# modelscope/KAN-TTS

Hardware: AMD Instinct MI355X
Metric: mel-frames/sec (SAM-BERT train) (higher is better)
Workload: dtype bf16; 1 GPU; SAM-BERT full (sambert_16k.yaml zhcn) fwd+bwd+clip+Adam, batch 32/GPU, T_in 64, 14797 valid mel frames on rank 0, dropout on; global_batch=32, parallelism=dp1, launch=graph, collective_world_size=1

## Files before the change

include/kantts_hip.h:

```cpp
#ifndef KANTTS_HIP_H
#define KANTTS_HIP_H

#include <stddef.h>
#include <stdint.h>

#ifdef __cplusplus
extern "C" {
#endif

#define KANTTS_OK 0
#define KANTTS_E_BADARG (-1)
#define KANTTS_E_UNSUPPORTED (-2)
#define KANTTS_E_WORKSPACE (-3)

int kantts_abi_version(void);
const char* kantts_target_arch(void);

#define KANTTS_GEMM_MAX_SEG 4
typedef struct kantts_gemm_seg {
  const float* a;
  const float* a_gate;
  const float* b;
  int64_t a_is, a_ks;
  int64_t b_js, b_ks;
  int64_t b_tap;
  int32_t klen;
  int32_t ntaps;
  int32_t a_tok_axis;
  int32_t a_shift0, a_shift_step;
  int32_t b_tok_axis;
  int32_t b_shift0, b_shift_step;
  float a_drop_p;
  uint64_t a_drop_seed;
  int32_t a_inner, a_Tq, a_Tsrc, a_mul, a_div, a_up;
  int32_t b_inner, b_Tq, b_Tsrc, b_mul, b_div, b_up;
  float a_slope;
  int32_t a_act;
  float b_slope;
  int32_t b_act;
  float a_gate_slope;
  int32_t a_mode, b_mode;
} kantts_gemm_seg;

typedef struct kantts_gemm_args {
  kantts_gemm_seg seg[KANTTS_GEMM_MAX_SEG];
  int32_t nseg;
  int32_t M, N;
  int32_t T;
  float* c;
  int64_t c_is, c_js;
  const float* bias;
  const float* bias2;
  const float* res;
  int64_t r_is, r_js;
  const uint8_t* rowmask;
  const uint8_t* kmask;
  float* a_rowsum;
  float alpha;
  int32_t relu;
  int32_t accumulate;
  int32_t splitk;
  int32_t precision;
  float drop_p;
  uint64_t drop_seed;
  const uint64_t* seed_dev;
  int32_t groups;
  int64_t a_gs, b_gs, c_gs, bias_gs, r_gs;
  float out_slope;
  int32_t out_act;
  const float* gate;
  float gate_slope;
  int32_t z_taps;
  int64_t c_tap;
} kantts_gemm_args;

int kantts_gemm_seg_launch(const kantts_gemm_args* args_host, void* stream);

int kantts_layernorm_fwd(const float* x, const float* gamma, const float* beta, float* y, float* mean,
                         float* rstd, int M, int C, float eps, void* stream);
int kantts_layernorm_bwd(const float* dy, const float* x, const float* gamma, const float* mean,
                         const float* rstd, float* dx, float* dgamma_accum, float* dbeta_accum, int M, int C,
                         void* stream);

int kantts_attn_fwd(const float* q, const float* k, const float* v, int ldq, int ldk, int ldv, float* o, int ldo,
                    float* lse, float* probs, const int32_t* lens, const int32_t* bw_dev, int bw, int B, int H,
                    int L, int d_head, int mode, float drop_p, uint64_t seed, const uint64_t* seed_dev,
                    void* stream);
int kantts_attn_bwd(const float* q, const float* k, const float* v, int ldq, int ldk, int ldv, const float* o,
                    int ldo, const float* d_o, int lddo, const float* lse, float* dvec, float* dq, float* dk,
                    float* dv, int lddq, int lddk, int lddv, int accumulate_dq, const int32_t* lens,
                    const int32_t* bw_dev, int bw, int B, int H, int L, int d_head, int mode, float drop_p,
                    uint64_t seed, const uint64_t* seed_dev, void* stream);

int kantts_pnca_attn_fwd(const float* qkv, const float* hkv, int ldh, float* ox, float* oh, float* lse_x, float* lse_h,
                         const int32_t* lens, const int32_t* bw_dev, int bw_x, int bw_h, int B, int H, int L, int d_head,
                         float drop_p, uint64_t seed_x, uint64_t seed_h, const uint64_t* seed_dev, void* stream);
int kantts_pnca_attn_bwd(const float* qkv, const float* hkv, int ldh, const float* ox, const float* oh, const float* d_ox,
                         const float* d_oh, const float* lse_x, const float* lse_h, float* dqkv, float* dqh, float* dhkv,
                         const int32_t* lens, const int32_t* bw_dev, int bw_x, int bw_h, int B, int H, int L, int d_head,
                         float drop_p, uint64_t seed_x, uint64_t seed_h, const uint64_t* seed_dev, void* stream);

int kantts_lstm_fwd(const float* gx, const float* whh, const float* bhh, const int32_t* lens, float* out,
                    float* gates_save, float* c_save, int B, int T, int H, int ndir, int reverse_first,
                    int precision, void* stream);
int kantts_lstm_bwd(const float* dout, const float* whh, const int32_t* lens, const float* gates_save,
                    const float* c_save, float* dgates, int B, int T, int H, int ndir, int reverse_first,
                    int precision, void* stream);
int kantts_lstm_fwd_range(const float* gx, const float* whh, const float* bhh, const int32_t* lens, float* out,
                          float* gates_save, float* c_save, int B, int T, int H, int ndir, int reverse_first, int t0,
                          int t1, int precision, void* stream);

int kantts_embed_sum_fwd(const float* const* tables_host, int ntab, const int64_t* ids, const float* pos,
                         float* out, float* scaled_out, int rows, int T, int D, float scale, void* stream);
int kantts_embed_sum_bwd(float* const* dtables_host, int ntab, const int64_t* ids, const float* dout, int rows,
                         int D, float scale, void* stream);
typedef struct kantts_plan_args {
  const int64_t* in_lens;
  const int64_t* out_lens;
  const int64_t* dur;
  const float* mel;
  const float* pos;
  const float* inv_ts;
  int32_t B, N, T_mel, Tp, max_len, r, d_mel, depth;
  int64_t* in_l64;
  int32_t* in_l32;
  uint8_t* in_mask;
  int64_t* out_l64;
  int32_t* out_l32;
  uint8_t* out_mask;
  int64_t* lfr_l64;
  int32_t* lfr_l32;
  uint8_t* lfr_mask;
  int64_t* valid;
  float* pos_enc;
  float* prev;
  float* bw_val;
  int32_t* bw_dev;
  float* dec_input;
} kantts_plan_args;
int kantts_teacher_plan(const kantts_plan_args* args, void* stream);

int kantts_lr_index(const int64_t* dur_int, const float* dur_float, int32_t* idx, float* pos, int32_t* cs,
                    int64_t* lens, int B, int N, int Tp, void* stream);
int kantts_lr_gather_fwd(const float* x, const int32_t* idx, const int64_t* valid_lens, float* out, int B, int N,
                         int Tp, int C, int ldo, int out_col_offset, void* stream);
int kantts_lr_gather_bwd(const float* dout, const int32_t* cs, const int64_t* valid_lens, float* dx, int B, int N,
                         int Tp, int C, int ldo, int out_col_offset, int accumulate, void* stream);

int kantts_fsmn_dwconv_fwd(const float* x, const float* w, const float* res, const int64_t* lens, float* y, int B,
                           int T, int C, int K, int left_pad, void* stream);
int kantts_fsmn_dwconv_fwd_rows(const float* x, const float* w, const float* res, const int64_t* lens, float* y, int B,
                                int T, int C, int K, int left_pad, int t0, int t1, void* stream);
int kantts_fsmn_dwconv_bwd(const float* dy, const float* x, const float* w, const int64_t* lens, float* dx,
                           float* dw_accum, float* workspace, long long ws_floats, int B, int T, int C, int K,
                           int left_pad, void* stream);
long long kantts_fsmn_dwconv_bwd_ws(int B, int T, int C, int K);

int kantts_masked_l1(const float* pred, const float* target, const int64_t* lens, float* loss_accum, float* grad,
                     int B, int T, int C, void* stream);

int kantts_elem_loss(const float* a, const float* b, float target, int mode, float scale, float* loss_accum,
                     float* grad, long long n, void* stream);

int kantts_sumsq(const float* x, float* out_accum, long long n, void* stream);

int kantts_adam_step(float* p, const float* g, float* m, float* v, long long n, float lr, float beta1,
                     float beta2, float eps, float weight_decay, float bias_corr1, float bias_corr2,
                     const float* gnorm_sq, float max_norm, const float* dyn_lr_step, void* stream);

int kantts_melspec_fwd(const float* wav, int B, int T, int n_fft, int hop, int frames, int pad_mode,
                       const float* window, const float* twiddle, float eps_power, const int32_t* mel_start,
                       const int32_t* mel_len, const int32_t* mel_off, const float* mel_w, int n_mels,
                       float eps_mel, float* out_mel, float* out_mag, void* stream);

int kantts_melspec_norm_fwd(const float* wav, int B, int T, int n_fft, int hop, int frames, int pad_mode,
                            const float* window, const float* twiddle, float eps_power, const int32_t* mel_start,
                            const int32_t* mel_len, const int32_t* mel_off, const float* mel_w, int n_mels,
                            float eps_mel, float ref_level_db, float min_level_db, float max_norm, int symmetric,
                            float* out_mel, float* out_mag, void* stream);

int kantts_melspec_norm_fwd_fm(const float* wav, int B, int T, int n_fft, int hop, int frames, int pad_mode,
                               const float* window, const float* twiddle, float eps_power, const int32_t* mel_start,
                               const int32_t* mel_len, const int32_t* mel_off, const float* mel_w, int n_mels, float eps_mel,
                               float ref_level_db, float min_level_db, float max_norm, int symmetric, int mel_frame_major,
                               float* out_mel, float* out_mag, void* stream);
int kantts_melspec_bwd_fm(const float* wav, const float* dmel, int B, int T, int n_fft, int hop, int frames, int pad_mode,
                          const float* window, const float* twiddle, float eps_power, const int32_t* mel_start,
                          const int32_t* mel_len, const int32_t* mel_off, const float* mel_w, int n_mels, float eps_mel,
                          int mel_frame_major, float* dwav_accum, void* stream);

int kantts_copy_roof(const void* src, long long read_bytes, void* dst, long long write_bytes, void* stream);

int kantts_melspec_tuning(int grid_cap, int generic_only);

int kantts_melspec_bwd(const float* wav, const float* dmel, int B, int T, int n_fft, int hop, int frames,
                       int pad_mode, const float* window, const float* twiddle, float eps_power,
                       const int32_t* mel_start, const int32_t* mel_len, const int32_t* mel_off, const float* mel_w,
                       int n_mels, float eps_mel, float* dwav_accum, void* stream);

#define KANTTS_LOSS_MAX_TERMS 5
typedef struct kantts_loss_term {
  const float* pred;
  const void* target;
  const int64_t* lens;
  float* grad;
  int32_t B, T, C, target_log1p;
} kantts_loss_term;
int kantts_masked_l1_many(const kantts_loss_term* terms, int nterms, float* losses, void* stream);
int kantts_scale_many(float* const* x, const long long* n, int count, const float* scale_dev, void* stream);

#define KANTTS_ELOSS_MAX_TERMS 64
typedef struct kantts_eloss_term {
  const float* a;
  const float* b;
  float* grad;
  long long n;
  float target, scale;
  int32_t mode, out;
} kantts_eloss_term;
int kantts_elem_loss_many(const kantts_eloss_term* terms, int nterms, float* losses, void* stream);

int kantts_weight_norm_fwd(const float* v, const float* g, float* w, int rows, int cols, void* stream);
int kantts_weight_norm_bwd(const float* dw, const float* v, const float* g, float* dv, float* dg, int rows,
                           int cols, void* stream);

int kantts_weight_norm_strided_fwd(const float* v, const float* g, float* w, int rows, int cin, int K, long long rs,
                                   long long cs, long long ks, void* stream);
int kantts_weight_norm_strided_bwd(const float* dw, const float* v, const float* g, float* dv, float* dg, int rows,
                                   int cin, int K, long long rs, long long cs, long long ks, void* stream);

int kantts_weight_norm_tap_images(const float* v, const float* g, float* w, void* wf_bf16, void* wd_bf16, int rows, int cin,
                                  int K, int groups, void* stream);

typedef struct kantts_wn_desc {
  int64_t v_off, g_off, w_off, wf_off, wd_off;
  int32_t rows, cin, K, groups, row0, pad_;
} kantts_wn_desc;
int kantts_weight_norm_table(const float* flat, float* w, void* wf_bf16, void* wd_bf16, const kantts_wn_desc* table_dev,
                             int ndesc, int total_tiles, void* stream);

#define KANTTS_WN_BWD_MAX 64
typedef struct kantts_wn_bwd_args {
  const float* dw[KANTTS_WN_BWD_MAX];
  int32_t desc[KANTTS_WN_BWD_MAX];
  int32_t tile0[KANTTS_WN_BWD_MAX + 1];
  int32_t nl;
} kantts_wn_bwd_args;
int kantts_weight_norm_table_bwd(const float* flat, float* grad_flat, const kantts_wn_desc* table_dev,
                                 const kantts_wn_bwd_args* args, void* stream);

int kantts_sinadd_fwd(const float* x, float* y, long long n, void* stream);
int kantts_sinadd_bwd(const float* dy, const float* x, float* dx, long long n, void* stream);

typedef struct {
  const float* in;
  const float* in_gate;
  const float* w;
  float* out;
  const float* bias;
  const float* res;
  const float* out_gate;
  int B, Tsrc, Tdst, Cin_tot, Ntot, CR, NG, groups, K;
  int in_mul, in_add, in_kstep, in_div, phases;
  int inner;
  int up;
  float in_slope;
  int in_act;
  float in_gate_slope;
  float out_slope;
  int out_act;
  float out_gate_slope;
  int precision;
} kantts_conv_args;
int kantts_conv_win_launch(const kantts_conv_args* args, void* stream);

typedef struct {
  const float* x;
  const float* dy;
  const float* dy_gate;
  float* dw;
  float* db;
  int B, Tsrc, Tdst, Cin_tot, Ntot, CR, NG, groups, K;
  int stride, dil, pad, inner;
  int up;
  float x_slope;
  int x_act;
  float dy_gate_slope;
  int precision;
} kantts_convw_args;
int kantts_conv_wgrad_launch(const kantts_convw_args* args, void* stream);

typedef struct {
  const float* x;
  float* dx;
  float* y;
  const float* gate;
  const float* w;
  const float* bias;
  float* dw;
  float* db;
// ... 135 lines not shown
  int32_t relu;
  float alpha1;
  float drop1_p;
  float drop2_p;
  float xdrop_p;
  uint64_t drop1_seed;
  uint64_t drop2_seed;
  uint64_t xdrop_seed;
  const uint64_t* seed_dev;
  const void* gate;
  const uint8_t* rowmask1;
  const uint8_t* rowmask2;
  const uint8_t* xrowmask;
  void* t_out;
  const float* res;
  int64_t ldr;
  void* y;
  int64_t ldy;
  int32_t y_bf16;
  int32_t KT2, s2_first, s2_step;
  const float* ln_gamma;
  const float* ln_beta;
  void* ln_out;
  int32_t ln_out_bf16;
  float ln_eps;
  float* ln_mean;
  float* ln_rstd;
} kantts_ffn_args;
int kantts_ffn_pair(const kantts_ffn_args* args, void* stream);

typedef struct kantts_pnca_block_args {
  const float* x;
  const void* xn;
  const float* hkv;
  int64_t ldh;
  int32_t B, L, H, C, F;
  const int32_t* lens;
  const int32_t* bw_dev;
  int32_t bw_x, bw_h;
  const uint8_t* rowmask;
  const void* wqkv;
  const float* bqkv;
  const void* wfcx;
  const void* wfch;
  const float* bfcx;
  const float* bfch;
  const float* ln1_gamma;
  const float* ln1_beta;
  float ln1_eps;
  const void* w1;
  const void* w2;
  const float* bias1;
  const float* bias2;
  float att_p, fc_p, drop1_p, drop2_p;
  uint64_t seed_x, seed_h, fc_seed, drop1_seed, drop2_seed;
  const uint64_t* seed_dev;
  float* qkv;
  float* ox;
  float* oh;
  float* lse_x;
  float* lse_h;
  float* y1;
  void* xn1;
  float* mean1;
  float* rstd1;
  void* hid;
  float* out;
  const float* ln2_gamma;
  const float* ln2_beta;
  void* ln2_out;
  int32_t ln2_out_bf16;
  float ln2_eps;
  float* ln2_mean;
  float* ln2_rstd;
} kantts_pnca_block_args;
int kantts_pnca_block_fwd(const kantts_pnca_block_args* args, void* stream);

typedef struct kantts_pnca_block_bwd_args {
  const float* dy;
  const void* hid;
  const float* y1;
  const float* mean1;
  const float* rstd1;
  const float* ln1_gamma;
  const uint8_t* rowmask;
  int32_t M, C, F;
  const void* wt2;
  const void* wt1;
  const void* wfcxT;
  const void* wfchT;
  float alpha1, drop2_p, fc_p;
  uint64_t drop2_seed, fc_seed;
  const uint64_t* seed_dev;
  void* dz;
  float* g1;
  float* d_ox;
  float* d_oh;
  float* ws;
  long long ws_floats;
} kantts_pnca_block_bwd_args;
int kantts_pnca_block_bwd(const kantts_pnca_block_bwd_args* args, void* stream);
long long kantts_pnca_block_bwd_ws_floats(int M);
typedef struct kantts_pnca_attn_bwd_args {
  const float* qkv;
  const float* hkv;
  int64_t ldh;
  const float* ox;
  const float* oh;
  const float* d_ox;
  const float* d_oh;
  const float* lse_x;
  const float* lse_h;
  int32_t B, L, H, C;
  const int32_t* lens;
  const int32_t* bw_dev;
  int32_t bw_x, bw_h;
  float att_p;
  uint64_t seed_x, seed_h;
  const uint64_t* seed_dev;
  const void* wqkvT;
  const float* x;
  const float* mean0;
  const float* rstd0;
  const float* ln0_gamma;
  const float* dres;
  const uint8_t* zero_rows;
  float* dqkv;
  float* dhkv;
  int64_t lddh;
  float* dx;
  float* ws;
  long long ws_floats;
} kantts_pnca_attn_bwd_args;
int kantts_pnca_attn_qkv_bwd(const kantts_pnca_attn_bwd_args* args, void* stream);

#define KANTTS_ROWSUM_MAX 32
typedef struct kantts_rowsum_args {
  int32_t n, cols, split;
  int32_t rows[KANTTS_ROWSUM_MAX];
  const float* src[KANTTS_ROWSUM_MAX];
  float* dst0[KANTTS_ROWSUM_MAX];
  float* dst1[KANTTS_ROWSUM_MAX];
} kantts_rowsum_args;
int kantts_rows_sum_many(const kantts_rowsum_args* args, void* stream);

typedef struct kantts_fragmajor_desc {
  int64_t src_off, dst_off;
  int64_t sr, sk;
  int32_t R, K;
} kantts_fragmajor_desc;
int kantts_fragmajor_bf16(const float* src, void* dst_bf16, const kantts_fragmajor_desc* table_dev, int ndesc,
                          int blocks_per_desc, void* stream);

int kantts_ln128_fwd(const float* x, const float* gamma, const float* beta, void* y, int y_bf16, float* mean, float* rstd,
                     int M, float eps, void* stream);
int kantts_ln128_bwd(const void* dy, int dy_bf16, const float* x, const float* gamma, const float* mean, const float* rstd,
                     const float* dres, float* dx, float* dgamma_accum, float* dbeta_accum, int M, void* stream);
int kantts_ln128_bwd_rows(const void* dy, int dy_bf16, const float* x, const float* gamma, const float* mean,
                          const float* rstd, const float* dres, float* dx, float* dgamma_accum, float* dbeta_accum,
                          const unsigned char* zero_rows, int M, void* stream);

int kantts_stft_mag_bwd(const float* wav, const float* dmag, int B, int T, int n_fft, int hop, int frames, int pad_mode,
                        const float* window, const float* twiddle, float eps_power, float* dwav_accum, void* stream);

int kantts_sumsq_det(const float* x, float* out, float* workspace, long long ws_floats, long long n, void* stream);

int kantts_pnca_decode_step(const float* qkv, int ldq, float* xkv_cache, const float* hkv, float* ox, float* oh,
                            const int32_t* lens, const int32_t* bw_seq, int B, int H, int L, int d_head, int step,
                            const int32_t* step_dev, int bw, void* stream);
int kantts_step_rows(const float* src, float* dst, int B, int n, long long src_batch_stride, long long dst_batch_stride,
                     long long src_step_stride, long long dst_step_stride, int step, const int32_t* step_dev, void* stream);
int kantts_step_rowmask(const int32_t* lens, uint8_t* mask, int B, int step, const int32_t* step_dev, void* stream);

int kantts_mean_many(const float* const* xs_host, int n, float scale, float* out, void* act_bf16, float slope,
                     long long numel, void* stream);
int kantts_scale_to_many(const float* g, float scale, float* const* outs_host, int n, long long numel, void* stream);

int kantts_upsample_stream(const void* x_bf16, const void* wp_bf16, const float* bias, const void* res, void* out, int B,
                           int T, int Cin, int Cout, int S, float in_slope, int out_bf16, void* stream);
int kantts_sinadd_lrelu_fwd(const float* x, float* y, void* act_bf16, float slope, long long n, void* stream);

int kantts_dropout2_add(const float* x, const float* res, float* y, long long n, float p1, uint64_t seed1, float p2,
                        uint64_t seed2, const uint64_t* seed_dev, void* stream);

typedef struct {
  const void* in;
  const void* w;
  const float* bias;
  const float* res;
  const void* out_gate;
  float* out;
  void* out_bf;
  int B, Tsrc, Tdst, Cin_tot, Ntot, CR, NG, groups, K;
  int in_mul, in_add, in_kstep, in_div, phases;
  int inner;
  int up;
  float out_slope;
  int out_act;
  float out_gate_slope;
  int out_gate_bf16;
  float bf_slope;
  int bf_act;
  int tile;
  int res_after_gate;
} kantts_cconv_args;
int kantts_cconv_launch(const kantts_cconv_args* args, void* stream);

typedef struct {
  const void* x;
  const void* dy;
  float* dw;
  float* db;
  int B, Tsrc, Tdst, Cin_tot, Ntot, CR, NG, groups, K;
  int stride, dil, pad, inner, up;
  int slices;
  float* workspace;
  long long ws_floats;
} kantts_cconvw_args;
int kantts_cconv_wgrad_launch(const kantts_cconvw_args* args, void* stream);
long long kantts_cconv_wgrad_ws_floats(const kantts_cconvw_args* args);

int kantts_act_cast_bf16(const float* src, const void* gate, int gate_bf16, void* dst, int act, float slope, long long n,
                         void* stream);

int kantts_ragged_rows_f32(const float* src, const int64_t* row_off, const int32_t* start, const int32_t* len,
                           const float* pad, float* out, int B, int Tmax, int C, int transpose, void* stream);
int kantts_ragged_rows_i64(const int64_t* src, const int64_t* row_off, const int32_t* start, const int32_t* len,
                           const int64_t* pad, int64_t* out, int B, int Tmax, int C, int transpose, void* stream);

int kantts_launch_tuning(int tn_tile, int tn_slices, int c1_wgrad_wgs);

typedef struct kantts_decode_args {
  const void* w;
  const float* f;
  const float* memory;
  const float* hkv;
  float* xkv;
  float* out;
  const int32_t* lens;
  const int32_t* bw_seq;
  int B, L, d_mem, d_mel, d_out, n_layer, bw;
  float in_scale;
  float eps;
} kantts_decode_args;
int kantts_pnca_decode_run(const kantts_decode_args* args, void* stream);
int kantts_pnca_decode_range(const kantts_decode_args* args, int t0, int t1, void* stream);
int kantts_pnca_decode_blob_sizes(int d_mel, int d_mem, int d_out, int n_layer, long long* w_elems, long long* f_elems);

typedef struct kantts_durar_args {
  const void* w;
  const float* f;
  const float* gc;
  float* out;
  const int32_t* lens;
  int B, T;
} kantts_durar_args;
int kantts_dur_ar_run(const kantts_durar_args* args, void* stream);
int kantts_dur_ar_run_f32(const kantts_durar_args* args, void* stream);

typedef struct kantts_ctc_args {
  const float* logits;
  const int32_t* in_lens;
  const int32_t* out_lens;
  float* ws;
  float* loss;
  float* grad;
  int B, T1, T2;
  float blank;
  float grad_scale;
} kantts_ctc_args;
long long kantts_ctc_attn_workspace(int B, int T1, int T2);
int kantts_ctc_attn(const kantts_ctc_args* args, void* stream);

typedef struct kantts_enc_attn_args {
  const float* x;
  const void* xn;
  const int32_t* lens;
  const uint8_t* rowmask;
  const void* wqkv;
  const float* bqkv;
  const void* wfc;
  const float* bfc;
  const float* ln1_gamma;
  const float* ln1_beta;
  float ln1_eps;
  float att_p, fc_p;
  uint64_t att_seed, fc_seed;
  const uint64_t* seed_dev;
  float* qkv;
  float* o;
  float* lse;
  float* y1;
  void* xn1;
  int xn1_bf16;
  float* mean1;
  float* rstd1;
  int B, L;
} kantts_enc_attn_args;
int kantts_enc_attn_fwd(const kantts_enc_attn_args* args, void* stream);

typedef struct {
  const float* in;
  const float* hist_in;
  float* hist_out;
  const void* w;
  const float* bias;
// ... 17 lines not shown
```

kan-tts_amd/csrc/ffn_pair.hip:

```cpp
#include "common.h"

typedef float f32x4 __attribute__((ext_vector_type(4)));
typedef __bf16 bf16x8 __attribute__((ext_vector_type(8)));
typedef __bf16 bf16x4 __attribute__((ext_vector_type(4)));
typedef unsigned int u32x4 __attribute__((ext_vector_type(4)));
typedef unsigned int u32x2 __attribute__((ext_vector_type(2)));

#define FP_THREADS 512
#define FP_BM 32
#define FP_K1 128
#define FP_N 128
#define FP_F 1024
#define FP_XP (FP_K1 + 16)
#define FP_XROWS 40
#define FP_TP (FP_F + 16)

__device__ __forceinline__ unsigned fp_pack2(float a, float b) {
  bf16x4 t = {(__bf16)a, (__bf16)b, (__bf16)0.f, (__bf16)0.f};
  return ((u32x2&)t).x;
}
__device__ __forceinline__ float fp_lo(unsigned u) { return __uint_as_float(u << 16); }
__device__ __forceinline__ float fp_hi(unsigned u) { return __uint_as_float(u & 0xffff0000u); }

template <bool BWD, int KT2>
__global__ __launch_bounds__(FP_THREADS) void ffn_pair_kernel(const kantts_ffn_args g) {
#include "ffn_pair_body.inc"
}
static bool fp_aligned16(const void* p) { return ((uintptr_t)p & 15) == 0; }

extern "C" int kantts_ffn_pair(const kantts_ffn_args* gp, void* stream) {
  if (!gp) return KANTTS_E_BADARG;
  const kantts_ffn_args& g = *gp;
  if (!g.x || !g.w1 || !g.w2 || !g.y || g.M < 0 || g.KT < 1) return KANTTS_E_BADARG;
  if (g.K1 != FP_K1 || g.N != FP_N || g.F != FP_F) return KANTTS_E_UNSUPPORTED;
  if (g.KT > 9 || g.pad < 0 || g.pad >= g.KT || (g.KT > 1 && g.T <= 0)) return KANTTS_E_UNSUPPORTED;
  if ((g.ldx & 7) || (g.ldy & 3) || (g.res && (g.ldr & 3))) return KANTTS_E_UNSUPPORTED;
  if (!fp_aligned16(g.x) || !fp_aligned16(g.w1) || !fp_aligned16(g.w2) || !fp_aligned16(g.y) ||
      (g.t_out && !fp_aligned16(g.t_out)) || (g.gate && !fp_aligned16(g.gate)) || (g.res && !fp_aligned16(g.res)) ||
      (g.bias1 && !fp_aligned16(g.bias1)) || (g.bias2 && !fp_aligned16(g.bias2)))
    return KANTTS_E_UNSUPPORTED;
  if (g.xdrop_p > 0.f && !g.x_f32) return KANTTS_E_UNSUPPORTED;
  if (g.gate && g.KT != 1) return KANTTS_E_UNSUPPORTED;
  const int kt2 = g.KT2 < 1 ? 1 : g.KT2;
  if (kt2 != 1 && kt2 != 3) return KANTTS_E_UNSUPPORTED;
  if (kt2 == 3 && (!g.gate || g.T <= 0 || (g.s2_step != 1 && g.s2_step != -1) || g.M % g.T)) return KANTTS_E_UNSUPPORTED;
  if (g.ln_out) {
    if (!g.ln_gamma || !g.ln_beta || !g.ln_mean || !g.ln_rstd) return KANTTS_E_BADARG;
    if (g.gate || kt2 != 1 || !fp_aligned16(g.ln_out) || !fp_aligned16(g.ln_gamma) || !fp_aligned16(g.ln_beta))
      return KANTTS_E_UNSUPPORTED;
  }
  if (g.M == 0) return KANTTS_OK;
  hipStream_t st = (hipStream_t)stream;
  if (kt2 == 3)
    hipLaunchKernelGGL((ffn_pair_kernel<true, 3>), dim3(kantts_cdiv(g.M, FP_BM - 2)), dim3(FP_THREADS), 0, st, g);
  else if (g.gate)
    hipLaunchKernelGGL((ffn_pair_kernel<true, 1>), dim3(kantts_cdiv(g.M, FP_BM)), dim3(FP_THREADS), 0, st, g);
  else
    hipLaunchKernelGGL((ffn_pair_kernel<false, 1>), dim3(kantts_cdiv(g.M, FP_BM)), dim3(FP_THREADS), 0, st, g);
  KANTTS_CHECK_LAUNCH();
}

__global__ __launch_bounds__(256) void fragmajor_bf16_kernel(const float* __restrict__ src, __bf16* __restrict__ dst,
                                                            const kantts_fragmajor_desc* __restrict__ tab) {
  const kantts_fragmajor_desc d = tab[blockIdx.y];
  const long long total = (long long)d.R * d.K;
  const unsigned KB = (unsigned)d.K >> 5;
  const bool fast = total < (1ll << 31) && (d.dst_off & 7) == 0;
  if (fast) {
    const unsigned total8 = (unsigned)(total >> 3);
    const bool contig = d.sk == 1 && ((d.src_off | d.sr) & 3) == 0;
    for (unsigned o8 = blockIdx.x * blockDim.x + threadIdx.x; o8 < total8; o8 += gridDim.x * blockDim.x) {
      const unsigned lane = o8 & 63u, blk = o8 >> 6;
      const unsigned rb = blk / KB, kb = blk - rb * KB;
      const long long r = (long long)rb * 16 + (lane & 15u), k0 = (long long)kb * 32 + (lane >> 4) * 8;
      const float* sp = src + d.src_off + r * d.sr + k0 * d.sk;
      float v[8];
      if (contig) {
        const float4 a = reinterpret_cast<const float4*>(sp)[0], b = reinterpret_cast<const float4*>(sp)[1];
        v[0] = a.x, v[1] = a.y, v[2] = a.z, v[3] = a.w, v[4] = b.x, v[5] = b.y, v[6] = b.z, v[7] = b.w;
      } else {
#pragma unroll
        for (int e = 0; e < 8; ++e) v[e] = sp[(long long)e * d.sk];
      }
      bf16x8 o;
#pragma unroll
      for (int e = 0; e < 8; ++e) o[e] = (__bf16)v[e];
      *reinterpret_cast<bf16x8*>(dst + d.dst_off + (long long)o8 * 8) = o;
    }
    return;
  }
  for (long long o = (long long)blockIdx.x * blockDim.x + threadIdx.x; o < total; o += (long long)gridDim.x * blockDim.x) {
    const int e = (int)(o & 7), lane = (int)((o >> 3) & 63);
    const long long blk = o >> 9;
    const int kb = (int)(blk % KB), rb = (int)(blk / KB);
    const long long r = (long long)rb * 16 + (lane & 15), k = (long long)kb * 32 + (lane >> 4) * 8 + e;
    dst[d.dst_off + o] = (__bf16)src[d.src_off + r * d.sr + k * d.sk];
  }
}

extern "C" int kantts_fragmajor_bf16(const float* src, void* dst, const kantts_fragmajor_desc* table_dev, int ndesc,
                                     int blocks_per_desc, void* stream) {
  if (!src || !dst || !table_dev || ndesc < 0 || blocks_per_desc < 1) return KANTTS_E_BADARG;
  if (ndesc == 0) return KANTTS_OK;
  hipLaunchKernelGGL(fragmajor_bf16_kernel, dim3(blocks_per_desc, ndesc), dim3(256), 0, (hipStream_t)stream, src,
                     reinterpret_cast<__bf16*>(dst), table_dev);
  KANTTS_CHECK_LAUNCH();
}
```

kan-tts_amd/csrc/gemm_bf16.hip:

```cpp
#include <stdlib.h>

#include "common.h"

typedef float f32x4 __attribute__((ext_vector_type(4)));
typedef __bf16 bf16x8 __attribute__((ext_vector_type(8)));
typedef __bf16 bf16x4 __attribute__((ext_vector_type(4)));
typedef unsigned int u32x4 __attribute__((ext_vector_type(4)));
typedef unsigned int u32x2 __attribute__((ext_vector_type(2)));

#define BG_THREADS 256
#define BG_BN 128
#define BG_BK 64
#define BG_LDKN (BG_BN + 16)

typedef __attribute__((address_space(3))) bf16x4 bg_lds_bf16x4;
__device__ __forceinline__ bf16x4 bg_tr4(const __bf16* p) {
  return __builtin_amdgcn_ds_read_tr16_b64_v4bf16((bg_lds_bf16x4*)(p));
}

__device__ __forceinline__ unsigned bg_pack2(float a, float b) {
  bf16x4 t = {(__bf16)a, (__bf16)b, (__bf16)0.f, (__bf16)0.f};
  return ((u32x2&)t).x;
}
__device__ __forceinline__ float bg_lo(unsigned u) { return __uint_as_float(u << 16); }
// ... 320 lines not shown
#pragma unroll
      for (int m = 0; m < MR; ++m)
#pragma unroll
        for (int n = 0; n < NR; ++n)
          acc[m][n] = __builtin_amdgcn_mfma_f32_16x16x32_bf16(af[m], bf[n], acc[m][n], 0, 0, 0);
    }
  };

  const int st = g.slices;
  int t = slice;
  const int tlast = ntile - 1;
  fetch(min(t, tlast), ra0, rb0);
  fetch(min(t + st, tlast), ra1, rb1);
  for (; t < ntile; t += 2 * st) {
    commit(0, t, ra0, rb0);
    __syncthreads();
    fetch(min(t + 2 * st, tlast), ra0, rb0);
    compute(0);
    if (t + st < ntile) {
      commit(1, t + st, ra1, rb1);
      __syncthreads();
      fetch(min(t + 3 * st, tlast), ra1, rb1);
      compute(1);
    }
  }

  if (do_bias && tid < BN && (n0 + tid) < g.N && colsum != 0.f) atomicAdd(&g.db[n0 + tid], colsum * g.alpha);
  float* cbase = g.c + (long long)tap * g.c_ts;
#pragma unroll
  for (int m = 0; m < MR; ++m)
#pragma unroll
    for (int n = 0; n < NR; ++n)
#pragma unroll
      for (int r = 0; r < 4; ++r) {
        const int i = n0 + wr * (BN / 2) + m * 16 + kg * 4 + r;
        const int j = c0 + wc * (BK / 2) + n * 16 + li;
        if (i < g.N && j < g.K) {
          const float v = acc[m][n][r] * g.alpha;
#ifdef TN_NO_ATOMICS
          if (v != 0.f) cbase[(long long)i * g.c_ns + (long long)j * g.c_ks] = v;
#else
          if (v != 0.f) atomicAdd(cbase + (long long)i * g.c_ns + (long long)j * g.c_ks, v);
#endif
        }
      }
}

template <bool A_F32, bool B_F32, int BN, int BK>
static int bg_tn_go(TnGroupArgs& ga, dim3 grid, hipStream_t st) {
  constexpr size_t LDS = 2 * (size_t)TN_BT * ((BN + 16) + (BK + 16)) * 2;
  static bool attr_set = false;
  if (!attr_set && LDS > 64 * 1024) {
    hipError_t e = hipFuncSetAttribute(reinterpret_cast<const void*>(&bgemm_tn_kernel<A_F32, B_F32, BN, BK>),
                                       hipFuncAttributeMaxDynamicSharedMemorySize, (int)LDS);
    if (e != hipSuccess) return (int)e;
    attr_set = true;
  }
  hipLaunchKernelGGL((bgemm_tn_kernel<A_F32, B_F32, BN, BK>), grid, dim3(BG_THREADS), LDS, st, ga);
  KANTTS_CHECK_LAUNCH();
}

template <int BN, int BK>
static int bg_tn_dispatch(TnGroupArgs& ga, dim3 grid, hipStream_t st) {
  const kantts_bgemm_tn_args& g = ga.g;
  if (g.a_f32) {
    if (g.b_f32) return bg_tn_go<true, true, BN, BK>(ga, grid, st);
    return bg_tn_go<true, false, BN, BK>(ga, grid, st);
  }
  if (g.b_f32) return bg_tn_go<false, true, BN, BK>(ga, grid, st);
  return bg_tn_go<false, false, BN, BK>(ga, grid, st);
}

static int bg_tn_tile_rule(const kantts_bgemm_tn_args& g, int nprob) {
  (void)g;
  (void)nprob;
  return 64128;
}

static int bg_tn_launch(TnGroupArgs& ga, hipStream_t st) {
  kantts_bgemm_tn_args& g = ga.g;
  if (g.M < 0 || g.N < 1 || g.K < 1 || g.ntaps < 1 || ga.nprob < 1 || ga.nprob > KANTTS_TN_MAX_GROUP) return KANTTS_E_BADARG;
  if (g.M == 0) return KANTTS_OK;
  if ((g.N & 7) || (g.K & 7) || (g.lda & 7) || (g.ldb & 7)) return KANTTS_E_UNSUPPORTED;
  for (int p = 0; p < ga.nprob; ++p) {
    if (!ga.a[p] || !ga.b[p] || !ga.c[p]) return KANTTS_E_BADARG;
    if (!bg_aligned16(ga.a[p]) || !bg_aligned16(ga.b[p])) return KANTTS_E_UNSUPPORTED;
  }
  if ((g.shift0 != 0 || g.shift_step != 0) && g.T <= 0) return KANTTS_E_BADARG;
  int code = kantts_tune_tn_tile.load(std::memory_order_relaxed);
  const int forced_slices = kantts_tune_tn_slices.load(std::memory_order_relaxed);
  bool xcd_map = true;
  if (code == 64129 || code == 128129 || code == 64257 || code == 128257) code -= 1, xcd_map = false;
  if (code != 64128 && code != 128128 && code != 64256 && code != 128256) code = bg_tn_tile_rule(g, ga.nprob);
  const int BN = code / 1000, BK = code % 1000;
  const int tiles = kantts_cdiv(g.N, BN) * kantts_cdiv(g.K, BK) * g.ntaps * ga.nprob;
  const int ntile = kantts_cdiv(g.M, TN_BT);
  int slices = g.slices;
  if (forced_slices > 0) slices = forced_slices;
  if (slices <= 0) {
    static const bool r2_rule = getenv("KANTTS_TN_SLICE_RULE_R2") != nullptr;
    slices = r2_rule ? kantts_cdiv(320, tiles) : 512 / tiles;
    if (xcd_map && !r2_rule) {
      const int P = kantts_cdiv(g.N, BN) * kantts_cdiv(g.K, BK);
      const int per_xcd = P <= 64 ? 64 / P : 1;
      slices = 8 * per_xcd / (g.ntaps * ga.nprob);
    }
    if (slices < 1) slices = 1;
    if (slices > 16 && !r2_rule) slices = 16;
    const long long cap = ((r2_rule ? 3ll << 19 : 1ll << 22)) / ((long long)g.N * g.K * g.ntaps * ga.nprob) + 1;
    if (slices > cap) slices = (int)cap;
  }
  if (slices > ntile) slices = ntile;
  if (slices < 1) slices = 1;
  g.slices = slices;
  dim3 grid(kantts_cdiv(g.K, BK), kantts_cdiv(g.N, BN), ga.nprob * g.ntaps * slices);
  ga.ktiles = ga.ntiles = ga.ngroups = 0;
  if (xcd_map && (int)grid.z * 4 < 3 * 8 * kantts_cdiv((int)grid.z, 8)) xcd_map = false;
  if (xcd_map) {
    ga.ktiles = (int)grid.x, ga.ntiles = (int)grid.y, ga.ngroups = (int)grid.z;
    grid = dim3(8u * grid.x * grid.y * (unsigned)kantts_cdiv(ga.ngroups, 8), 1, 1);
  }
  switch (code) {
    case 128256: return bg_tn_dispatch<128, 256>(ga, grid, st);
    case 128128: return bg_tn_dispatch<128, 128>(ga, grid, st);
    case 64256: return bg_tn_dispatch<64, 256>(ga, grid, st);
    default: return bg_tn_dispatch<64, 128>(ga, grid, st);
  }
}

extern "C" int kantts_bgemm_tn(const kantts_bgemm_tn_args* gp, void* stream) {
  if (!gp) return KANTTS_E_BADARG;
  TnGroupArgs ga = {};
  ga.g = *gp;
  ga.nprob = 1;
  ga.a[0] = gp->a; ga.b[0] = gp->b; ga.c[0] = gp->c; ga.db[0] = gp->db; ga.a_drop_seed[0] = gp->a_drop_seed;
  return bg_tn_launch(ga, (hipStream_t)stream);
}

extern "C" int kantts_bgemm_tn_grouped(const kantts_bgemm_tn_args* shape, int nprob, const void* const* a,
                                       const void* const* b, float* const* c, float* const* db,
                                       const uint64_t* a_drop_seed, void* stream) {
  if (!shape || !a || !b || !c || nprob < 1 || nprob > KANTTS_TN_MAX_GROUP) return KANTTS_E_BADARG;
  TnGroupArgs ga = {};
  ga.g = *shape;
  ga.nprob = nprob;
  for (int p = 0; p < nprob; ++p) {
    ga.a[p] = a[p]; ga.b[p] = b[p]; ga.c[p] = c[p];
    ga.db[p] = db ? db[p] : nullptr;
    ga.a_drop_seed[p] = a_drop_seed ? a_drop_seed[p] : shape->a_drop_seed;
  }
  return bg_tn_launch(ga, (hipStream_t)stream);
}

__global__ __launch_bounds__(256) void cast_bf16_kernel(const float* __restrict__ src, __bf16* __restrict__ dst, long long n8) {
  const long long i = (long long)blockIdx.x * blockDim.x + threadIdx.x;
  if (i >= n8) return;
  const float4 a = reinterpret_cast<const float4*>(src)[2 * i], b = reinterpret_cast<const float4*>(src)[2 * i + 1];
  u32x4 w = {bg_pack2(a.x, a.y), bg_pack2(a.z, a.w), bg_pack2(b.x, b.y), bg_pack2(b.z, b.w)};
  reinterpret_cast<u32x4*>(dst)[i] = w;
}

extern "C" int kantts_cast_f32_bf16(const float* src, void* dst, long long n, void* stream) {
  if (!src || !dst || n < 0 || (n & 7) || !bg_aligned16(src) || !bg_aligned16(dst)) return KANTTS_E_BADARG;
  if (n == 0) return KANTTS_OK;
  const long long n8 = n / 8;
  hipLaunchKernelGGL(cast_bf16_kernel, dim3(kantts_cdiv(n8, 256)), dim3(256), 0, (hipStream_t)stream, src,
                     reinterpret_cast<__bf16*>(dst), n8);
  KANTTS_CHECK_LAUNCH();
}

__global__ __launch_bounds__(256) void tapmajor_bf16_kernel(const float* __restrict__ src, __bf16* __restrict__ dst,
                                                           const kantts_tapmajor_desc* __restrict__ tab) {
  const kantts_tapmajor_desc d = tab[blockIdx.y];
  const long long total = (long long)d.N * d.Cin * d.KT;
  for (long long o = (long long)blockIdx.x * blockDim.x + threadIdx.x; o < total; o += (long long)gridDim.x * blockDim.x) {
    const int c = (int)(o % d.Cin);
    const long long q = o / d.Cin;
    const int n = (int)(q % d.N), tap = (int)(q / d.N);
    dst[d.dst_off + o] = (__bf16)src[d.src_off + ((long long)n * d.Cin + c) * d.KT + tap];
  }
}

extern "C" int kantts_tapmajor_bf16(const float* src, void* dst, const kantts_tapmajor_desc* table_dev, int ndesc,
                                    int blocks_per_desc, void* stream) {
  if (!src || !dst || !table_dev || ndesc < 0 || blocks_per_desc < 1) return KANTTS_E_BADARG;
  if (ndesc == 0) return KANTTS_OK;
  hipLaunchKernelGGL(tapmajor_bf16_kernel, dim3(blocks_per_desc, ndesc), dim3(256), 0, (hipStream_t)stream, src,
                     reinterpret_cast<__bf16*>(dst), table_dev);
  KANTTS_CHECK_LAUNCH();
}

template <bool DY_BF16, bool Y_BF16>
__global__ __launch_bounds__(256) void relu_gate_kernel(const void* __restrict__ dy, const void* __restrict__ y,
                                                       __bf16* __restrict__ dz, float scale, long long n8) {
  const long long i = (long long)blockIdx.x * blockDim.x + threadIdx.x;
  if (i >= n8) return;
  float d[8], a[8];
  if (DY_BF16) {
    const u32x4 q = reinterpret_cast<const u32x4*>(dy)[i];
    d[0] = bg_lo(q.x); d[1] = bg_hi(q.x); d[2] = bg_lo(q.y); d[3] = bg_hi(q.y);
    d[4] = bg_lo(q.z); d[5] = bg_hi(q.z); d[6] = bg_lo(q.w); d[7] = bg_hi(q.w);
  } else {
    const float4 p = reinterpret_cast<const float4*>(dy)[2 * i], q = reinterpret_cast<const float4*>(dy)[2 * i + 1];
    d[0] = p.x; d[1] = p.y; d[2] = p.z; d[3] = p.w; d[4] = q.x; d[5] = q.y; d[6] = q.z; d[7] = q.w;
  }
  if (Y_BF16) {
    const u32x4 q = reinterpret_cast<const u32x4*>(y)[i];
    a[0] = bg_lo(q.x); a[1] = bg_hi(q.x); a[2] = bg_lo(q.y); a[3] = bg_hi(q.y);
    a[4] = bg_lo(q.z); a[5] = bg_hi(q.z); a[6] = bg_lo(q.w); a[7] = bg_hi(q.w);
  } else {
    const float4 p = reinterpret_cast<const float4*>(y)[2 * i], q = reinterpret_cast<const float4*>(y)[2 * i + 1];
    a[0] = p.x; a[1] = p.y; a[2] = p.z; a[3] = p.w; a[4] = q.x; a[5] = q.y; a[6] = q.z; a[7] = q.w;
  }
  float o[8];
#pragma unroll
  for (int e = 0; e < 8; ++e) o[e] = a[e] > 0.f ? d[e] * scale : 0.f;
  u32x4 w = {bg_pack2(o[0], o[1]), bg_pack2(o[2], o[3]), bg_pack2(o[4], o[5]), bg_pack2(o[6], o[7])};
  reinterpret_cast<u32x4*>(dz)[i] = w;
}

extern "C" int kantts_relu_gate_bf16(const void* dy, int dy_bf16, const void* y, int y_bf16, void* dz_bf16, float scale,
                                     long long n, void* stream) {
  if (!dy || !y || !dz_bf16 || n < 0 || (n & 7) || !bg_aligned16(dy) || !bg_aligned16(y) || !bg_aligned16(dz_bf16))
    return KANTTS_E_BADARG;
  if (n == 0) return KANTTS_OK;
  const long long n8 = n / 8;
  dim3 grid(kantts_cdiv(n8, 256)), block(256);
  hipStream_t st = (hipStream_t)stream;
  __bf16* o = reinterpret_cast<__bf16*>(dz_bf16);
  if (dy_bf16) {
    if (y_bf16)
      hipLaunchKernelGGL((relu_gate_kernel<true, true>), grid, block, 0, st, dy, y, o, scale, n8);
    else
      hipLaunchKernelGGL((relu_gate_kernel<true, false>), grid, block, 0, st, dy, y, o, scale, n8);
  } else {
    if (y_bf16)
      hipLaunchKernelGGL((relu_gate_kernel<false, true>), grid, block, 0, st, dy, y, o, scale, n8);
    else
      hipLaunchKernelGGL((relu_gate_kernel<false, false>), grid, block, 0, st, dy, y, o, scale, n8);
  }
  KANTTS_CHECK_LAUNCH();
}
```

kan-tts_amd/csrc/seq.hip:

```cpp
#include "common.h"

struct EmbedArgs {
  const float* tab[4];
  int ntab;
  const int64_t* ids;
  const float* pos;
  float* out;
  float* scaled;
  int rows, T, D;
  float scale;
};

__global__ void embed_sum_kernel(const EmbedArgs a) {
  long long idx = (long long)blockIdx.x * blockDim.x + threadIdx.x;
  long long total = (long long)a.rows * a.D;
  if (idx >= total) return;
  int row = (int)(idx / a.D), d = (int)(idx % a.D);
  float s = 0.f;
  for (int k = 0; k < a.ntab; ++k) s += a.tab[k][(long long)a.ids[(long long)row * a.ntab + k] * a.D + d];
  s *= a.scale;
  if (a.scaled) a.scaled[idx] = s;
  if (a.pos) s += a.pos[(long long)(row % a.T) * a.D + d];
  a.out[idx] = s;
}
// ... 53 lines not shown
      for (int w = 0; w < EB_WAYS; ++w) {
        if (w == next) {
          if (tag[w] >= 0) atomicAdd(&tab[tag[w] * a.D + d], acc[w]);
          tag[w] = id;
          acc[w] = g;
        }
      }
      next = (next + 1) & (EB_WAYS - 1);
    }
   }
  }
#pragma unroll
  for (int w = 0; w < EB_WAYS; ++w)
    if (tag[w] >= 0) atomicAdd(&tab[tag[w] * a.D + d], acc[w]);
}

extern "C" int kantts_embed_sum_fwd(const float* const* tables_host, int ntab, const int64_t* ids, const float* pos,
                                    float* out, float* scaled_out, int rows, int T, int D, float scale, void* stream) {
  if (!tables_host || ntab < 1 || ntab > 4 || !ids || !out || rows < 0 || D < 1 || T < 1) return KANTTS_E_BADARG;
  if (rows == 0) return KANTTS_OK;
  EmbedArgs a = {};
  for (int k = 0; k < ntab; ++k) a.tab[k] = tables_host[k];
  a.ntab = ntab; a.ids = ids; a.pos = pos; a.out = out; a.scaled = scaled_out; a.rows = rows; a.T = T; a.D = D;
  a.scale = scale;
  hipLaunchKernelGGL(embed_sum_kernel, dim3(kantts_cdiv((long long)rows * D, 256)), dim3(256), 0, (hipStream_t)stream, a);
  KANTTS_CHECK_LAUNCH();
}

extern "C" int kantts_embed_sum_bwd(float* const* dtables_host, int ntab, const int64_t* ids, const float* dout,
                                    int rows, int D, float scale, void* stream) {
  if (!dtables_host || ntab < 1 || ntab > 4 || !ids || !dout || rows < 0 || D < 1) return KANTTS_E_BADARG;
  if (rows == 0) return KANTTS_OK;
  EmbedBwdArgs a = {};
  for (int k = 0; k < ntab; ++k) a.dtab[k] = dtables_host[k];
  a.ntab = ntab; a.ids = ids; a.dout = dout; a.rows = rows; a.D = D; a.scale = scale;
  const long long threads = (long long)kantts_cdiv(rows, EB_CHUNK) * ntab * D;
  hipLaunchKernelGGL(embed_sum_bwd_kernel, dim3(kantts_cdiv(threads, 256)), dim3(256), 0, (hipStream_t)stream, a);
  KANTTS_CHECK_LAUNCH();
}

__global__ __launch_bounds__(64) void lr_index_kernel(const int64_t* __restrict__ dur_i, const float* __restrict__ dur_f,
                                                      int32_t* __restrict__ idx, float* __restrict__ pos,
                                                      int32_t* __restrict__ cs, int64_t* __restrict__ lens, int N,
                                                      int Tp) {
  const int b = blockIdx.x, lane = threadIdx.x;
  int32_t* csb = cs + (long long)b * (N + 1);
  int carry = 0;
  for (int n0 = 0; n0 < N; n0 += 64) {
    int n = n0 + lane;
    int rep = 0;
    if (n < N) {
      if (dur_i)
        rep = (int)dur_i[(long long)b * N + n];
      else
        rep = (int)(long long)(dur_f[(long long)b * N + n] + 0.5f);
    }
    int v = rep;
#pragma unroll
    for (int off = 1; off < 64; off <<= 1) {
      int u = __shfl_up(v, off, 64);
      if (lane >= off) v += u;
    }
    if (n < N) csb[n + 1] = carry + v;
    carry += __shfl(v, 63, 64);
  }
  if (lane == 0) {
    csb[0] = 0;
    lens[b] = carry;
  }
  __syncthreads();
  __threadfence_block();
  const int total = carry;
  for (int t = lane; t < Tp; t += 64) {
    int id = -1;
    float p = (float)(t + 1);
    if (t < total) {
      int lo = 0, hi = N;
      while (hi - lo > 1) {
        int mid = (lo + hi) >> 1;
        if (csb[mid] <= t)
          lo = mid;
        else
          hi = mid;
      }
      id = lo;
      p = (float)(t - csb[lo] + 1);
    }
    idx[(long long)b * Tp + t] = id;
    pos[(long long)b * Tp + t] = p;
  }
}

extern "C" int kantts_lr_index(const int64_t* dur_int, const float* dur_float, int32_t* idx, float* pos, int32_t* cs,
                               int64_t* lens, int B, int N, int Tp, void* stream) {
  if ((!dur_int && !dur_float) || !idx || !pos || !cs || !lens || B < 0 || N < 1 || Tp < 0) return KANTTS_E_BADARG;
  if (B == 0) return KANTTS_OK;
  hipLaunchKernelGGL(lr_index_kernel, dim3(B), dim3(64), 0, (hipStream_t)stream, dur_int, dur_float, idx, pos, cs,
                     lens, N, Tp);
  KANTTS_CHECK_LAUNCH();
}

__global__ void lr_gather_kernel(const float* __restrict__ x, const int32_t* __restrict__ idx,
                                 const int64_t* __restrict__ valid, float* __restrict__ out, int B, int N, int Tp, int C,
                                 int ldo, int ooff) {
  long long g = (long long)blockIdx.x * blockDim.x + threadIdx.x;
  long long total = (long long)B * Tp * C;
  if (g >= total) return;
  int c = (int)(g % C);
  long long bt = g / C;
  int t = (int)(bt % Tp), b = (int)(bt / Tp);
  int id = idx[bt];
  float v = 0.f;
  if (id >= 0 && (!valid || t < (int)valid[b])) v = x[((long long)b * N + id) * C + c];
  out[bt * ldo + ooff + c] = v;
}

__global__ void lr_gather_bwd_kernel(const float* __restrict__ dout, const int32_t* __restrict__ cs,
                                     const int64_t* __restrict__ valid, float* __restrict__ dx, int B, int N, int Tp,
                                     int C, int ldo, int ooff, int accumulate) {
  long long g = (long long)blockIdx.x * blockDim.x + threadIdx.x;
  long long total = (long long)B * N * C;
  if (g >= total) return;
  int c = (int)(g % C);
  long long bn = g / C;
  int n = (int)(bn % N), b = (int)(bn / N);
  int s = cs[(long long)b * (N + 1) + n], e = cs[(long long)b * (N + 1) + n + 1];
  if (e > Tp) e = Tp;
  if (valid && e > (int)valid[b]) e = (int)valid[b];
  float acc = 0.f;
  for (int t = s; t < e; ++t) acc += dout[((long long)b * Tp + t) * ldo + ooff + c];
  if (accumulate)
    dx[g] += acc;
  else
    dx[g] = acc;
}

extern "C" int kantts_lr_gather_fwd(const float* x, const int32_t* idx, const int64_t* valid_lens, float* out, int B,
                                    int N, int Tp, int C, int ldo, int out_col_offset, void* stream) {
  if (!x || !idx || !out || B < 0 || N < 1 || Tp < 0 || C < 1 || ldo < C) return KANTTS_E_BADARG;
  long long total = (long long)B * Tp * C;
  if (total == 0) return KANTTS_OK;
  hipLaunchKernelGGL(lr_gather_kernel, dim3(kantts_cdiv(total, 256)), dim3(256), 0, (hipStream_t)stream, x, idx,
                     valid_lens, out, B, N, Tp, C, ldo, out_col_offset);
  KANTTS_CHECK_LAUNCH();
}

extern "C" int kantts_lr_gather_bwd(const float* dout, const int32_t* cs, const int64_t* valid_lens, float* dx, int B,
                                    int N, int Tp, int C, int ldo, int out_col_offset, int accumulate, void* stream) {
  if (!dout || !cs || !dx || B < 0 || N < 1 || Tp < 0 || C < 1 || ldo < C) return KANTTS_E_BADARG;
  long long total = (long long)B * N * C;
  if (total == 0) return KANTTS_OK;
  hipLaunchKernelGGL(lr_gather_bwd_kernel, dim3(kantts_cdiv(total, 256)), dim3(256), 0, (hipStream_t)stream, dout, cs,
                     valid_lens, dx, B, N, Tp, C, ldo, out_col_offset, accumulate);
  KANTTS_CHECK_LAUNCH();
}

#define DW_TT 32
template <bool ROWS>
__global__ void fsmn_dwconv_fwd_kernel(const float* __restrict__ x, const float* __restrict__ w,
                                       const float* __restrict__ res, const int64_t* __restrict__ lens,
                                       float* __restrict__ y, int B, int T, int C, int K, int lp, int r0, int r1) {
  const int b = blockIdx.y, t0 = (ROWS ? r0 : 0) + blockIdx.x * DW_TT;
  const int len = lens ? (int)min((long long)lens[b], (long long)T) : T;
  const float* xb = x + (long long)b * T * C;
  for (int c = threadIdx.x; c < C; c += blockDim.x) {
    const float* wc = w + (long long)c * K;
    for (int tt = 0; tt < DW_TT; ++tt) {
      const int t = t0 + tt;
      if (t >= (ROWS ? r1 : T)) break;
      float acc = 0.f;
      if (t < len) {
        for (int k = 0; k < K; ++k) {
          int ts = t + k - lp;
          if (ts >= 0 && ts < len) acc = fmaf(wc[k], xb[(long long)ts * C + c], acc);
        }
        acc += xb[(long long)t * C + c];
      }
      long long o = ((long long)b * T + t) * C + c;
      if (res) acc += res[o];
      y[o] = acc;
    }
  }
}

__global__ void fsmn_dwconv_bwd_dx_kernel(const float* __restrict__ dy, const float* __restrict__ w,
                                          const int64_t* __restrict__ lens, float* __restrict__ dx, int B, int T, int C,
                                          int K, int lp) {
  const int b = blockIdx.y, t0 = blockIdx.x * DW_TT;
  const int len = lens ? (int)min((long long)lens[b], (long long)T) : T;
  const float* db = dy + (long long)b * T * C;
  for (int c = threadIdx.x; c < C; c += blockDim.x) {
    const float* wc = w + (long long)c * K;
    for (int tt = 0; tt < DW_TT; ++tt) {
      const int t = t0 + tt;
      if (t >= T) break;
      float acc = 0.f;
      if (t < len) {
        for (int k = 0; k < K; ++k) {
          int ts = t - k + lp;
          if (ts >= 0 && ts < len) acc = fmaf(wc[k], db[(long long)ts * C + c], acc);
        }
        acc += db[(long long)t * C + c];
      }
      dx[((long long)b * T + t) * C + c] = acc;
    }
  }
}

#define DW_WT 128
__global__ void fsmn_dwconv_bwd_dw_kernel(const float* __restrict__ dy, const float* __restrict__ x,
                                          const int64_t* __restrict__ lens, float* __restrict__ dw, int B, int T, int C,
                                          int K, int lp) {
  const int b = blockIdx.y, t0 = blockIdx.x * DW_WT;
  const int len = lens ? (int)min((long long)lens[b], (long long)T) : T;
  if (t0 >= len) return;
  const int t1 = min(t0 + DW_WT, len);
  const float* db = dy + (long long)b * T * C;
  const float* xb = x + (long long)b * T * C;
  for (int c = threadIdx.x; c < C; c += blockDim.x) {
    for (int k = 0; k < K; ++k) {
      float acc = 0.f;
      for (int t = t0; t < t1; ++t) {
        int ts = t + k - lp;
        if (ts >= 0 && ts < len) acc = fmaf(db[(long long)t * C + c], xb[(long long)ts * C + c], acc);
      }
      atomicAdd(&dw[(long long)c * K + k], acc);
    }
  }
}

#define FS_K 41
#define FS_TT 16
template <bool FLIP, bool ROWS>
__global__ __launch_bounds__(256, 2) void fsmn_fir41_kernel(const float* __restrict__ x, const float* __restrict__ w,
                                                        const float* __restrict__ res,
                                                        const int64_t* __restrict__ lens, float* __restrict__ y, int B,
                                                        int T, int C, int lp, int xcd_order, int r0, int r1) {
  int bx = blockIdx.x, by = blockIdx.y;
  if (xcd_order) {
    const int gx = gridDim.x, total = gx * gridDim.y;
    if (total >= 64) {
      const int L = by * gx + bx, k = L & 7, j = L >> 3;
      const int q = total >> 3, r = total & 7;
      const int vid = k * q + (k < r ? k : r) + j;
      by = vid / gx;
      bx = vid - by * gx;
    }
  }
  const int b = by, t0 = (ROWS ? r0 : 0) + bx * FS_TT;
  const int len = lens ? (int)min((long long)lens[b], (long long)T) : T;
  const int lpe = FLIP ? (FS_K - 1 - lp) : lp;
  const int xlim = ROWS ? min(len, r1 + (FS_K - 1 - lpe)) : len;
  const int tlim = ROWS ? r1 : T;
  const float* xb = x + (long long)b * T * C;
  for (int c = threadIdx.x; c < C; c += blockDim.x) {
    float wk[FS_K];
#pragma unroll
    for (int k = 0; k < FS_K; ++k) wk[k] = w[(long long)c * FS_K + (FLIP ? (FS_K - 1 - k) : k)];
    float xin[FS_TT + FS_K - 1];
#pragma unroll
    for (int n = 0; n < FS_TT + FS_K - 1; ++n) {
      const int ts = t0 + n - lpe;
      const bool ok = (ts >= 0) && (ts < xlim);
      const float v = xb[(long long)(ok ? ts : 0) * C + c];
      xin[n] = ok ? v : 0.f;
    }
    float ctr[FS_TT];
#pragma unroll
    for (int o = 0; o < FS_TT; ++o) {
      const int t = t0 + o;
      const bool ok = t < (ROWS ? min(len, r1) : len);
      const float v = xb[(long long)(ok ? t : 0) * C + c];
      ctr[o] = ok ? v : 0.f;
    }
#pragma unroll
    for (int o = 0; o < FS_TT; ++o) {
      const int t = t0 + o;
      float acc = ctr[o];
#pragma unroll
      for (int k = 0; k < FS_K; ++k) acc = fmaf(wk[k], xin[o + k], acc);
      if (t < tlim) {
        const long long oidx = ((long long)b * T + t) * C + c;
        float outv = (t < len) ? acc : 0.f;
        if (!FLIP && res) outv += res[oidx];
        y[oidx] = outv;
      }
    }
  }
}

#define FS_CH 128
#define FS_SUB (FS_CH / 4)
__global__ __launch_bounds__(256) void fsmn_dw41_partial_kernel(const float* __restrict__ dy, const float* __restrict__ x,
                                                            const int64_t* __restrict__ lens,
                                                            float* __restrict__ part, int B, int T, int C, int lp) {
  __shared__ float sm[4][FS_K][65];
  const int b = blockIdx.y, chunk = blockIdx.x, nchunk = gridDim.x;
  const int wave = threadIdx.x >> 6, lane = threadIdx.x & 63;
  const int c0 = blockIdx.z * 64, c = c0 + lane;
  const bool cok = c < C;
  const int cc = cok ? c : 0;
  const int len = lens ? (int)min((long long)lens[b], (long long)T) : T;
  const float* xb = x + (long long)b * T * C;
  const float* db = dy + (long long)b * T * C;
  const int tbeg = chunk * FS_CH + wave * FS_SUB, tend = min(tbeg + FS_SUB, T);
  float acc[FS_K];
// ... 223 lines not shown
```

kan-tts_amd/kantts/_hip/__init__.py:

```python
import ctypes
import os
from ctypes import (POINTER, Structure, c_char_p, c_float, c_int, c_int32, c_int64, c_longlong,
                    c_uint64, c_void_p)

import torch

_HERE = os.path.dirname(os.path.abspath(__file__))
LIB_PATH = os.environ.get("KANTTS_LIB") or os.path.normpath(os.path.join(_HERE, "..", "..", "libkantts_hip.so"))
_lib = None

GEMM_MAX_SEG = 4
PREC_FP32, PREC_BF16, PREC_REF = 0, 1, 2


class GemmSeg(Structure):
    _fields_ = [
        ("a", c_void_p), ("a_gate", c_void_p), ("b", c_void_p),
        ("a_is", c_int64), ("a_ks", c_int64), ("b_js", c_int64), ("b_ks", c_int64), ("b_tap", c_int64),
        ("klen", c_int32), ("ntaps", c_int32),
        ("a_tok_axis", c_int32), ("a_shift0", c_int32), ("a_shift_step", c_int32),
        ("b_tok_axis", c_int32), ("b_shift0", c_int32), ("b_shift_step", c_int32),
        ("a_drop_p", c_float), ("a_drop_seed", c_uint64),
        ("a_inner", c_int32), ("a_Tq", c_int32), ("a_Tsrc", c_int32), ("a_mul", c_int32), ("a_div", c_int32),
        ("a_up", c_int32),
# ... 125 lines not shown
        ("x", c_void_p), ("gamma", c_void_p), ("mean", c_void_p), ("rstd", c_void_p), ("dres", c_void_p),
        ("zero_rows", c_void_p), ("dx", c_void_p), ("dgamma_accum", c_void_p), ("dbeta_accum", c_void_p),
        ("part_rows", c_void_p),
    ]


LOSS_MAX_TERMS = 5


class LossTerm(Structure):
    _fields_ = [("pred", c_void_p), ("target", c_void_p), ("lens", c_void_p), ("grad", c_void_p),
                ("B", c_int32), ("T", c_int32), ("C", c_int32), ("target_log1p", c_int32)]


ELOSS_MAX_TERMS = 64


class ElossTerm(Structure):
    _fields_ = [("a", c_void_p), ("b", c_void_p), ("grad", c_void_p), ("n", ctypes.c_longlong), ("target", ctypes.c_float),
                ("scale", ctypes.c_float), ("mode", c_int32), ("out", c_int32)]


WN_BWD_MAX = 64


class WnBwdArgs(Structure):
    _fields_ = [("dw", c_void_p * WN_BWD_MAX), ("desc", c_int32 * WN_BWD_MAX), ("tile0", c_int32 * (WN_BWD_MAX + 1)),
                ("nl", c_int32)]


class BGemmTnArgs(Structure):
    _fields_ = [
        ("a", c_void_p), ("b", c_void_p), ("lda", c_int64), ("ldb", c_int64),
        ("M", c_int32), ("N", c_int32), ("K", c_int32), ("T", c_int32),
        ("a_f32", c_int32), ("b_f32", c_int32),
        ("ntaps", c_int32), ("shift0", c_int32), ("shift_step", c_int32), ("slices", c_int32),
        ("c", c_void_p), ("c_ns", c_int64), ("c_ks", c_int64), ("c_ts", c_int64),
        ("db", c_void_p), ("alpha", c_float), ("a_drop_p", c_float),
        ("a_drop_seed", c_uint64), ("seed_dev", c_void_p),
    ]


class FfnArgs(Structure):
    _fields_ = [
        ("x", c_void_p), ("ldx", c_int64), ("x_f32", c_int32),
        ("M", c_int32), ("T", c_int32), ("K1", c_int32), ("F", c_int32), ("N", c_int32), ("KT", c_int32), ("pad", c_int32),
        ("w1", c_void_p), ("w2", c_void_p), ("bias1", c_void_p), ("bias2", c_void_p),
        ("relu", c_int32), ("alpha1", c_float), ("drop1_p", c_float), ("drop2_p", c_float), ("xdrop_p", c_float),
        ("drop1_seed", c_uint64), ("drop2_seed", c_uint64), ("xdrop_seed", c_uint64), ("seed_dev", c_void_p),
        ("gate", c_void_p), ("rowmask1", c_void_p), ("rowmask2", c_void_p), ("xrowmask", c_void_p),
        ("t_out", c_void_p), ("res", c_void_p), ("ldr", c_int64), ("y", c_void_p), ("ldy", c_int64), ("y_bf16", c_int32),
        ("KT2", c_int32), ("s2_first", c_int32), ("s2_step", c_int32),
        ("ln_gamma", c_void_p), ("ln_beta", c_void_p), ("ln_out", c_void_p), ("ln_out_bf16", c_int32), ("ln_eps", c_float),
        ("ln_mean", c_void_p), ("ln_rstd", c_void_p),
    ]


class PncaBlockArgs(Structure):
    _fields_ = [
        ("x", c_void_p), ("xn", c_void_p), ("hkv", c_void_p), ("ldh", c_int64),
        ("B", c_int32), ("L", c_int32), ("H", c_int32), ("C", c_int32), ("F", c_int32),
        ("lens", c_void_p), ("bw_dev", c_void_p), ("bw_x", c_int32), ("bw_h", c_int32), ("rowmask", c_void_p),
        ("wqkv", c_void_p), ("bqkv", c_void_p), ("wfcx", c_void_p), ("wfch", c_void_p), ("bfcx", c_void_p), ("bfch", c_void_p),
        ("ln1_gamma", c_void_p), ("ln1_beta", c_void_p), ("ln1_eps", c_float),
        ("w1", c_void_p), ("w2", c_void_p), ("bias1", c_void_p), ("bias2", c_void_p),
        ("att_p", c_float), ("fc_p", c_float), ("drop1_p", c_float), ("drop2_p", c_float),
        ("seed_x", c_uint64), ("seed_h", c_uint64), ("fc_seed", c_uint64), ("drop1_seed", c_uint64), ("drop2_seed", c_uint64),
        ("seed_dev", c_void_p),
        ("qkv", c_void_p), ("ox", c_void_p), ("oh", c_void_p), ("lse_x", c_void_p), ("lse_h", c_void_p), ("y1", c_void_p),
        ("xn1", c_void_p), ("mean1", c_void_p), ("rstd1", c_void_p), ("hid", c_void_p), ("out", c_void_p),
        ("ln2_gamma", c_void_p), ("ln2_beta", c_void_p), ("ln2_out", c_void_p), ("ln2_out_bf16", c_int32), ("ln2_eps", c_float),
        ("ln2_mean", c_void_p), ("ln2_rstd", c_void_p),
    ]


class PncaBlockBwdArgs(Structure):
    _fields_ = [
        ("dy", c_void_p), ("hid", c_void_p), ("y1", c_void_p), ("mean1", c_void_p), ("rstd1", c_void_p), ("ln1_gamma", c_void_p),
        ("rowmask", c_void_p), ("M", c_int32), ("C", c_int32), ("F", c_int32),
        ("wt2", c_void_p), ("wt1", c_void_p), ("wfcxT", c_void_p), ("wfchT", c_void_p),
        ("alpha1", c_float), ("drop2_p", c_float), ("fc_p", c_float), ("drop2_seed", c_uint64), ("fc_seed", c_uint64),
        ("seed_dev", c_void_p),
        ("dz", c_void_p), ("g1", c_void_p), ("d_ox", c_void_p), ("d_oh", c_void_p), ("ws", c_void_p), ("ws_floats", c_int64),
    ]


class PncaAttnBwdArgs(Structure):
    _fields_ = [
        ("qkv", c_void_p), ("hkv", c_void_p), ("ldh", c_int64), ("ox", c_void_p), ("oh", c_void_p), ("d_ox", c_void_p),
        ("d_oh", c_void_p), ("lse_x", c_void_p), ("lse_h", c_void_p),
        ("B", c_int32), ("L", c_int32), ("H", c_int32), ("C", c_int32),
        ("lens", c_void_p), ("bw_dev", c_void_p), ("bw_x", c_int32), ("bw_h", c_int32), ("att_p", c_float),
        ("seed_x", c_uint64), ("seed_h", c_uint64), ("seed_dev", c_void_p),
        ("wqkvT", c_void_p), ("x", c_void_p), ("mean0", c_void_p), ("rstd0", c_void_p), ("ln0_gamma", c_void_p),
        ("dres", c_void_p), ("zero_rows", c_void_p),
        ("dqkv", c_void_p), ("dhkv", c_void_p), ("lddh", c_int64), ("dx", c_void_p), ("ws", c_void_p), ("ws_floats", c_int64),
    ]


class PlanArgs(Structure):
    _fields_ = [("in_lens", c_void_p), ("out_lens", c_void_p), ("dur", c_void_p), ("mel", c_void_p), ("pos", c_void_p),
                ("inv_ts", c_void_p),
                ("B", c_int32), ("N", c_int32), ("T_mel", c_int32), ("Tp", c_int32), ("max_len", c_int32), ("r", c_int32),
                ("d_mel", c_int32), ("depth", c_int32),
                ("in_l64", c_void_p), ("in_l32", c_void_p), ("in_mask", c_void_p), ("out_l64", c_void_p), ("out_l32", c_void_p),
                ("out_mask", c_void_p), ("lfr_l64", c_void_p), ("lfr_l32", c_void_p), ("lfr_mask", c_void_p),
                ("valid", c_void_p), ("pos_enc", c_void_p), ("prev", c_void_p), ("bw_val", c_void_p), ("bw_dev", c_void_p),
                ("dec_input", c_void_p)]


class DecodeArgs(Structure):
    _fields_ = [("w", c_void_p), ("f", c_void_p), ("memory", c_void_p), ("hkv", c_void_p), ("xkv", c_void_p),
                ("out", c_void_p), ("lens", c_void_p), ("bw_seq", c_void_p),
                ("B", c_int32), ("L", c_int32), ("d_mem", c_int32), ("d_mel", c_int32), ("d_out", c_int32),
                ("n_layer", c_int32), ("bw", c_int32), ("in_scale", c_float), ("eps", c_float)]


class DurArArgs(Structure):
    _fields_ = [("w", c_void_p), ("f", c_void_p), ("gc", c_void_p), ("out", c_void_p), ("lens", c_void_p),
                ("B", c_int32), ("T", c_int32)]


class EncAttnArgs(Structure):
    _fields_ = [("x", c_void_p), ("xn", c_void_p), ("lens", c_void_p), ("rowmask", c_void_p), ("wqkv", c_void_p),
                ("bqkv", c_void_p), ("wfc", c_void_p), ("bfc", c_void_p), ("ln1_gamma", c_void_p), ("ln1_beta", c_void_p),
                ("ln1_eps", c_float), ("att_p", c_float), ("fc_p", c_float), ("att_seed", c_uint64), ("fc_seed", c_uint64),
                ("seed_dev", c_void_p), ("qkv", c_void_p), ("o", c_void_p), ("lse", c_void_p), ("y1", c_void_p),
                ("xn1", c_void_p), ("xn1_bf16", c_int32), ("mean1", c_void_p), ("rstd1", c_void_p), ("B", c_int32),
                ("L", c_int32)]


class CtcArgs(Structure):
    _fields_ = [("logits", c_void_p), ("in_lens", c_void_p), ("out_lens", c_void_p), ("ws", c_void_p), ("loss", c_void_p),
                ("grad", c_void_p), ("B", c_int32), ("T1", c_int32), ("T2", c_int32), ("blank", c_float),
                ("grad_scale", c_float)]


ROWSUM_MAX = 32


class RowSumArgs(Structure):
    _fields_ = [("n", c_int32), ("cols", c_int32), ("split", c_int32), ("rows", c_int32 * ROWSUM_MAX),
                ("src", c_void_p * ROWSUM_MAX), ("dst0", c_void_p * ROWSUM_MAX), ("dst1", c_void_p * ROWSUM_MAX)]


class FragMajorDesc(Structure):
    _fields_ = [("src_off", c_int64), ("dst_off", c_int64), ("sr", c_int64), ("sk", c_int64), ("R", c_int32),
                ("K", c_int32)]


class TapMajorDesc(Structure):
    _fields_ = [("src_off", c_int64), ("dst_off", c_int64), ("N", c_int32), ("Cin", c_int32), ("KT", c_int32),
                ("pad_", c_int32)]


def available() -> bool:
    return os.path.exists(LIB_PATH)


def lib():
    global _lib
    if _lib is None:
        if not os.path.exists(LIB_PATH):
            raise RuntimeError(
                "libkantts_hip.so is not built (%s). Run `python -c 'import __graft_entry__ as g; g.build()'` "
                "or `make -C kan-tts_amd/csrc`. There is no CPU fallback." % LIB_PATH)
        L = ctypes.CDLL(LIB_PATH)
        L.kantts_abi_version.restype = c_int
        L.kantts_target_arch.restype = c_char_p
        L.kantts_gemm_seg_launch.argtypes = [POINTER(GemmArgs), c_void_p]
        i, f, p, ll, u64 = c_int, c_float, c_void_p, c_longlong, c_uint64
        L.kantts_layernorm_fwd.argtypes = [p, p, p, p, p, p, i, i, f, p]
        L.kantts_layernorm_bwd.argtypes = [p, p, p, p, p, p, p, p, i, i, p]
        L.kantts_attn_fwd.argtypes = [p, p, p, i, i, i, p, i, p, p, p, p, i, i, i, i, i, i, f, u64, p, p]
        L.kantts_attn_bwd.argtypes = [p, p, p, i, i, i, p, i, p, i, p, p, p, p, p, i, i, i, i, p, p, i, i, i, i, i,
                                      i, f, u64, p, p]
        L.kantts_pnca_attn_fwd.argtypes = [p, p, i, p, p, p, p, p, p, i, i, i, i, i, i, f, u64, u64, p, p]
        L.kantts_pnca_attn_bwd.argtypes = [p, p, i, p, p, p, p, p, p, p, p, p, p, p, i, i, i, i, i, i, f, u64, u64, p, p]
        L.kantts_lstm_fwd.argtypes = [p, p, p, p, p, p, p, i, i, i, i, i, i, p]
        L.kantts_attn_decode.argtypes = [p, p, p, i, i, i, p, i, p, p, i, i, i, i, i, i, i, p]
        L.kantts_lstm_cell.argtypes = [p, p, p, p, i, i, p]
        L.kantts_mas_width1.argtypes = [p, p, p, p, p, i, i, i, p]
        L.kantts_align_attn_fwd.argtypes = [p, p, p, p, p, p, i, i, i, i, p]
        L.kantts_align_attn_bwd.argtypes = [p, p, p, p, p, p, p, p, p, p, i, i, i, i, p]
        L.kantts_lstm_bwd.argtypes = [p, p, p, p, p, p, i, i, i, i, i, i, p]
        L.kantts_embed_sum_fwd.argtypes = [POINTER(c_void_p), i, p, p, p, p, i, i, i, f, p]
        L.kantts_embed_sum_bwd.argtypes = [POINTER(c_void_p), i, p, p, i, i, f, p]
        L.kantts_lr_index.argtypes = [p, p, p, p, p, p, i, i, i, p]
        L.kantts_lr_gather_fwd.argtypes = [p, p, p, p, i, i, i, i, i, i, p]
        L.kantts_lr_gather_bwd.argtypes = [p, p, p, p, i, i, i, i, i, i, i, p]
        L.kantts_fsmn_dwconv_fwd.argtypes = [p, p, p, p, p, i, i, i, i, i, p]
        L.kantts_fsmn_dwconv_bwd.argtypes = [p, p, p, p, p, p, p, ll, i, i, i, i, i, p]
        L.kantts_fsmn_dwconv_bwd_ws.argtypes = [i, i, i, i]
        L.kantts_fsmn_dwconv_bwd_ws.restype = ll
        L.kantts_masked_l1.argtypes = [p, p, p, p, p, i, i, i, p]
        L.kantts_sumsq.argtypes = [p, p, ll, p]
        L.kantts_elem_loss.argtypes = [p, p, f, i, f, p, p, ll, p]
        L.kantts_adam_step.argtypes = [p, p, p, p, ll, f, f, f, f, f, f, f, p, f, p, p]
        L.kantts_melspec_fwd.argtypes = [p, i, i, i, i, i, i, p, p, f, p, p, p, p, i, f, p, p, p]
        L.kantts_melspec_norm_fwd.argtypes = [p, i, i, i, i, i, i, p, p, f, p, p, p, p, i, f, f, f, f, i, p, p, p]
        L.kantts_melspec_bwd.argtypes = [p, p, i, i, i, i, i, i, p, p, f, p, p, p, p, i, f, p, p]
        L.kantts_melspec_norm_fwd_fm.argtypes = [p, i, i, i, i, i, i, p, p, f, p, p, p, p, i, f, f, f, f, i, i, p, p, p]
        L.kantts_melspec_bwd_fm.argtypes = [p, p, i, i, i, i, i, i, p, p, f, p, p, p, p, i, f, i, p, p]
        L.kantts_weight_norm_fwd.argtypes = [p, p, p, i, i, p]
        L.kantts_weight_norm_bwd.argtypes = [p, p, p, p, p, i, i, p]
        L.kantts_weight_norm_strided_fwd.argtypes = [p, p, p, i, i, i, ll, ll, ll, p]
        L.kantts_weight_norm_strided_bwd.argtypes = [p, p, p, p, p, i, i, i, ll, ll, ll, p]
        L.kantts_sinadd_fwd.argtypes = [p, p, ll, p]
        L.kantts_sinadd_bwd.argtypes = [p, p, p, ll, p]
        L.kantts_conv_win_launch.argtypes = [POINTER(ConvArgs), c_void_p]
        L.kantts_conv_wgrad_launch.argtypes = [POINTER(ConvWArgs), c_void_p]
        L.kantts_conv_c1_launch.argtypes = [POINTER(ConvC1Args), c_int, c_void_p]
        L.kantts_pnca_decode_step.argtypes = [p, i, p, p, p, p, p, p, i, i, i, i, i, p, i, p]
        L.kantts_step_rows.argtypes = [p, p, i, i, ll, ll, ll, ll, i, p, p]
        L.kantts_step_rowmask.argtypes = [p, p, i, i, p, p]
        L.kantts_upsample_stream.argtypes = [p, p, p, p, p, i, i, i, i, i, f, i, p]
        L.kantts_sinadd_lrelu_fwd.argtypes = [p, p, p, f, ll, p]
        L.kantts_dropout2_add.argtypes = [p, p, p, ll, f, c_uint64, f, c_uint64, p, p]
        L.kantts_sumsq_det.argtypes = [p, p, p, ll, ll, p]
        L.kantts_stft_mag_bwd.argtypes = [p, p, i, i, i, i, i, i, p, p, f, p, p]
        L.kantts_bgemm_nt.argtypes = [POINTER(BGemmArgs), c_void_p]
        L.kantts_ffn_pair.argtypes = [POINTER(FfnArgs), c_void_p]
        L.kantts_pnca_block_fwd.argtypes = [POINTER(PncaBlockArgs), c_void_p]
        L.kantts_pnca_block_bwd.argtypes = [POINTER(PncaBlockBwdArgs), c_void_p]
        L.kantts_rows_sum_many.argtypes = [POINTER(RowSumArgs), c_void_p]
        L.kantts_teacher_plan.argtypes = [POINTER(PlanArgs), c_void_p]
        L.kantts_pnca_attn_qkv_bwd.argtypes = [POINTER(PncaAttnBwdArgs), c_void_p]
        L.kantts_copy_roof.argtypes = [c_void_p, ctypes.c_longlong, c_void_p, ctypes.c_longlong, c_void_p]
        L.kantts_launch_tuning.argtypes = [c_int, c_int, c_int]
        L.kantts_pnca_decode_run.argtypes = [POINTER(DecodeArgs), c_void_p]
        L.kantts_dur_ar_run.argtypes = [POINTER(DurArArgs), c_void_p]
        L.kantts_dur_ar_run_f32.argtypes = [POINTER(DurArArgs), c_void_p]
        L.kantts_enc_attn_fwd.argtypes = [POINTER(EncAttnArgs), c_void_p]
        L.kantts_ctc_attn.argtypes = [POINTER(CtcArgs), c_void_p]
        L.kantts_ctc_attn_workspace.argtypes = [c_int, c_int, c_int]
        L.kantts_ctc_attn_workspace.restype = c_longlong
        L.kantts_pnca_decode_blob_sizes.argtypes = [c_int, c_int, c_int, c_int, POINTER(ctypes.c_longlong),
                                                    POINTER(ctypes.c_longlong)]
        L.kantts_pnca_block_bwd_ws_floats.argtypes = [c_int]
        L.kantts_pnca_block_bwd_ws_floats.restype = ctypes.c_longlong
        L.kantts_fragmajor_bf16.argtypes = [c_void_p, c_void_p, c_void_p, c_int, c_int, c_void_p]
        L.kantts_bgemm_tn.argtypes = [POINTER(BGemmTnArgs), c_void_p]
        L.kantts_bgemm_tn_grouped.argtypes = [POINTER(BGemmTnArgs), c_int, p, p, p, p, p, c_void_p]
        L.kantts_cast_f32_bf16.argtypes = [p, p, ll, p]
        L.kantts_tapmajor_bf16.argtypes = [p, p, p, i, i, p]
        L.kantts_relu_gate_bf16.argtypes = [p, i, p, i, p, f, ll, p]
        L.kantts_ln128_fwd.argtypes = [p, p, p, p, i, p, p, i, f, p]
        L.kantts_ln128_bwd.argtypes = [p, i, p, p, p, p, p, p, p, p, i, p]
        L.kantts_bgemm_nt_lnbwd.argtypes = [POINTER(BGemmArgs), POINTER(LnBwdArgs), c_void_p]
        L.kantts_ln128_bwd_rows.argtypes = [p, i, p, p, p, p, p, p, p, p, p, i, p]
        L.kantts_cconv_launch.argtypes = [POINTER(CConvArgs), c_void_p]
        L.kantts_cconv_wgrad_launch.argtypes = [POINTER(CConvWArgs), c_void_p]
        L.kantts_cconv_wgrad_ws_floats.argtypes = [POINTER(CConvWArgs)]
        L.kantts_cconv_wgrad_ws_floats.restype = ll
        L.kantts_act_cast_bf16.argtypes = [p, p, i, p, i, f, ll, p]
        L.kantts_ragged_rows_f32.argtypes = [p, p, p, p, p, p, i, i, i, i, p]
        L.kantts_weight_norm_tap_images.argtypes = [p, p, p, p, p, i, i, i, i, p]
        L.kantts_weight_norm_table.argtypes = [p, p, p, p, p, i, i, p]
        L.kantts_weight_norm_table_bwd.argtypes = [p, p, p, POINTER(WnBwdArgs), p]
        L.kantts_masked_l1_many.argtypes = [POINTER(LossTerm), i, p, p]
        L.kantts_scale_many.argtypes = [POINTER(c_void_p), POINTER(ll), i, p, p]
        L.kantts_conv_n1_launch.argtypes = [POINTER(ConvN1Args), i, p]
        L.kantts_elem_loss_many.argtypes = [POINTER(ElossTerm), i, p, p]
        L.kantts_mean_many.argtypes = [POINTER(c_void_p), i, f, p, p, f, ll, p]
        L.kantts_scale_to_many.argtypes = [p, f, POINTER(c_void_p), i, ll, p]
        L.kantts_ragged_rows_i64.argtypes = [p, p, p, p, p, p, i, i, i, i, p]
        L.kantts_sconv_launch.argtypes = [POINTER(SConvArgs), c_void_p]
        L.kantts_pnca_decode_range.argtypes = [POINTER(DecodeArgs), c_int, c_int, c_void_p]
        L.kantts_lstm_fwd_range.argtypes = [p, p, p, p, p, p, p, i, i, i, i, i, i, i, i, p]
        L.kantts_fsmn_dwconv_fwd_rows.argtypes = [p, p, p, p, p, i, i, i, i, i, i, i, p]
        _lib = L
    return _lib


EXPORTED_SYMBOLS = [
    "kantts_abi_version", "kantts_target_arch", "kantts_gemm_seg_launch", "kantts_layernorm_fwd",
    "kantts_layernorm_bwd", "kantts_attn_fwd", "kantts_attn_bwd", "kantts_pnca_attn_fwd", "kantts_pnca_attn_bwd", "kantts_lstm_fwd", "kantts_lstm_bwd",
    "kantts_embed_sum_fwd", "kantts_embed_sum_bwd", "kantts_lr_index", "kantts_lr_gather_fwd",
    "kantts_lr_gather_bwd", "kantts_fsmn_dwconv_fwd", "kantts_fsmn_dwconv_bwd", "kantts_fsmn_dwconv_bwd_ws", "kantts_masked_l1",
    "kantts_sumsq", "kantts_elem_loss", "kantts_adam_step", "kantts_melspec_fwd", "kantts_melspec_norm_fwd", "kantts_melspec_bwd", "kantts_melspec_norm_fwd_fm", "kantts_melspec_bwd_fm", "kantts_weight_norm_fwd", "kantts_weight_norm_bwd", "kantts_weight_norm_strided_fwd", "kantts_weight_norm_strided_bwd",
    "kantts_sinadd_fwd", "kantts_sinadd_bwd", "kantts_conv_win_launch", "kantts_conv_wgrad_launch", "kantts_conv_c1_launch", "kantts_attn_decode",
    "kantts_lstm_cell", "kantts_mas_width1", "kantts_align_attn_fwd", "kantts_align_attn_bwd",
    "kantts_bgemm_nt", "kantts_ffn_pair", "kantts_fragmajor_bf16", "kantts_bgemm_tn", "kantts_cast_f32_bf16", "kantts_tapmajor_bf16", "kantts_relu_gate_bf16",
    "kantts_ln128_fwd", "kantts_ln128_bwd", "kantts_ln128_bwd_rows", "kantts_bgemm_nt_lnbwd", "kantts_stft_mag_bwd", "kantts_bgemm_tn_grouped", "kantts_sumsq_det",
    "kantts_pnca_decode_step", "kantts_step_rows", "kantts_step_rowmask", "kantts_upsample_stream",
    "kantts_sinadd_lrelu_fwd", "kantts_dropout2_add",
    "kantts_cconv_launch", "kantts_cconv_wgrad_launch", "kantts_cconv_wgrad_ws_floats", "kantts_act_cast_bf16",
    "kantts_ragged_rows_f32", "kantts_ragged_rows_i64", "kantts_weight_norm_tap_images",
    "kantts_weight_norm_table", "kantts_weight_norm_table_bwd", "kantts_masked_l1_many", "kantts_scale_many",
    "kantts_mean_many", "kantts_scale_to_many", "kantts_elem_loss_many", "kantts_conv_n1_launch",
    "kantts_pnca_block_fwd", "kantts_pnca_block_bwd", "kantts_pnca_block_bwd_ws_floats", "kantts_rows_sum_many",
    "kantts_melspec_tuning", "kantts_teacher_plan", "kantts_copy_roof", "kantts_pnca_attn_qkv_bwd",
    "kantts_pnca_decode_run", "kantts_pnca_decode_blob_sizes", "kantts_dur_ar_run", "kantts_dur_ar_run_f32", "kantts_ctc_attn", "kantts_ctc_attn_workspace", "kantts_enc_attn_fwd",
    "kantts_launch_tuning", "kantts_sconv_launch",
    "kantts_pnca_decode_range", "kantts_lstm_fwd_range", "kantts_fsmn_dwconv_fwd_rows",
]


_launch_tuning = [None]


def apply_launch_tuning():
    L = lib()
    env = os.environ
    want = (id(L), int(env.get("KANTTS_TN_TILE", "0") or 0), int(env.get("KANTTS_TN_SLICES", "0") or 0),
            int(env.get("KANTTS_C1_WGRAD_WGS", "0") or 0))
    if want != _launch_tuning[0]:
        rc = L.kantts_launch_tuning(want[1], max(want[2], 0), max(want[3], 0))
        if rc != 0:
            raise RuntimeError("libkantts_hip: launch_tuning failed with code %d" % rc)
        _launch_tuning[0] = want


def check(rc, what):
    if rc != 0:
        raise RuntimeError("libkantts_hip: %s failed with code %d" % (what, rc))


def stream():
    return c_void_p(torch.cuda.current_stream().cuda_stream)


def ptr(t, dtype=None):
    if t is None:
        return None
    if not t.is_cuda:
        raise RuntimeError("kantts HIP op called with a CPU tensor; the product path has no CPU fallback")
    if dtype is not None and t.dtype != dtype:
        raise TypeError("expected %s, got %s" % (dtype, t.dtype))
    return t.data_ptr()


_precision = {"gemm": PREC_BF16 if os.environ.get("KANTTS_PRECISION", "fp32") == "bf16" else PREC_FP32}
if os.environ.get("KANTTS_GEMM_IMPL", "") == "ref":
    _precision["gemm"] = PREC_REF


def set_precision(mode: str):
    _precision["gemm"] = {"fp32": PREC_FP32, "bf16": PREC_BF16, "ref": PREC_REF}[mode]


def get_precision() -> str:
    return {PREC_FP32: "fp32", PREC_BF16: "bf16", PREC_REF: "ref"}[_precision["gemm"]]


class precision_scope:

    def __init__(self, mode):
        self.mode = mode

    def __enter__(self):
        self.before = _precision["gemm"]
        if self.mode is not None:
            set_precision(self.mode)
        return self

    def __exit__(self, *exc):
        _precision["gemm"] = self.before
        return False


def make_seg(a, a_is, a_ks, b, b_js, b_ks, klen, ntaps=1, b_tap=0, a_tok_axis=0, a_shift0=0, a_shift_step=0,
             b_tok_axis=0, b_shift0=0, b_shift_step=0, a_gate=None, a_drop_p=0.0, a_drop_seed=0, a_map=None,
             b_map=None, a_leaky=None, b_leaky=None, a_gate_slope=0.0):

    def addr(x):
        if x is None:
            return None
        if isinstance(x, tuple):
            return ptr(x[0], torch.float32) + 4 * int(x[1])
        return ptr(x, torch.float32)

    s = GemmSeg()
    s.a, s.a_gate, s.b = addr(a), addr(a_gate), addr(b)
    s.a_is, s.a_ks, s.b_js, s.b_ks, s.b_tap = int(a_is), int(a_ks), int(b_js), int(b_ks), int(b_tap)
    s.klen, s.ntaps = int(klen), int(ntaps)
    s.a_tok_axis, s.a_shift0, s.a_shift_step = int(a_tok_axis), int(a_shift0), int(a_shift_step)
    s.b_tok_axis, s.b_shift0, s.b_shift_step = int(b_tok_axis), int(b_shift0), int(b_shift_step)
    s.a_drop_p, s.a_drop_seed = float(a_drop_p), int(a_drop_seed)
    if a_map:
        s.a_inner, s.a_Tq, s.a_Tsrc = int(a_map.get("inner", 0)), int(a_map.get("Tq", 0)), int(a_map.get("Tsrc", 0))
        s.a_mul, s.a_div, s.a_up = int(a_map.get("mul", 0)), int(a_map.get("div", 0)), int(a_map.get("up", 0))
    if b_map:
        s.b_inner, s.b_Tq, s.b_Tsrc = int(b_map.get("inner", 0)), int(b_map.get("Tq", 0)), int(b_map.get("Tsrc", 0))
        s.b_mul, s.b_div, s.b_up = int(b_map.get("mul", 0)), int(b_map.get("div", 0)), int(b_map.get("up", 0))
    if a_leaky is not None:
        s.a_act, s.a_slope = 1, float(a_leaky)
    if b_leaky is not None:
        s.b_act, s.b_slope = 1, float(b_leaky)
    s.a_gate_slope = float(a_gate_slope)
    return s


def _staging_mode(base, row_stride, k_stride, klen, rows, tok_axis, group_stride, gate=None):
    aligned = (base % 16 == 0) and (gate is None or gate % 16 == 0) and (group_stride % 4 == 0)
    if k_stride == 1 and aligned and klen % 4 == 0 and row_stride % 4 == 0 and tok_axis != 2:
        return 2
    if row_stride == 1 and aligned and rows % 4 == 0 and k_stride % 4 == 0 and tok_axis != 1:
        return 3
    if row_stride == 1 and k_stride != 1:
        return 1
    return 0


_gemm_log = {} if os.environ.get("KANTTS_GEMM_LOG") else None


def gemm(segs, M, N, c, c_is, c_js, bias=None, bias2=None, res=None, r_is=0, r_js=0, rowmask=None, kmask=None,
         a_rowsum=None, alpha=1.0, relu=False, accumulate=False, splitk=1, T=0, drop_p=0.0, drop_seed=0,
         precision=None, c_off=0, groups=1, a_gs=0, b_gs=0, c_gs=0, bias_gs=0, r_gs=0, out_leaky=None, gate=None,
         gate_slope=0.0, res_off=0, z_taps=0, c_tap=0):
    g = GemmArgs()
    assert 1 <= len(segs) <= GEMM_MAX_SEG
    for k, s in enumerate(segs):
        s.a_mode = _staging_mode(s.a or 0, s.a_is, s.a_ks, s.klen, M, s.a_tok_axis, a_gs, s.a_gate)
        s.b_mode = _staging_mode((s.b or 0) + 0, s.b_js, s.b_ks, s.klen, N, 1 if False else (2 if s.b_tok_axis == 2 else 0),
                                 b_gs)
        if s.b_mode == 2 and (s.b_tap % 4 != 0 and s.ntaps > 1):
            s.b_mode = 0
        g.seg[k] = s
    g.nseg, g.M, g.N, g.T = len(segs), int(M), int(N), int(T)
    if _gemm_log is not None:
        s0 = segs[0]
        slow = any(s.a_mode < 2 or s.b_mode < 2 or s.a_inner > 1 or s.a_mul > 1 or s.a_div > 1 or s.a_up > 1 or
                   s.b_inner > 1 or s.b_mul > 1 or s.b_up > 1 for s in segs)
        key = ("generic" if slow else "fast", int(M), int(N), s0.klen, s0.ntaps, int(groups), int(splitk), int(z_taps),
               s0.a_mode, s0.b_mode)
        _gemm_log[key] = _gemm_log.get(key, 0) + 1
    g.c = ptr(c, torch.float32) + 4 * int(c_off)
    g.c_is, g.c_js = int(c_is), int(c_js)
    g.bias, g.bias2 = ptr(bias, torch.float32), ptr(bias2, torch.float32)
    g.res, g.r_is, g.r_js = ptr(res, torch.float32), int(r_is), int(r_js)
    if res is not None and res_off:
        g.res = g.res + 4 * int(res_off)
    g.groups, g.a_gs, g.b_gs, g.c_gs, g.bias_gs, g.r_gs = int(groups), int(a_gs), int(b_gs), int(c_gs), int(bias_gs), int(r_gs)
    if out_leaky is not None:
        g.out_act, g.out_slope = 1, float(out_leaky)
    if gate is not None:
        g.gate = ptr(gate, torch.float32) + 4 * int(c_off)
        g.gate_slope = float(gate_slope)
    g.z_taps, g.c_tap = int(z_taps), int(c_tap)
    g.rowmask = ptr(rowmask)
    g.kmask = ptr(kmask)
    g.a_rowsum = ptr(a_rowsum, torch.float32)
    g.alpha, g.relu, g.accumulate, g.splitk = float(alpha), int(bool(relu)), int(bool(accumulate)), int(splitk)
    g.precision = _precision["gemm"] if precision is None else precision
    g.drop_p, g.drop_seed = float(drop_p), int(drop_seed)
    g.seed_dev = rng_ptr(c.device) if (drop_p > 0 or any(s.a_drop_p > 0 for s in segs)) else None
# ... 781 lines not shown
```

kan-tts_amd/kantts/_hip/ops.py:

```python
import itertools
import os
import weakref
import math

import torch

from . import (E_UNSUPPORTED, act_cast_bf16, bgemm_nt, bgemm_tn, cconv, cconv_wgrad, check, get_precision, conv_c1, conv_n1, conv_wgrad,
               conv_win, gemm, lib, make_seg, ptr, rng_state, stream)
from . import ops_bf16

_seed_counter = itertools.count(1)


def next_seed():
    return (torch.initial_seed() * 0x9E3779B97F4A7C15 + next(_seed_counter) * 0xD1B54A32D192ED03) & ((1 << 63) - 1)


def _c(t):
    return t if t.is_contiguous() else t.contiguous()


def _new_side_stream():
    pr = os.environ.get("KANTTS_SIDE_PRIORITY")
    return torch.cuda.Stream(priority=int(pr)) if pr else torch.cuda.Stream()


class _ZeroPool:

    def __init__(self):
        self.buf = None
        self.off = self.hw = 0
        self.calls = 0
        self.plan = None
        self.log = None

    def enable(self, numel, device):
        have = 0 if (self.buf is None or self.buf.device != torch.device(device)) else self.buf.numel()
        self.buf = torch.zeros(int(have + numel), device=device, dtype=torch.float32)
        self.off = 0
        self.hw = 0

    def reset(self):
        self.calls = 0
        if self.buf is not None:
            self.buf[:min(self.buf.numel(), max(64, (self.hw + 63) // 64 * 64))].zero_()
            self.off = 0

    def take(self, shape, device):
        n = 1
        for d in shape:
            n *= int(d)
        idx = self.calls
        self.calls += 1
        if self.plan is not None:
            v = self.plan.get(idx)
            if v is not None and v.numel() == n and v.device == device:
                return v.view(shape)
        t = self._take(shape, device, n)
        if self.log is not None:
            self.log.append((idx, t.data_ptr(), n))
        return t

    def _take(self, shape, device, n):
        if self.buf is None or self.buf.device != device or self.off + n > self.buf.numel():
            return torch.zeros(shape, device=device, dtype=torch.float32)
        a = (self.off + 63) // 64 * 64
        if a + n > self.buf.numel():
            return torch.zeros(shape, device=device, dtype=torch.float32)
        self.off = a + n
        self.hw = max(self.hw, self.off)
        return self.buf[a:a + n].view(shape)


zero_pool = _ZeroPool()


def gzeros(shape, device):
    return zero_pool.take(tuple(shape), torch.device(device))


def gzeros_like(t):
    return zero_pool.take(tuple(t.shape), t.device)


def _splitk_for(n_out_rows, n_out_cols, k_total):
    tiles = ((n_out_rows + 63) // 64) * ((n_out_cols + 63) // 64)
    ktiles = max(1, (k_total + 31) // 32)
    want = max(1, 512 // max(1, tiles))
    return int(max(1, min(want, ktiles, 64)))


class _WgradOverlap:

    def __init__(self):
        self.enabled = False
        self._stream = None
        self._keep = []
        self._used = False

    def enable(self, on=True, group_wgrads=None):
        from . import deferred_tn

        self.enabled = bool(on)
        side_branch.enabled = bool(on) and os.environ.get("KANTTS_NO_SIDE_BRANCH", "") == ""
        deferred_tn.enabled = bool(on if group_wgrads is None else group_wgrads)
        if not deferred_tn.enabled:
            deferred_tn.flush()

    class _Ctx:
        def __init__(self, owner, keep):
            self.owner, self.keep, self.cm = owner, keep, None

        def __enter__(self):
            o = self.owner
            if not o.enabled:
                return self
            if o._stream is None:
                o._stream = _new_side_stream()
            ev = torch.cuda.Event()
            ev.record(torch.cuda.current_stream())
            o._stream.wait_event(ev)
            self.cm = torch.cuda.stream(o._stream)
            self.cm.__enter__()
            o._keep.extend(t for t in self.keep if t is not None)
            o._used = True
            return self

        def __exit__(self, *exc):
            if self.cm is not None:
                self.cm.__exit__(*exc)
            return False

    def side(self, *keep):
        return _WgradOverlap._Ctx(self, keep)

    def flush_early(self):
        from . import deferred_tn

        if not self.enabled or not (deferred_tn.groups or deferred_tn.copies or deferred_tn.rowsums):
            return
        keep = [k for probs in deferred_tn.groups.values() for q in probs for k in q[6] if k is not None]
        keep += [r[0] for r in deferred_tn.rowsums]
        with self.side(*keep):
            deferred_tn.flush()

    def join(self):
        from . import deferred_tn

        deferred_tn.flush()
        flush_weight_norm_backward()
        side_branch.join()
        side_branch.release()
# ... 718 lines not shown
        sv = ctx.saved_tensors
        lens, whh, out, gates, cst = sv[:5]
        xs, params = list(sv[5:5 + nx]), list(sv[5 + nx:5 + nx + 4 * ndir])
        wbs = list(sv[5 + nx + 4 * ndir:])
        dout = _c(dout)
        dg = torch.empty((ndir, B, T, G), device=dout.device, dtype=torch.float32)
        check(lib().kantts_lstm_bwd(ptr(dout, torch.float32), ptr(whh), ptr(lens), ptr(gates), ptr(cst), ptr(dg), B, T,
                                    H, ndir, 0, prec, stream()), "lstm_bwd")
        needs = ctx.needs_input_grad
        dxs = [None] * nx
        dparams = [None] * (4 * ndir)
        for d in range(ndir):
            dgd = dg[d].view(M, G)
            w_ih = _c(params[4 * d])
            ld = w_ih.shape[1]
            off = 0
            dw_ih = gzeros_like(w_ih)
            db = gzeros((G,), dout.device)
            first = True
            for k, x in enumerate(xs):
                kk = x.shape[-1]
                if ctx.use_b:
                    if needs[3 + k]:
                        first_dir = dxs[k] is None
                        if first_dir:
                            dxs[k] = torch.empty_like(x)
                        if not bgemm_nt([(dgd, G, (wbs[d], off), ld, G, 0)], M, kk, dxs[k], kk, b_kn=True,
                                        res=None if first_dir else dxs[k], ldr=kk):
                            raise RuntimeError("bgemm_nt declined the LSTM input gradient")
                    with wgrad_overlap.side(dgd, x):
                        if not bgemm_tn(dgd, G, x, kk, M, G, kk, (dw_ih, off), ld, 1, db=db if first else None):
                            raise RuntimeError("bgemm_tn declined the LSTM input-weight gradient")
                else:
                    if needs[3 + k]:
                        if dxs[k] is None:
                            dxs[k] = torch.zeros_like(x) if ndir > 1 else torch.empty_like(x)
                        gemm([make_seg(dgd, G, 1, (w_ih, off), 1, ld, G)], M, kk, dxs[k], kk, 1, accumulate=(ndir > 1))
                    gemm([make_seg(dgd, 1, G, x, 1, kk, M)], G, kk, dw_ih, ld, 1, c_off=off, accumulate=True,
                         splitk=_splitk_for(G, kk, M), a_rowsum=db if first else None)
                first = False
                off += kk
            dw_hh = gzeros((G, H), dout.device)
            shift = 1 if d == 1 else -1
            if ctx.use_b:
                with wgrad_overlap.side(dgd, out):
                    if not bgemm_tn(dgd, G, (out, d * H), ndir * H, M, G, H, dw_hh, H, 1, T=T, shift0=shift):
                        raise RuntimeError("bgemm_tn declined the LSTM recurrent-weight gradient")
            else:
                seg = make_seg(dgd, 1, G, (out, d * H), 1, ndir * H, M, b_tok_axis=2, b_shift0=shift)
                gemm([seg], G, H, dw_hh, H, 1, accumulate=True, splitk=_splitk_for(G, H, M), T=T)
            from . import deferred_tn

            dparams[4 * d], dparams[4 * d + 1] = dw_ih, dw_hh
            dparams[4 * d + 2], dparams[4 * d + 3] = db, (deferred_tn.shared_gradient(db) if ctx.use_b else db)
        return (None, None, None, *dxs, *dparams, *([None] * len(wbs)))


def lstm(xs, params, lens_i32=None):
    xs = [xs] if torch.is_tensor(xs) else list(xs)
    ndir = len(params) // 4
    return _LSTM.apply(len(xs), ndir, lens_i32, *xs, *params)


def _ptr_array(tensors):
    import ctypes

    arr = (ctypes.c_void_p * len(tensors))()
    for i, t in enumerate(tensors):
        arr[i] = ptr(t, torch.float32) if t is not None else None
    return arr


class _EmbedSum(torch.autograd.Function):
    @staticmethod
    def forward(ctx, ids, pos, scale, want_scaled, *tables):
        ids = _c(ids)
        if ids.dim() == 2:
            ids = ids.unsqueeze(-1)
        B, T, n = ids.shape
        assert n == len(tables) and ids.dtype == torch.int64
        D = tables[0].shape[1]
        out = torch.empty((B, T, D), device=ids.device, dtype=torch.float32)
        scaled = torch.empty_like(out) if want_scaled else None
        tabs = [_c(t) for t in tables]
        check(lib().kantts_embed_sum_fwd(_ptr_array(tabs), n, ptr(ids), ptr(pos), ptr(out), ptr(scaled), B * T, T, D,
                                         float(scale), stream()), "embed_sum_fwd")
        ctx.save_for_backward(ids)
        ctx.cfg = (scale, [tuple(t.shape) for t in tables])
        if want_scaled and want_scaled != "grad":
            ctx.mark_non_differentiable(scaled)
        return out, scaled

    @staticmethod
    def backward(ctx, dout, d_scaled):
        (ids,) = ctx.saved_tensors
        scale, shapes = ctx.cfg
        if d_scaled is not None:
            dout = d_scaled if dout is None else dout + d_scaled
        dout = _c(dout)
        B, T, n = ids.shape
        D = shapes[0][1]
        dt = [gzeros(s, dout.device) for s in shapes]
        check(lib().kantts_embed_sum_bwd(_ptr_array(dt), n, ptr(ids), ptr(dout, torch.float32), B * T, D, float(scale),
                                         stream()), "embed_sum_bwd")
        return (None, None, None, None, *dt)


def embed_sum(ids, tables, pos=None, scale=1.0, want_scaled=False):
    return _EmbedSum.apply(ids, pos, float(scale), want_scaled if want_scaled == "grad" else bool(want_scaled), *tables)


def lr_index(durations, Tp):
    d = _c(durations)
    B, N = d.shape
    dev = d.device
    idx = torch.empty((B, Tp), device=dev, dtype=torch.int32)
    pos = torch.empty((B, Tp), device=dev, dtype=torch.float32)
    cs = torch.empty((B, N + 1), device=dev, dtype=torch.int32)
    lens = torch.empty((B,), device=dev, dtype=torch.int64)
    if d.dtype == torch.int64:
        di, df = ptr(d), None
    else:
        di, df = None, ptr(d, torch.float32)
    check(lib().kantts_lr_index(di, df, ptr(idx), ptr(pos), ptr(cs), ptr(lens), B, N, Tp, stream()), "lr_index")
    return idx, pos, cs, lens


class _LRGather(torch.autograd.Function):
    @staticmethod
    def forward(ctx, x, idx, cs, valid):
        x = _c(x)
        B, N, C = x.shape
        Tp = idx.shape[1]
        out = torch.empty((B, Tp, C), device=x.device, dtype=torch.float32)
        check(lib().kantts_lr_gather_fwd(ptr(x, torch.float32), ptr(idx), ptr(valid), ptr(out), B, N, Tp, C, C, 0,
                                         stream()), "lr_gather_fwd")
        ctx.save_for_backward(cs, valid)
        ctx.cfg = (B, N, Tp, C)
        return out

    @staticmethod
    def backward(ctx, dout):
        cs, valid = ctx.saved_tensors
        B, N, Tp, C = ctx.cfg
        dout = _c(dout)
        dx = torch.empty((B, N, C), device=dout.device, dtype=torch.float32)
        check(lib().kantts_lr_gather_bwd(ptr(dout, torch.float32), ptr(cs), ptr(valid), ptr(dx), B, N, Tp, C, C, 0, 0,
                                         stream()), "lr_gather_bwd")
        return dx, None, None, None


def lr_gather(x, idx, cs, valid_lens):
    return _LRGather.apply(x, idx, cs, valid_lens)


class _FsmnMemory(torch.autograd.Function):
    @staticmethod
    def forward(ctx, x, w, res, lens, lp):
        x, w = _c(x), _c(w)
        B, T, C = x.shape
        K = w.shape[-1]
        y = torch.empty_like(x)
        r = _c(res) if res is not None else None
        check(lib().kantts_fsmn_dwconv_fwd(ptr(x, torch.float32), ptr(w, torch.float32), ptr(r), ptr(lens), ptr(y), B,
                                           T, C, K, int(lp), stream()), "fsmn_dwconv_fwd")
        ctx.save_for_backward(x, w, lens)
        ctx.cfg = (B, T, C, K, int(lp), res is not None)
        return y

    @staticmethod
    def backward(ctx, dy):
        x, w, lens = ctx.saved_tensors
        B, T, C, K, lp, has_res = ctx.cfg
        dy = _c(dy)
        dx = torch.empty_like(x)
        dw = gzeros_like(w)
        ws_n = int(lib().kantts_fsmn_dwconv_bwd_ws(B, T, C, K))
        ws = torch.empty(max(ws_n, 1), device=dy.device, dtype=torch.float32)
        check(lib().kantts_fsmn_dwconv_bwd(ptr(dy, torch.float32), ptr(x), ptr(w), ptr(lens), ptr(dx), None, None, 0,
                                           B, T, C, K, lp, stream()), "fsmn_dwconv_bwd (dx)")
        with wgrad_overlap.side(dy, x, ws):
            check(lib().kantts_fsmn_dwconv_bwd(ptr(dy, torch.float32), ptr(x), ptr(w), ptr(lens), None, ptr(dw), ptr(ws),
                                               ws_n, B, T, C, K, lp, stream()), "fsmn_dwconv_bwd (dw)")
        return dx, dw, (dy if has_res else None), None, None


def fsmn_memory(x, w, lens_i64, left_pad, res=None):
    return _FsmnMemory.apply(x, w, res, lens_i64, left_pad)


class _MaskedL1(torch.autograd.Function):
    @staticmethod
    def forward(ctx, pred, target, lens):
        pred, target = _c(pred), _c(target)
        if pred.dim() == 2:
            B, T = pred.shape
            C = 1
        else:
            B, T, C = pred.shape
        loss = torch.zeros((), device=pred.device, dtype=torch.float32)
        need_grad = ctx.needs_input_grad[0]
        grad = torch.empty_like(pred) if need_grad else None
        check(lib().kantts_masked_l1(ptr(pred, torch.float32), ptr(target, torch.float32), ptr(lens, torch.int64),
                                     ptr(loss), ptr(grad), B, T, C, stream()), "masked_l1")
        ctx.save_for_backward(grad)
        return loss

    @staticmethod
    def backward(ctx, g):
        (grad,) = ctx.saved_tensors
        return grad * g, None, None


def masked_l1(pred, target, lens_i64):
    return _MaskedL1.apply(pred, target, lens_i64)


class _MaskedL1Many(torch.autograd.Function):

    @staticmethod
    def forward(ctx, spec, *preds):
        from . import LOSS_MAX_TERMS, LossTerm

        n = len(preds)
        assert 1 <= n <= LOSS_MAX_TERMS and len(spec) == n
        terms = (LossTerm * n)()
        grads, keep = [], []
        for k, (p, (target, lens, log1p)) in enumerate(zip(preds, spec)):
            p, target = _c(p), _c(target)
            B, T = p.shape[0], p.shape[1]
            C = 1 if p.dim() == 2 else p.shape[2]
            assert tuple(target.shape) == tuple(p.shape) and p.dtype == torch.float32
            g = torch.empty_like(p) if ctx.needs_input_grad[1 + k] else None
            q = terms[k]
            q.pred, q.lens, q.grad = ptr(p, torch.float32), ptr(lens, torch.int64), ptr(g)
            q.target = ptr(target, torch.int64) if log1p else ptr(target, torch.float32)
            q.B, q.T, q.C, q.target_log1p = int(B), int(T), int(C), int(bool(log1p))
            grads.append(g)
            keep.extend((p, target, lens))
        losses = torch.zeros((LOSS_MAX_TERMS + 1,), device=preds[0].device, dtype=torch.float32)
        check(lib().kantts_masked_l1_many(terms, n, ptr(losses, torch.float32), stream()), "masked_l1_many")
        ctx.grads = grads
        total = losses[LOSS_MAX_TERMS]
        comps = losses[:n]
        ctx.mark_non_differentiable(comps)
        return total, comps

    @staticmethod
    def backward(ctx, g, _gc):
        import ctypes

        live = [t for t in ctx.grads if t is not None and t.numel() > 0]
        if live:
            g = _c(g).reshape(1)
            xs = (ctypes.c_void_p * len(live))(*[ptr(t, torch.float32) for t in live])
            ns = (ctypes.c_longlong * len(live))(*[t.numel() for t in live])
            check(lib().kantts_scale_many(xs, ns, len(live), ptr(g, torch.float32), stream()), "scale_many")
        return (None, *ctx.grads)


def masked_l1_many(terms):
    spec = tuple((t, lens, bool(log1p)) for _, t, lens, log1p in terms)
    return _MaskedL1Many.apply(spec, *[p for p, _, _, _ in terms])


class _ElemLoss(torch.autograd.Function):

    @staticmethod
    def forward(ctx, a, b, target, mode, scale):
        a = _c(a)
        b = _c(b) if b is not None else None
        loss = torch.zeros((), device=a.device, dtype=torch.float32)
        grad = torch.empty_like(a) if ctx.needs_input_grad[0] else None
        check(lib().kantts_elem_loss(ptr(a, torch.float32), ptr(b), float(target), int(mode), float(scale), ptr(loss),
                                     ptr(grad), a.numel(), stream()), "elem_loss")
        ctx.save_for_backward(grad)
        return loss

    @staticmethod
    def backward(ctx, g):
        (grad,) = ctx.saved_tensors
        return (grad * g if grad is not None else None), None, None, None, None


class _ElemLossMany(torch.autograd.Function):

    @staticmethod
    def forward(ctx, n_out, spec, *a_list):
        from . import ELOSS_MAX_TERMS, ElossTerm

        dev = a_list[0].device
        losses = torch.zeros((n_out,), device=dev, dtype=torch.float32)
        grads, keep = [], []
        for s0 in range(0, len(a_list), ELOSS_MAX_TERMS):
            chunk = list(zip(a_list[s0:s0 + ELOSS_MAX_TERMS], spec[s0:s0 + ELOSS_MAX_TERMS]))
            terms = (ElossTerm * len(chunk))()
            for k, (a, (b, target, mode, scale, out)) in enumerate(chunk):
                a = _c(a)
                g = torch.empty_like(a) if ctx.needs_input_grad[2 + s0 + k] else None
                q = terms[k]
                q.a, q.grad, q.n = ptr(a, torch.float32), ptr(g), a.numel()
                if mode == 0:
                    b = _c(b)
                    assert b.numel() == a.numel()
                    q.b = ptr(b, torch.float32)
                    keep.append(b)
# ... 1054 lines not shown
```

kan-tts_amd/kantts/models/sambert/kantts_sambert.py:

```python
import contextlib
import types

import torch
import torch.nn as nn
import torch.nn.functional as F

import os

import kantts._hip as hip_rt
from kantts._hip import ops
from kantts.models.sambert import FFTBlock, PNCABlock, Prenet
from kantts.models.sambert.alignment import b_mas
from kantts.models.sambert.attention import ConvAttention
from kantts.models.sambert.adaptors import LengthRegulator, VarFsmnRnnNARPredictor, VarRnnARPredictor
from kantts.models.sambert.fsmn import FsmnEncoderV2
from kantts.models.sambert.positions import DurSinusoidalPositionEncoder, SinusoidalPositionEncoder
from kantts.models.utils import SeqInfo, get_mask_from_lengths


_BESIDE_PARTS = tuple(x for x in os.environ.get("KANTTS_BESIDE_PARTS", "prenet").split(",") if x)
_PREDICTORS_LATE = not os.environ.get("KANTTS_PREDICTORS_EARLY")
_PLAN_KERNEL = not os.environ.get("KANTTS_NO_PLAN_KERNEL")
_PREDICTORS_AFTER_POSTNET = bool(os.environ.get("KANTTS_PREDICTORS_AFTER_POSTNET"))
_EARLY_FORK = bool(os.environ.get("KANTTS_EARLY_FORK"))
_CATS_EARLY = bool(os.environ.get("KANTTS_CATS_EARLY"))
_FLUSH_EVERY = {"dec": int(os.environ.get("KANTTS_FLUSH_EVERY_DEC", "0")), "enc": int(os.environ.get("KANTTS_FLUSH_EVERY_ENC", "4"))}


class SelfAttentionEncoder(nn.Module):

    def __init__(self, n_layer, d_in, d_model, n_head, d_head, d_inner, dropout, dropout_att, dropout_relu,
                 position_encoder):
        super(SelfAttentionEncoder, self).__init__()
        self.d_in = d_in
        self.d_model = d_model
        self.dropout = dropout
        d_in_lst = [d_in] + [d_model] * (n_layer - 1)
        self.fft = nn.ModuleList([
            FFTBlock(d, d_model, n_head, d_head, d_inner, (3, 1), dropout, dropout_att, dropout_relu)
            for d in d_in_lst
        ])
        self.ln = nn.LayerNorm(d_model, eps=1e-6)
        self.ln._kantts_out_bf16 = False
        self.position_enc = position_encoder

    def forward(self, input, mask=None, return_attns=False, prescaled=False):
        if not prescaled:
            input = self.position_enc(input * self.d_model ** 0.5)
        if self.training and self.dropout > 0:
            input = ops.dropout2_add(input, p1=self.dropout)
        info = SeqInfo.of(mask)
        attns = []
        x = input
        every = _FLUSH_EVERY["enc"] if self.training else 0
        for i, layer in enumerate(self.fft):
            if every and i and i % every == 0:
                x = ops.wgrad_flush_point(x)
            nxt = self.fft[i + 1].slf_attn.layer_norm if i + 1 < len(self.fft) else self.ln
            x, a = layer(x, mask=info, return_attn=return_attns, private_input=i > 0, next_ln=nxt)
            if return_attns:
                attns.append(a)
        x = ops.layer_norm(x, self.ln.weight, self.ln.bias, self.ln.eps, private_input=len(self.fft) > 0)
        return x, attns


class HybridAttentionDecoder(nn.Module):

    def __init__(self, d_in, prenet_units, n_layer, d_model, d_mem, n_head, d_head, d_inner, dropout, dropout_att,
                 dropout_relu, d_out):
        super(HybridAttentionDecoder, self).__init__()
        self.d_model = d_model
        self.dropout = dropout
        self.prenet = Prenet(d_in, prenet_units, d_model)
        self.dec_in_proj = nn.Linear(d_model + d_mem, d_model)
        self.pnca = nn.ModuleList([
            PNCABlock(d_model, d_mem, n_head, d_head, d_inner, (1, 1), dropout, dropout_att, dropout_relu)
            for _ in range(n_layer)
        ])
        self.ln = nn.LayerNorm(d_model, eps=1e-6)
        self.ln._kantts_out_bf16 = False
        self.dec_out_proj = nn.Linear(d_model, d_out)

    def reset_state(self):
        for layer in self.pnca:
            layer.reset_state()

    def forward(self, input, memory, x_band_width, h_band_width, mask=None, return_attns=False, bw_dev=None,
                prenet_out=None):
        info = SeqInfo.of(mask)
        rows = None if info is None else info.mask
        x = prenet_out if prenet_out is not None else self.prenet(input)
        x = ops.linear([memory, x], self.dec_in_proj.weight, self.dec_in_proj.bias, mode="concat", rowmask=rows,
                       alpha=self.d_model ** 0.5)
        if self.training and self.dropout > 0:
            x = ops.dropout2_add(x, p1=self.dropout)
        hkvs = ops.shared_input_linears(memory, [layer.pnca_attn.w_h_kv for layer in self.pnca])
        ax_l, ah_l = [], []
        every = _FLUSH_EVERY["dec"] if self.training else 0
        for i, layer in enumerate(self.pnca):
            if every and i and i % every == 0:
                x = ops.wgrad_flush_point(x)
            x, ax, ah = layer(x, memory, mask=info, x_band_width=x_band_width, h_band_width=h_band_width,
                              return_attn=return_attns, bw_dev=bw_dev, hkv=hkvs[i], private_input=i > 0,
                              next_ln=self.pnca[i + 1].pnca_attn.layer_norm if i + 1 < len(self.pnca) else self.ln)
            if return_attns:
                ax_l.append(ax)
                ah_l.append(ah)
        x = ops.layer_norm(x, self.ln.weight, self.ln.bias, self.ln.eps, private_input=len(self.pnca) > 0)
        x = ops.linear(x, self.dec_out_proj.weight, self.dec_out_proj.bias)
        return x, ax_l, ah_l

    @torch.no_grad()
    def infer(self, step, input, memory, x_band_width, h_band_width, mask=None, return_attns=False, bw_seq=None):
        if return_attns:
            raise NotImplementedError("attention maps of the free-running decode are not materialised")
        info = SeqInfo.of(mask)
        rows = None if info is None else info.mask[:, step].contiguous()
        B = memory.size(0)
        x = self.prenet(input.reshape(B, -1))
        x = ops.linear([memory[:, step, :], x], self.dec_in_proj.weight, self.dec_in_proj.bias, mode="concat",
                       alpha=self.d_model ** 0.5)
        x = x.view(B, 1, -1)
        lens32 = None if info is None else info.lens32
        for layer in self.pnca:
            x = layer.infer_step(step, x, memory, x_band_width, h_band_width, zero_rows=rows, lens32=lens32,
                                 bw_seq=bw_seq)
        x = ops.layer_norm(x, self.ln.weight, self.ln.bias, self.ln.eps)
        x = ops.linear(x, self.dec_out_proj.weight, self.dec_out_proj.bias)
        return x, [], []


class TextFftEncoder(nn.Module):

    def __init__(self, config):
        super(TextFftEncoder, self).__init__()
        d_emb = config["embedding_dim"]
        self.using_byte = False
        self.ling_embedding_grad = False
        if config.get("using_byte", False):
            raise NotImplementedError("byte-index inputs (sambert_16k_MAS_byte.yaml) are outside the hot path")
        self.sy_emb = nn.Embedding(config["sy"], d_emb)
        self.tone_emb = nn.Embedding(config["tone"], d_emb)
        self.syllable_flag_emb = nn.Embedding(config["syllable_flag"], d_emb)
        self.ws_emb = nn.Embedding(config["word_segment"], d_emb)
        max_len = config["max_len"]
        nb_layers = config["encoder_num_layers"]
        nb_heads = config["encoder_num_heads"]
        d_model = config["encoder_num_units"]
        d_head = d_model // nb_heads
        d_inner = config["encoder_ffn_inner_dim"]
        dropout = config["encoder_dropout"]
        dropout_attn = config["encoder_attention_dropout"]
        dropout_relu = config["encoder_relu_dropout"]
        d_proj = config["encoder_projection_units"]
        self.d_model = d_model
        position_enc = SinusoidalPositionEncoder(max_len, d_emb)
        self.ling_enc = SelfAttentionEncoder(nb_layers, d_emb, d_model, nb_heads, d_head, d_inner, dropout,
                                             dropout_attn, dropout_relu, position_enc)
        self.ling_proj = nn.Linear(d_model, d_proj, bias=False)

    def forward(self, inputs_ling, masks=None, return_attns=False):
        T = inputs_ling.size(1)
        pos = self.ling_enc.position_enc.table_for(T, inputs_ling.device)
        x, ling_embedding = ops.embed_sum(
            inputs_ling[:, :, :4],
            [self.sy_emb.weight, self.tone_emb.weight, self.syllable_flag_emb.weight, self.ws_emb.weight],
            pos=pos, scale=self.d_model ** 0.5, want_scaled="grad" if self.ling_embedding_grad else True)
        enc_output, attns = self.ling_enc(x, masks, return_attns, prescaled=True)
        if hasattr(self, "ling_proj"):
            enc_output = ops.linear(enc_output, self.ling_proj.weight, None)
        return enc_output, attns, ling_embedding


class VarianceAdaptor(nn.Module):

    def __init__(self, config):
        super(VarianceAdaptor, self).__init__()
        input_dim = config["encoder_projection_units"] + config["emotion_units"] + config["speaker_units"]
        filter_size = config["predictor_filter_size"]
        fsmn_num_layers = config["predictor_fsmn_num_layers"]
        num_memory_units = config["predictor_num_memory_units"]
        ffn_inner_dim = config["predictor_ffn_inner_dim"]
        dropout = config["predictor_dropout"]
        shift = config["predictor_shift"]
        lstm_units = config["predictor_lstm_units"]
        dur_pred_prenet_units = config["dur_pred_prenet_units"]
        dur_pred_lstm_units = config["dur_pred_lstm_units"]
        self.pitch_predictor = VarFsmnRnnNARPredictor(input_dim, filter_size, fsmn_num_layers, num_memory_units,
                                                      ffn_inner_dim, dropout, shift, lstm_units)
        self.energy_predictor = VarFsmnRnnNARPredictor(input_dim, filter_size, fsmn_num_layers, num_memory_units,
                                                       ffn_inner_dim, dropout, shift, lstm_units)
        self.duration_predictor = VarRnnARPredictor(input_dim, dur_pred_prenet_units, dur_pred_lstm_units)
        self.length_regulator = LengthRegulator(config["outputs_per_step"])
        self.dur_position_encoder = DurSinusoidalPositionEncoder(config["encoder_projection_units"],
                                                                 config["outputs_per_step"])
        self.pitch_emb = nn.Conv1d(1, config["encoder_projection_units"], kernel_size=9, padding=4)
        self.energy_emb = nn.Conv1d(1, config["encoder_projection_units"], kernel_size=9, padding=4)

    def pitch_energy_embedding(self, pitch, energy):
        return (ops.conv_cl(pitch.unsqueeze(-1).contiguous(), self.pitch_emb.weight, self.pitch_emb.bias, pad=4)
                + ops.conv_cl(energy.unsqueeze(-1).contiguous(), self.energy_emb.weight, self.energy_emb.bias, pad=4))

    def position_term(self, plan, out_info):
        idx, pos, cs, LR_length_rounded, Tp, max_len = plan[:6]
        t = torch.arange(Tp, device=pos.device)[None, :]
        limit = (LR_length_rounded if out_info is None else out_info.lens64).clamp(max=max_len)
        pos = torch.where(t < limit[:, None], pos, torch.zeros_like(pos))
        return self.dur_position_encoder.from_positions(pos)

    def forward(self, inputs_text_embedding, inputs_emo_embedding, inputs_spk_embedding, masks=None,
                output_masks=None, duration_targets=None, pitch_targets=None, energy_targets=None, max_out_len=None,
                teacher_plan=None):
        info = SeqInfo.of(masks)
        out_info = SeqInfo.of(output_masks)

        def vp_inputs():
            return torch.cat([inputs_text_embedding, inputs_spk_embedding, inputs_emo_embedding], dim=-1)
        teacher = (self.training and duration_targets is not None and pitch_targets is not None
                   and energy_targets is not None)
        lens_keep = None if info is None else (info.lens64, info.mask)
        late = teacher and _PREDICTORS_LATE
        cats_late = late and duration_targets is not None and not _CATS_EARLY
        variance_predictor_inputs = None if cats_late else vp_inputs()
        self.deferred = None
        pitch_predictions = energy_predictions = None
        if not late:
            with ops.side_branch.fork(variance_predictor_inputs, *(lens_keep or ())) if teacher else contextlib.nullcontext():
                pitch_predictions = self.pitch_predictor(variance_predictor_inputs, info)
                energy_predictions = self.energy_predictor(variance_predictor_inputs, info)
        pitch_src = pitch_targets if pitch_targets is not None else pitch_predictions
        energy_src = energy_targets if energy_targets is not None else energy_predictions
        if teacher_plan is not None and "pe_emb" in teacher_plan:
            aug = inputs_text_embedding + teacher_plan["pe_emb"]
        else:
            aug = (inputs_text_embedding
                   + ops.conv_cl(pitch_src.unsqueeze(-1).contiguous(), self.pitch_emb.weight, self.pitch_emb.bias, pad=4)
                   + ops.conv_cl(energy_src.unsqueeze(-1).contiguous(), self.energy_emb.weight, self.energy_emb.bias, pad=4))
        duration_predictor_cond = (None if cats_late
                                   else torch.cat([aug, inputs_spk_embedding, inputs_emo_embedding], dim=-1))
        if duration_targets is not None:
            prev = (teacher_plan["prev"] if teacher_plan is not None
                    else torch.log(F.pad(duration_targets[:, :-1].float(), (1, 0)) + 1).unsqueeze(-1))
            log_duration_predictions = None
            if late:
                ready = ops.side_branch.mark() if _EARLY_FORK else None

                def deferred():
                    with ops.side_branch.fork(variance_predictor_inputs, duration_predictor_cond, prev, aug,
                                              inputs_text_embedding, inputs_spk_embedding, inputs_emo_embedding,
                                              *(lens_keep or ()), after=ready):
                        vpi = variance_predictor_inputs if variance_predictor_inputs is not None else vp_inputs()
                        cond = (duration_predictor_cond if duration_predictor_cond is not None
                                else torch.cat([aug, inputs_spk_embedding, inputs_emo_embedding], dim=-1))
                        p_ = self.pitch_predictor(vpi, info)
                        e_ = self.energy_predictor(vpi, info)
                        d_, _ = self.duration_predictor(prev, cond, masks=info)
                    return d_, p_, e_

                self.deferred = deferred
            else:
                with ops.side_branch.fork(duration_predictor_cond, prev) if teacher else contextlib.nullcontext():
                    log_duration_predictions, _ = self.duration_predictor(prev, duration_predictor_cond, masks=info)
            durations = duration_targets
        else:
            log_duration_predictions = self.duration_predictor.infer(duration_predictor_cond, masks=info)
            durations = torch.exp(log_duration_predictions) - 1
        if teacher_plan is not None:
            plan, pos_enc = teacher_plan["lr_plan"], teacher_plan["pos_enc"]
        else:
            plan = self.length_regulator.index(durations, max_len=max_out_len)
            pos_enc = self.position_term(plan, out_info)
        LR_length_rounded = plan[3]
        LR_text_outputs, _ = self.length_regulator(aug, durations, masks=out_info, plan=plan)
        if teacher_plan is not None and "LR_emo" in teacher_plan:
            LR_emo_outputs, LR_spk_outputs = teacher_plan["LR_emo"], teacher_plan["LR_spk"]
        else:
            LR_emo_outputs, _ = self.length_regulator(inputs_emo_embedding, durations, masks=out_info, plan=plan)
            LR_spk_outputs, _ = self.length_regulator(inputs_spk_embedding, durations, masks=out_info, plan=plan)
        LR_text_outputs = LR_text_outputs + pos_enc
        return (LR_text_outputs, LR_emo_outputs, LR_spk_outputs, LR_length_rounded, log_duration_predictions,
                pitch_predictions, energy_predictions)


class MelPNCADecoder(nn.Module):

    def teacher_input(self, target, L):
        B = target.size(0)
        input = torch.zeros((B, L, self.d_mel), device=target.device, dtype=target.dtype)
        input[:, 1:, :] = target[:, self.r - 1:: self.r, :][:, : L - 1, :]
        return input

    def __init__(self, config):
        super(MelPNCADecoder, self).__init__()
        prenet_units = config["decoder_prenet_units"]
        nb_layers = config["decoder_num_layers"]
        nb_heads = config["decoder_num_heads"]
        d_model = config["decoder_num_units"]
        d_head = d_model // nb_heads
        d_inner = config["decoder_ffn_inner_dim"]
        dropout = config["decoder_dropout"]
        dropout_attn = config["decoder_attention_dropout"]
        dropout_relu = config["decoder_relu_dropout"]
        outputs_per_step = config["outputs_per_step"]
        d_mem = (config["encoder_projection_units"] * outputs_per_step + config["emotion_units"]
                 + config["speaker_units"])
        d_mel = config["num_mels"]
        self.d_mel = d_mel
        self.r = outputs_per_step
        self.nb_layers = nb_layers
        self.mel_dec = HybridAttentionDecoder(d_mel, prenet_units, nb_layers, d_model, d_mem, nb_heads, d_head,
                                              d_inner, dropout, dropout_attn, dropout_relu, d_mel * outputs_per_step)
        self.decode_mode = "loop"
        self._decode_cache = None
        self._decode_kernel = None

    def forward(self, memory, x_band_width, h_band_width, target=None, mask=None, return_attns=False, bw_dev=None,
                teacher_input=None, teacher_prenet=None):
        if target is None:
            return self._free_run(memory, x_band_width, h_band_width, mask, bw_dev)
        self.mel_dec.reset_state()
        input = teacher_input if teacher_input is not None else self.teacher_input(target, memory.size(1))
        return self.mel_dec(input, memory, x_band_width, h_band_width, mask=mask, return_attns=return_attns,
                            bw_dev=bw_dev, prenet_out=teacher_prenet)


    @torch.no_grad()
    def _free_run(self, memory, x_band_width, h_band_width, mask, bw_seq=None):
        B, L = memory.size(0), memory.size(1)
        if self.decode_mode == "kernel":
            from kantts.models.sambert.ar_kernels import DecoderKernel
            from kantts.models.utils import SeqInfo as _SeqInfo

            host_bw = not torch.is_tensor(x_band_width) and not torch.is_tensor(h_band_width)
            bw_max = int(x_band_width) if host_bw else -1
            if host_bw and int(h_band_width) == bw_max and DecoderKernel.eligible(self.mel_dec, self.d_mel, bw_max):
                if self._decode_kernel is None:
                    self._decode_kernel = DecoderKernel(self.mel_dec, self.d_mel)
                info = _SeqInfo.of(mask)
                lens32 = None if info is None else info.lens32.clamp(max=L)
                return self._decode_kernel.run(memory, lens32, bw_seq, bw_max), [], []
        if (self.decode_mode in ("graph", "fused", "kernel") and memory.is_cuda) or self.decode_mode == "fused":
            from kantts.models.sambert.decode_graph import DecodeGraphCache
            from kantts.models.utils import SeqInfo as _SeqInfo

            if self._decode_cache is None:
                self._decode_cache = DecodeGraphCache()
            info = _SeqInfo.of(mask)
            lens32 = info.lens32 if info is not None else torch.full((B,), L, device=memory.device, dtype=torch.int32)
            bw = bw_seq if bw_seq is not None else torch.full((B,), int(x_band_width), device=memory.device,
                                                              dtype=torch.int32)
            Lp = (L + 15) // 16 * 16 if self.decode_mode != "fused" else L
            if Lp != L:
                memory = F.pad(memory, (0, 0, 0, Lp - L))
            fr = self._decode_cache.get(self.mel_dec, self.d_mel, self.r, B, Lp, memory.device)
            fr.load(memory, lens32.clamp(max=L), bw)
            return fr.run(graph=(self.decode_mode != "fused"))[:, :L].clone(), [], []
        self.mel_dec.reset_state()
        memory = memory.contiguous()
        out = torch.empty((B, L, self.d_mel * self.r), device=memory.device, dtype=torch.float32)
        frame = torch.zeros((B, 1, self.d_mel), device=memory.device, dtype=torch.float32)
        for step in range(L):
            o, _, _ = self.mel_dec.infer(step, frame, memory, x_band_width, h_band_width, mask=mask, bw_seq=bw_seq)
            out[:, step, :] = o[:, 0, :]
            frame = o[:, :, -self.d_mel:]
        return out, [], []


class PostNet(nn.Module):

    def __init__(self, config):
        super(PostNet, self).__init__()
        self.filter_size = config["postnet_filter_size"]
        self.fsmn_num_layers = config["postnet_fsmn_num_layers"]
        self.num_memory_units = config["postnet_num_memory_units"]
        self.ffn_inner_dim = config["postnet_ffn_inner_dim"]
        self.dropout = config["postnet_dropout"]
        self.shift = config["postnet_shift"]
        self.lstm_units = config["postnet_lstm_units"]
        self.num_mels = config["num_mels"]
        self.fsmn = FsmnEncoderV2(self.filter_size, self.fsmn_num_layers, self.num_mels, self.num_memory_units,
                                  self.ffn_inner_dim, self.dropout, self.shift)
        self.lstm = nn.LSTM(self.num_memory_units, self.lstm_units, num_layers=1, batch_first=True)
        self.fc = nn.Linear(self.lstm_units, self.num_mels)

    def forward(self, x, mask=None, res=None, zero_rows=None):
        h = self.fsmn(x, mask)
        h = ops.lstm(h, [self.lstm.weight_ih_l0, self.lstm.weight_hh_l0, self.lstm.bias_ih_l0, self.lstm.bias_hh_l0])
        return ops.linear(h, self.fc.weight, self.fc.bias, res=res, rowmask=zero_rows)


def band_width_of(duration_targets, input_lengths, r):
    T = duration_targets.size(1)
    valid = torch.arange(T, device=duration_targets.device)[None, :] < input_lengths[:, None]
    return int(float((duration_targets * valid).max()) / r + 0.5)


def average_frame_feat(pitch, durs):
    ends = torch.cumsum(durs, dim=1).long()
    starts = F.pad(ends[:, :-1], (1, 0))
    n_form = pitch.size(1)
    e = ends[:, None, :].expand(-1, n_form, -1)
    s = starts[:, None, :].expand(-1, n_form, -1)
    count_ps = F.pad(torch.cumsum(pitch != 0.0, dim=2), (1, 0))
    value_ps = F.pad(torch.cumsum(pitch, dim=2), (1, 0))
    sums = (torch.gather(value_ps, 2, e) - torch.gather(value_ps, 2, s)).float()
    counts = (torch.gather(count_ps, 2, e) - torch.gather(count_ps, 2, s)).float()
    return torch.where(counts == 0.0, counts, sums / counts)


class KanTtsSAMBERT(nn.Module):

    def __init__(self, config):
        super(KanTtsSAMBERT, self).__init__()
        self.text_encoder = TextFftEncoder(config)
        self.se_enable = config.get("SE", False)
        if not self.se_enable:
            self.spk_tokenizer = nn.Embedding(config["speaker"], config["speaker_units"])
        self.emo_tokenizer = nn.Embedding(config["emotion"], config["emotion_units"])
        self.variance_adaptor = VarianceAdaptor(config)
        self.mel_decoder = MelPNCADecoder(config)
        self.mel_postnet = PostNet(config)
        self.inline_teacher_plan = False
        self.MAS = False
        if config.get("MAS", False):
            self.MAS = True
            self.text_encoder.ling_embedding_grad = True
            self.align_attention = ConvAttention(n_mel_channels=config["num_mels"],
                                                 n_text_channels=config["embedding_dim"],
                                                 n_att_channels=config["num_mels"])
        self.fp_enable = config.get("FP", False)
        if self.fp_enable:
            raise NotImplementedError("filled-pause predictor is outside the hot path")
        self.return_attns = False
        self.device_band_width = False
        self.band_width_bound = None
        self.infer_front_fp32 = True

    def get_lfr_mask_from_lengths(self, lengths, max_len):
        r = self.mel_decoder.r
        return get_mask_from_lengths((lengths + r - 1) // r, max_len=max_len // r)

    def binarize_attention_parallel(self, attn, in_lens, out_lens):
        with torch.no_grad():
            return b_mas(attn, in_lens, out_lens, width=1)

    @torch.no_grad()
    def teacher_forced_plan(self, in_info, output_lengths, mel_targets, duration_targets):
        r = self.mel_decoder.r
        va = self.variance_adaptor
        max_out_len = mel_targets.size(1)
        out_info = SeqInfo(output_lengths, max_out_len)
        lr_plan = va.length_regulator.index(duration_targets, max_len=max_out_len)
        Tp, max_len = lr_plan[4], lr_plan[5]
        lr_plan = tuple(lr_plan) + (torch.clamp(out_info.lens64, max=max_len),)
        plan = {"out_info": out_info, "lr_plan": lr_plan, "pos_enc": va.position_term(lr_plan, out_info),
                "prev": torch.log(F.pad(duration_targets[:, :-1].float(), (1, 0)) + 1).unsqueeze(-1),
                "lfr_info": SeqInfo((output_lengths + r - 1) // r, Tp // r),
                "bw_val": duration_targets.float().masked_fill(in_info.mask, 0).max() / r + 0.5,
                "dec_input": self.mel_decoder.teacher_input(mel_targets, Tp // r)}
        if self.device_band_width:
            plan["bw_dev"] = plan["bw_val"].to(torch.int32).reshape(1)
        return plan

    @torch.no_grad()
    def teacher_forced_plan_fused(self, input_lengths, T_in, output_lengths, mel_targets, duration_targets):
        from kantts._hip import teacher_plan

        r = self.mel_decoder.r
        va = self.variance_adaptor
        max_out_len = mel_targets.size(1)
        idx, pos, cs, lens, Tp, max_len = va.length_regulator.index(duration_targets, max_len=max_out_len)
        o = teacher_plan(input_lengths.to(torch.int64).contiguous(), output_lengths.to(torch.int64).contiguous(),
                         duration_targets.contiguous(), mel_targets.contiguous(), pos,
                         va.dur_position_encoder.inv_timescales.detach(), Tp, max_len, r)
        in_info = SeqInfo.from_parts(o["in_mask"], o["in_l64"], o["in_l32"])
        plan = {"out_info": SeqInfo.from_parts(o["out_mask"], o["out_l64"], o["out_l32"]),
                "lr_plan": (idx, pos, cs, lens, Tp, max_len, o["valid"]), "pos_enc": o["pos_enc"], "prev": o["prev"],
                "lfr_info": SeqInfo.from_parts(o["lfr_mask"], o["lfr_l64"], o["lfr_l32"]), "bw_val": o["bw_val"],
                "dec_input": o["dec_input"]}
        if self.device_band_width:
            plan["bw_dev"] = o["bw_dev"]
        return in_info, plan

    def _embed_emo_spk(self, inputs_emotion, inputs_speaker):
        (emo_hid, _) = ops.embed_sum(inputs_emotion, [self.emo_tokenizer.weight])
        if self.se_enable:
            spk_hid = inputs_speaker.to(torch.float32)
        else:
            (spk_hid, _) = ops.embed_sum(inputs_speaker, [self.spk_tokenizer.weight])
        return emo_hid, spk_hid

    def _beside_encoder(self, in_info, output_lengths, mel_targets, duration_targets, inputs_emotion, inputs_speaker,
                        pitch_targets, energy_targets, base_plan=None):
        plan = base_plan if base_plan is not None else self.teacher_forced_plan(in_info, output_lengths, mel_targets,
                                                                                duration_targets)
        parts = _BESIDE_PARTS
        if "emb" in parts:
            emo_hid, spk_hid = self._embed_emo_spk(inputs_emotion, inputs_speaker)
            lr = self.variance_adaptor.length_regulator
            plan["emo_hid"], plan["spk_hid"] = emo_hid, spk_hid
            plan["LR_emo"], _ = lr(emo_hid, duration_targets, masks=plan["out_info"], plan=plan["lr_plan"])
            plan["LR_spk"], _ = lr(spk_hid, duration_targets, masks=plan["out_info"], plan=plan["lr_plan"])
        if "pe" in parts:
            plan["pe_emb"] = self.variance_adaptor.pitch_energy_embedding(pitch_targets, energy_targets)
        if "prenet" in parts:
            plan["dec_prenet"] = self.mel_decoder.mel_dec.prenet(plan["dec_input"])
        return plan

    _TOKEN_SIDE_FIELDS = ("batch_size", "is_training", "tplan", "memory", "bw_int", "bw_dev", "x_band_width", "h_band_width",
                          "lfr_info", "out_info", "enc_sla_attn_lst", "LR_length_rounded", "log_duration_predictions",
                          "pitch_predictions", "energy_predictions", "duration_targets", "pitch_targets", "energy_targets",
                          "inter_lengths", "LR_text_outputs", "LR_emo_outputs", "LR_spk_outputs", "ling_embedding",
                          "attn_soft", "attn_hard", "attn_logprob")

    def _token_side(self, inputs_ling, inputs_emotion, inputs_speaker, input_lengths, output_lengths=None,
                    mel_targets=None, duration_targets=None, pitch_targets=None, energy_targets=None, attn_priors=None):
        batch_size = inputs_ling.size(0)
        r = self.mel_decoder.r
        T_in = inputs_ling.size(1)
        is_training = mel_targets is not None
        tplan = base_plan = in_info = None
        teacher = (is_training and not self.MAS and not getattr(self, "inline_teacher_plan", False)
                   and output_lengths is not None and duration_targets is not None and pitch_targets is not None
                   and energy_targets is not None)
        if (teacher and _PLAN_KERNEL and duration_targets.dtype == torch.int64 and mel_targets.dtype == torch.float32
                and mel_targets.dim() == 3 and inputs_ling.numel() > 0):
            in_info, base_plan = self.teacher_forced_plan_fused(input_lengths, T_in, output_lengths, mel_targets,
                                                                duration_targets)
        if in_info is None:
            in_info = SeqInfo(input_lengths, T_in)
        front = hip_rt.precision_scope("fp32" if (not is_training and self.infer_front_fp32) else None)
        with front:
            if teacher:
                (text_hid, enc_sla_attn_lst, ling_embedding), tplan = ops.run_beside(
                    lambda: self.text_encoder(inputs_ling, in_info, self.return_attns),
                    lambda: self._beside_encoder(in_info, output_lengths, mel_targets, duration_targets, inputs_emotion,
                                                 inputs_speaker, pitch_targets, energy_targets, base_plan=base_plan),
                    side_inputs=(output_lengths, mel_targets, duration_targets, in_info.mask, in_info.lens64, inputs_emotion,
                                 inputs_speaker, pitch_targets, energy_targets))
            else:
                text_hid, enc_sla_attn_lst, ling_embedding = self.text_encoder(inputs_ling, in_info, self.return_attns)
            text_hid = ops.wgrad_flush_point(text_hid)
            inter_lengths = input_lengths
            attn_soft = attn_hard = attn_logprob = None
            if self.MAS and is_training:
                attn_soft, attn_logprob = self.align_attention.forward_cl(mel_targets, ling_embedding, input_lengths,
                                                                          attn_priors)
                attn_hard = self.binarize_attention_parallel(attn_soft, input_lengths, output_lengths)
                duration_targets = attn_hard.sum(2)[:, 0, :]
                pitch_targets = average_frame_feat(pitch_targets.unsqueeze(1), duration_targets).squeeze(1)
                energy_targets = average_frame_feat(energy_targets.unsqueeze(1), duration_targets).squeeze(1)
                pad = (mel_targets.size(1) - output_lengths).to(duration_targets.dtype)
                duration_targets.scatter_(1, input_lengths.view(-1, 1), pad.view(-1, 1))
            if tplan is not None and "emo_hid" in tplan:
                emo_hid, spk_hid = tplan["emo_hid"], tplan["spk_hid"]
            else:
                emo_hid, spk_hid = self._embed_emo_spk(inputs_emotion, inputs_speaker)
            out_info = None
            max_out_len = None
            if output_lengths is not None:
                max_out_len = mel_targets.size(1)
                out_info = tplan["out_info"] if tplan is not None else SeqInfo(output_lengths, max_out_len)
            (LR_text_outputs, LR_emo_outputs, LR_spk_outputs, LR_length_rounded, log_duration_predictions,
             pitch_predictions, energy_predictions) = self.variance_adaptor(
                text_hid, emo_hid, spk_hid, masks=in_info, output_masks=out_info, duration_targets=duration_targets,
                pitch_targets=pitch_targets, energy_targets=energy_targets, max_out_len=max_out_len, teacher_plan=tplan)
        Tp = LR_text_outputs.size(1)
        if tplan is not None:
            lfr_info = tplan["lfr_info"]
        elif output_lengths is not None:
            lfr_info = SeqInfo((output_lengths + r - 1) // r, Tp // r)
        else:
            out_info = SeqInfo(LR_length_rounded, Tp)
            lfr_info = SeqInfo((LR_length_rounded + r - 1) // r, Tp // r)
        d_t, d_s, d_e = text_hid.shape[-1], spk_hid.shape[-1], emo_hid.shape[-1]
        memory = torch.cat([
            LR_text_outputs.reshape(batch_size, -1, r * d_t),
            LR_spk_outputs.reshape(batch_size, -1, r * d_s)[:, :, :d_s],
            LR_emo_outputs.reshape(batch_size, -1, r * d_e)[:, :, :d_e],
        ], dim=-1)
        if tplan is not None:
            bw_val = tplan["bw_val"]
        elif duration_targets is not None:
            bw_val = duration_targets.float().masked_fill(in_info.mask, 0).max() / r + 0.5
        else:
            bw_val = (torch.exp(log_duration_predictions) - 1).max() / r + 0.5
        bw_dev = None
        if duration_targets is None:
            pred = (torch.exp(log_duration_predictions) - 1)
            bw_dev = (pred.max(dim=1).values / r + 0.5).to(torch.int32).contiguous()
        elif mel_targets is None:
            bw_dev = (duration_targets.float().masked_fill(in_info.mask, 0).max(dim=1).values / r + 0.5).to(
                torch.int32).contiguous()
        if self.device_band_width and duration_targets is not None and mel_targets is not None:
            bw_dev = tplan["bw_dev"] if (tplan is not None and "bw_dev" in tplan) else bw_val.to(torch.int32).reshape(1)
            x_band_width = h_band_width = bw_dev
            bw_int = 0
        else:
            x_band_width = h_band_width = bw_int = int(bw_val)
        here = locals()
        return types.SimpleNamespace(**{k: here[k] for k in self._TOKEN_SIDE_FIELDS})

    def forward(self, inputs_ling, inputs_emotion, inputs_speaker, input_lengths, output_lengths=None,
                mel_targets=None, duration_targets=None, pitch_targets=None, energy_targets=None, attn_priors=None,
                fp_label=None):
        ts = self._token_side(inputs_ling, inputs_emotion, inputs_speaker, input_lengths, output_lengths, mel_targets,
                              duration_targets, pitch_targets, energy_targets, attn_priors)
        batch_size, tplan, memory, bw_int, bw_dev = ts.batch_size, ts.tplan, ts.memory, ts.bw_int, ts.bw_dev
        lfr_info, out_info = ts.lfr_info, ts.out_info
        from kantts._hip import ops_bf16

        bound_before = ops_bf16.BAND_BOUND["max"]
        ops_bf16.BAND_BOUND["max"] = self.band_width_bound if (self.device_band_width and mel_targets is not None) else None
        try:
            dec_outputs, pnca_x_attn_lst, pnca_h_attn_lst = self.mel_decoder(
                memory, bw_int, bw_int, target=mel_targets, mask=lfr_info, return_attns=self.return_attns, bw_dev=bw_dev,
                teacher_input=None if tplan is None else tplan["dec_input"],
                teacher_prenet=None if tplan is None else tplan.get("dec_prenet"))
        finally:
            ops_bf16.BAND_BOUND["max"] = bound_before
        dec_outputs = dec_outputs.reshape(batch_size, -1, self.mel_decoder.d_mel)
        rows = out_info.mask
        if rows.size(1) != dec_outputs.size(1):
            rows = F.pad(rows, (0, dec_outputs.size(1) - rows.size(1)), value=True)
        dec_outputs = ops.wgrad_flush_point(dec_outputs.masked_fill(rows.unsqueeze(-1), 0))
        post_info = out_info if out_info.mask.size(1) == dec_outputs.size(1) else SeqInfo(out_info.lens64,
                                                                                         dec_outputs.size(1))
        deferred = getattr(self.variance_adaptor, "deferred", None)
        if deferred is not None and not _PREDICTORS_AFTER_POSTNET:
            ts.log_duration_predictions, ts.pitch_predictions, ts.energy_predictions = deferred()
        postnet_outputs = self.mel_postnet(dec_outputs, post_info, res=dec_outputs, zero_rows=post_info.mask)
        if deferred is not None and _PREDICTORS_AFTER_POSTNET:
            ts.log_duration_predictions, ts.pitch_predictions, ts.energy_predictions = deferred()
        self.variance_adaptor.deferred = None
        ops.side_branch.join()
        return self._result(ts, mel_targets, dec_outputs, postnet_outputs, pnca_x_attn_lst, pnca_h_attn_lst)

    def _result(self, ts, mel_targets, dec_outputs, postnet_outputs, pnca_x_attn_lst, pnca_h_attn_lst):
        res = {
            "x_band_width": ts.x_band_width,
            "h_band_width": ts.h_band_width,
            "enc_slf_attn_lst": ts.enc_sla_attn_lst,
            "pnca_x_attn_lst": pnca_x_attn_lst,
            "pnca_h_attn_lst": pnca_h_attn_lst,
            "dec_outputs": dec_outputs,
            "postnet_outputs": postnet_outputs,
            "LR_length_rounded": ts.LR_length_rounded,
            "log_duration_predictions": ts.log_duration_predictions,
            "pitch_predictions": ts.pitch_predictions,
            "energy_predictions": ts.energy_predictions,
            "duration_targets": ts.duration_targets,
            "pitch_targets": ts.pitch_targets,
            "energy_targets": ts.energy_targets,
            "fp_predictions": None,
            "valid_inter_lengths": ts.inter_lengths,
        }
        if ts.bw_dev is not None and ts.bw_dev.numel() == ts.batch_size and mel_targets is None:
            res["band_width_per_sequence"] = ts.bw_dev
        res["LR_text_outputs"] = ts.LR_text_outputs
        res["LR_emo_outputs"] = ts.LR_emo_outputs
        res["LR_spk_outputs"] = ts.LR_spk_outputs
        res["ling_embedding"] = ts.ling_embedding
        if self.MAS and ts.is_training:
            res["attn_soft"] = ts.attn_soft
            res["attn_hard"] = ts.attn_hard
            res["attn_logprob"] = ts.attn_logprob
        return res


class KanTtsTextsyBERT(nn.Module):

    def __init__(self, config):
        super(KanTtsTextsyBERT, self).__init__()
        self.text_encoder = TextFftEncoder(config)
        delattr(self.text_encoder, "ling_proj")
        self.fc = nn.Linear(self.text_encoder.d_model, config["sy"])

    def forward(self, inputs_ling, input_lengths):
        info = SeqInfo(input_lengths, inputs_ling.size(1))
        text_hid, attns, _ = self.text_encoder(inputs_ling, info, return_attns=False)
        return {"logits": ops.linear(text_hid, self.fc.weight, self.fc.bias), "enc_slf_attn_lst": attns}
```

kan-tts_amd/kantts/train/optim.py:

```python
import torch
import torch.distributed as dist

from kantts._hip import ops


class ParamArena:
    def __init__(self, module, bf16_shadow=False):
        self.module = module
        self.params = [p for p in module.parameters() if p.requires_grad]
        if not self.params:
            raise ValueError("module has no trainable parameters")
        dev = self.params[0].device
        self.align = 64
        self.offsets = []
        off = 0
        for p in self.params:
            self.offsets.append(off)
            off += (p.numel() + self.align - 1) // self.align * self.align
        self.numel = off
        self.flat = torch.zeros(self.numel, device=dev, dtype=torch.float32)
        self.grad = torch.zeros(self.numel, device=dev, dtype=torch.float32)
        with torch.no_grad():
            for p, o in zip(self.params, self.offsets):
                view = self.flat[o:o + p.numel()].view(p.shape)
                view.copy_(p.data)
                p.data = view
        self.grad_views = [self.grad[o:o + p.numel()].view(p.shape) for p, o in zip(self.params, self.offsets)]
        self._zero_cache = {}
        self.world_size = 1
        self.force_exchange = False
        self.bucket_ready = None
        self.capture_stream = None
        self.n_buckets = 4
        self.flat_bf16 = None
        self._weights_version = 0
        self._shadow_stale = False
        self._wn_table = None
        self._direct, self._plan = None, None
        if bf16_shadow:
            self._build_shadow()

    @property
    def shadow_stale(self):
        return self._shadow_stale

    @shadow_stale.setter
    def shadow_stale(self, value):
        self._shadow_stale = bool(value)
        if value:
            self._weights_version += 1
            ops.weights_epoch[0] += 1

    def enable_direct_grads(self):
        if self._direct is None and not __import__("os").environ.get("KANTTS_NO_DIRECT_GRADS"):
            self._direct = "record"

    def _direct_begin(self):
        if self._direct == "record":
            ops.zero_pool.plan, ops.zero_pool.log = None, []
        elif self._direct == "on":
            self.grad.zero_()
            ops.zero_pool.plan, ops.zero_pool.log = self._plan, None

    def _direct_end(self):
        if self._direct == "record":
            self._direct_finish_recording()
        elif self._direct == "on" and ops.zero_pool.plan is self._plan:
            ops.zero_pool.plan = None

    def _direct_finish_recording(self):
        log, ops.zero_pool.log = ops.zero_pool.log, None
        if not log:
            return
        where = {ptr_: (idx, n) for idx, ptr_, n in log}
        plan = {}
        for i, p in enumerate(self.params):
            g = p.grad
            if g is None or not g.is_contiguous() or g.dtype != torch.float32:
                continue
            hit = where.get(g.data_ptr())
            if hit is not None and hit[1] == p.numel():
                plan[hit[0]] = self.grad_views[i]
        self._plan = plan
        self._direct = "on"

    def build_weight_norm_images(self):
        import torch.nn as nn

        index = {id(p): i for i, p in enumerate(self.params)}
        rows_tab, layers = [], []
        w_off = wf_off = wd_off = row0 = 0
        al = self.align
        for m in self.module.modules():
            g, v = getattr(m, "weight_g", None), getattr(m, "weight_v", None)
            if g is None or v is None or id(g) not in index or id(v) not in index:
                continue
            if isinstance(m, (nn.ConvTranspose1d, nn.ConvTranspose2d)):
                continue
            shape = tuple(v.shape[:3]) if (v.dim() == 4 and v.shape[3] == 1) else tuple(v.shape)
            if len(shape) != 3 or shape[1] % 4:
                continue
            cout, cin, k = shape
            groups = int(getattr(m, "groups", 1))
            n = cout * cin * k
            img = cin % 8 == 0 and (cout // groups) % 8 == 0
            rows_tab.append([self.offsets[index[id(v)]], self.offsets[index[id(g)]], w_off, wf_off if img else -1,
                             wd_off if img else -1, cout | (cin << 32), k | (groups << 32), row0])
            layers.append((m, w_off, wf_off if img else -1, wd_off if img else -1, (k, cout, cin), groups))
            pad = (n + al - 1) // al * al
            w_off += pad
            if img:
                wf_off += pad
                wd_off += pad
            row0 += (cout + 7) // 8
        if not layers:
            return 0
        dev = self.flat.device
        self._wn_tiles = []
        self._wn_pending = []
        self._wn_extra = []
        self._wn_seen = set()
        self._wn_defer = False
        self._index_of = index
        self._wn_w = torch.zeros(max(w_off, 8), device=dev, dtype=torch.float32)
        self._wn_wf = torch.zeros(max(wf_off, 8), device=dev, dtype=torch.bfloat16)
        self._wn_wd = torch.zeros(max(wd_off, 8), device=dev, dtype=torch.bfloat16)
        self._wn_table = torch.tensor(rows_tab, dtype=torch.int64, device=dev)
        self._wn_rows = row0
        self._wn_version = -1
        self._wn_params = [q for m, *_ in layers for q in (m.weight_v, m.weight_g)]
        self._wn_sig = None
        import weakref

        ref = weakref.ref(self)
        for m, wo, fo, do, (k, cout, cin), groups in layers:
            n = k * cout * cin
            m._kantts_wn = (ref, self._wn_w[wo:wo + n].view(k, cout, cin),
                            None if fo < 0 else self._wn_wf[fo:fo + n].view(k, cout, cin),
                            None if do < 0 else self._wn_wd[do:do + n].view(k, groups, cin, cout // groups), groups,
                            len(self._wn_tiles))
            self._wn_tiles.append((cout + 7) // 8)
        def _pre(m, a):
            self.refresh_weight_norm_images()

        self.module.register_forward_pre_hook(_pre)
        self.module.register_load_state_dict_post_hook(lambda m, keys: self.mark_shadow_stale())
        return len(layers)

    def grad_slot(self, p):
        i = self._index_of[id(p)]
        return self.grad[self.offsets[i]:self.offsets[i] + p.numel()].view(p.shape)

    def defer_weight_norm_backward(self, entry, dw):
        if not self._wn_defer or self._wn_table is None:
            return False
        entry = int(entry)
        if not self._wn_pending and not self._wn_extra:
            ops.wn_pending_arenas.append(self)
        if entry in self._wn_seen:
            self._wn_extra.append((entry, dw))
            return "extra"
        self._wn_seen.add(entry)
        self._wn_pending.append((entry, dw))
        return True

    def flush_weight_norm_backward(self):
        import ctypes

        from kantts._hip import WN_BWD_MAX, WnBwdArgs, check, lib, ptr, stream

        pend, self._wn_pending = self._wn_pending, []
        extra, self._wn_extra = self._wn_extra, []
        for s0 in range(0, len(pend), WN_BWD_MAX):
            chunk = pend[s0:s0 + WN_BWD_MAX]
            a = WnBwdArgs()
            t = 0
            for l, (entry, dw) in enumerate(chunk):
                a.dw[l], a.desc[l], a.tile0[l] = ptr(dw, torch.float32), entry, t
                t += self._wn_tiles[entry]
            a.tile0[len(chunk)] = t
            a.nl = len(chunk)
            check(lib().kantts_weight_norm_table_bwd(ptr(self.flat, torch.float32), ptr(self.grad, torch.float32),
                                                     ptr(self._wn_table), ctypes.byref(a), stream()), "weight_norm_table_bwd")
        for entry, _ in pend:
            for q in self._wn_params[2 * entry:2 * entry + 2]:
                slot = self.grad_slot(q)
                if q.grad is not None and q.grad.data_ptr() != slot.data_ptr():
                    q.grad = slot
        for entry, dw in extra:
            v, g = self._wn_params[2 * entry:2 * entry + 2]
            v3 = v.detach().squeeze(-1) if v.dim() == 4 else v.detach()
            v3 = v3 if v3.is_contiguous() else v3.contiguous()
            cout, cin, k = v3.shape
            dv, dg = torch.empty_like(v3), torch.empty_like(g)
            check(lib().kantts_weight_norm_strided_bwd(ptr(dw, torch.float32), ptr(v3), ptr(g.detach()), ptr(dv), ptr(dg), cout,
                                                       cin, k, cin, 1, cout * cin, stream()), "weight_norm_strided_bwd")
            for q, d in ((v, dv), (g, dg)):
                slot = self.grad_slot(q)
                if q.grad is not None and q.grad.data_ptr() != slot.data_ptr():
                    q.grad = slot
                slot.add_(d.view(slot.shape))

    def weight_norm_images_fresh(self):
        return self._wn_table is not None and self._wn_version == self._weights_version

    def refresh_weight_norm_images(self, force=False):
        import os

        if self._wn_table is None or (os.environ.get("KANTTS_NO_WEIGHT_NORM_TABLE") and not force):
            return False
        sig = sum(q._version for q in self._wn_params)
        if sig != self._wn_sig:
            self._wn_sig = sig
            self._weights_version += 1
            ops.weights_epoch[0] += 1
        if not force and self._wn_version == self._weights_version:
            return False
        from kantts._hip import check, lib, ptr, stream

        check(lib().kantts_weight_norm_table(ptr(self.flat, torch.float32), ptr(self._wn_w, torch.float32),
                                             ptr(self._wn_wf, torch.bfloat16), ptr(self._wn_wd, torch.bfloat16),
                                             ptr(self._wn_table), int(self._wn_table.shape[0]), int(self._wn_rows),
                                             stream()), "weight_norm_table")
        self._wn_version = self._weights_version
        return True

    def _build_shadow(self):
        dev = self.flat.device
        self.flat_bf16 = torch.zeros(self.numel, device=dev, dtype=torch.bfloat16)
        rows, off = [], 0
        for p, o in zip(self.params, self.offsets):
            p._kantts_bf16 = self.flat_bf16[o:o + p.numel()].view(p.shape)
            if p.dim() == 3 and p.shape[2] > 1:
                n, cin, kt = p.shape
                rows.append((o, off, n, cin, kt, p, "_kantts_bf16_tap"))
                off += (p.numel() + self.align - 1) // self.align * self.align
        self.tap_bf16 = torch.zeros(max(off, 8), device=dev, dtype=torch.bfloat16)
        self._tap_blocks = 1
        tab = []
        for o, to, n, cin, kt, p, attr in rows:
            setattr(p, attr, self.tap_bf16[to:to + p.numel()].view(kt, n, cin))
            tab.append([o, to, n | (cin << 32), kt])
            self._tap_blocks = max(self._tap_blocks, min(64, (n * cin * kt + 1023) // 1024))
        self._tap_table = torch.tensor(tab, dtype=torch.int64, device=dev) if tab else None
        ftab, foff = [], 0
        self._frag_blocks = 1

        def image(p, src_off, R, K, sr, sk, attr, n_img=1):
            nonlocal foff
            base = foff
            for t in range(n_img):
                ftab.append([src_off + t, base + t * R * K, sr, sk, R | (K << 32)])
            foff += (n_img * R * K + self.align - 1) // self.align * self.align
            self._frag_blocks = max(self._frag_blocks, min(64, (R * K + 2047) // 2048))
            return (attr, p, base, n_img * R * K)

        views = []
        for p, o in zip(self.params, self.offsets):
            role = getattr(p, "_kantts_ffn_role", None)
            if role == "w1" and p.dim() == 3 and p.shape[0] == 1024 and p.shape[1] == 128 and p.shape[2] % 2 == 1:
                F_, C_, KT_ = p.shape
                views.append(image(p, o, F_, C_, C_ * KT_, KT_, "_kantts_frag", n_img=KT_))
                views.append(image(p, o, C_, F_, KT_, C_ * KT_, "_kantts_fragT", n_img=KT_))
            elif role == "w2" and p.dim() == 3 and p.shape[0] == 128 and p.shape[1] == 1024 and p.shape[2] == 1:
                N_, F_, _ = p.shape
                views.append(image(p, o, N_, F_, F_, 1, "_kantts_frag"))
                views.append(image(p, o, F_, N_, 1, F_, "_kantts_fragT"))
            elif role == "lin" and p.dim() == 2 and p.shape[0] % 16 == 0 and p.shape[1] % 32 == 0:
                N_, K_ = p.shape
                views.append(image(p, o, N_, K_, K_, 1, "_kantts_frag"))
                if N_ % 32 == 0 and K_ % 16 == 0:
                    views.append(image(p, o, K_, N_, 1, K_, "_kantts_fragT"))
        self.frag_bf16 = torch.zeros(max(foff, 8), device=dev, dtype=torch.bfloat16)
        for attr, p, base, n in views:
            setattr(p, attr, self.frag_bf16[base:base + n])
        self._frag_table = torch.tensor(ftab, dtype=torch.int64, device=dev) if ftab else None
        import weakref

        ref = weakref.ref(self)
        for p in self.params:
            p._kantts_arena = ref
        self.shadow_stale = True
        self.refresh_shadow()
        self.module.register_forward_pre_hook(lambda m, a: self.refresh_shadow(only_if_bf16=True))
        self.module.register_load_state_dict_post_hook(lambda m, keys: self.mark_shadow_stale())

    def mark_shadow_stale(self):
        self.shadow_stale = True

    def refresh_shadow(self, only_if_bf16=False):
        if self.flat_bf16 is None:
            return
        from kantts._hip import check, get_precision, lib, ptr, stream

        if only_if_bf16 and get_precision() != "bf16":
            return
        self.shadow_stale = False

        check(lib().kantts_cast_f32_bf16(ptr(self.flat, torch.float32), ptr(self.flat_bf16, torch.bfloat16), self.numel,
                                         stream()), "cast_f32_bf16")
        if self._tap_table is not None:
            check(lib().kantts_tapmajor_bf16(ptr(self.flat, torch.float32), ptr(self.tap_bf16, torch.bfloat16),
                                             ptr(self._tap_table), int(self._tap_table.shape[0]), int(self._tap_blocks),
                                             stream()), "tapmajor_bf16")
        if self._frag_table is not None:
            check(lib().kantts_fragmajor_bf16(ptr(self.flat, torch.float32), ptr(self.frag_bf16, torch.bfloat16),
                                              ptr(self._frag_table), int(self._frag_table.shape[0]),
                                              int(self._frag_blocks), stream()), "fragmajor_bf16")

    def view_of(self, flat, i):
        p = self.params[i]
        return flat[self.offsets[i]:self.offsets[i] + p.numel()].view(p.shape)

    def enable_data_parallel(self, n_buckets=4, overlap=True):
        if not dist.is_initialized():
            raise RuntimeError("torch.distributed is not initialised")
        self.world_size = dist.get_world_size()
        self.n_buckets = n_buckets
        dist.broadcast(self.flat, src=0)
        self.shadow_stale = True
        self.refresh_shadow(only_if_bf16=True)
        self.force_exchange = bool(__import__("os").environ.get("KANTTS_DP_FORCE")) and self.world_size == 1
        self.overlap = bool(overlap) and (self.world_size > 1 or self.force_exchange)
        if self.overlap:
            self._build_buckets()

    def _build_buckets(self):
        n = self.numel
        step = (n + self.n_buckets - 1) // self.n_buckets
        self.buckets = []
        self.bucket_of = [0] * len(self.params)
        cur = None
        for i, o in enumerate(self.offsets):
            if cur is None:
                cur = {"lo": o, "hi": o, "params": [], "pending": 0, "handle": None}
            cur["params"].append(i)
            self.bucket_of[i] = len(self.buckets)
            end = self.offsets[i + 1] if i + 1 < len(self.offsets) else n
            cur["hi"] = end
            if cur["hi"] - cur["lo"] >= step and len(self.buckets) + 1 < self.n_buckets:
                self.buckets.append(cur)
                cur = None
        if cur is not None:
            self.buckets.append(cur)
        if self.buckets:
            self.buckets[0]["lo"], self.buckets[-1]["hi"] = 0, n
        assert all(x["hi"] == y["lo"] for x, y in zip(self.buckets, self.buckets[1:])) and (
            not self.buckets or (self.buckets[0]["lo"] == 0 and self.buckets[-1]["hi"] == n))
        assert all(0 <= self.bucket_of[i] < len(self.buckets) for i in range(len(self.params)))
        self._active = False
        if not getattr(self, "_hooked", False):
            for i, p in enumerate(self.params):
                p.register_post_accumulate_grad_hook(lambda _p, i=i: self._on_grad(i))
            self._hooked = True

    def begin_step(self):
        if self._wn_table is not None and not __import__("os").environ.get("KANTTS_NO_WEIGHT_NORM_TABLE"):
            self._wn_defer = True
            self._wn_seen.clear()
        if self._direct is not None:
            self._direct_begin()
        if not getattr(self, "overlap", False):
            return
        for b in self.buckets:
            b["pending"], b["handle"] = len(b["params"]), None
        self._active = True

    def _on_grad(self, i):
        if not self._active:
            return
        b = self.buckets[self.bucket_of[i]]
        b["pending"] -= 1
        if b["pending"] == 0:
            self._launch_bucket(b)

    def _launch_bucket(self, b):
        cap = self.capture_stream
        if cap is not None and torch.cuda.current_stream() != cap:
            if torch.cuda.is_current_stream_capturing():
                cap.wait_stream(torch.cuda.current_stream())
            with torch.cuda.stream(cap):
                return self._launch_bucket_on_current_stream(b)
        return self._launch_bucket_on_current_stream(b)

    def _launch_bucket_on_current_stream(self, b):
        if self.bucket_ready is not None:
            ops.join_capturing_side_streams()
        elif torch.cuda.is_available() and self.grad.is_cuda:
            cur = torch.cuda.current_stream()
            for st in ops.helper_streams():
                if st != cur:
                    cur.wait_stream(st)
        ops.wgrad_overlap.join()
        dst, src = [], []
        for i in b["params"]:
            p = self.params[i]
            g = p.grad
            if g is None:
                self.grad_views[i].zero_()
            elif g.data_ptr() != self.grad_views[i].data_ptr():
                dst.append(self.grad_views[i])
                src.append(self._out_of_arena(g))
        if dst:
            torch._foreach_copy_(dst, src)
        if self.bucket_ready is not None:
            b["handle"] = "captured"
            self.bucket_ready(b)
            return
        b["handle"] = self.exchange(b)

    def exchange(self, b):
        return dist.all_reduce(self.grad[b["lo"]:b["hi"]], op=dist.ReduceOp.SUM, async_op=True)

    def finish_reduce(self):
        for b in self.buckets:
            if b["handle"] is None:
                self._launch_bucket(b)
        for b in self.buckets:
            if self.bucket_ready is None:
                b["handle"].wait()
            b["handle"] = None
        self._active = False
        self.grad.mul_(1.0 / self.world_size)
        return self.grad

    def _out_of_arena(self, g):
        base = self.grad.data_ptr()
        if base <= g.data_ptr() < base + 4 * self.numel:
            return g.clone()
        return g

    def pack_grads(self):
        if self._direct is not None:
            self._direct_end()
        dst, src = [], []
        for i, p in enumerate(self.params):
            g = p.grad
            if g is None:
                z = self._zero_cache.get(tuple(p.shape))
                if z is None:
                    z = torch.zeros(p.shape, device=self.grad.device, dtype=torch.float32)
                    self._zero_cache[tuple(p.shape)] = z
                g = z
            elif g.data_ptr() == self.grad_views[i].data_ptr():
                continue
            dst.append(self.grad_views[i])
            src.append(g)
        if dst:
            src = [self._out_of_arena(g) for g in src]
            torch._foreach_copy_(dst, src)
        return self.grad
# ... 120 lines not shown
```

Baseline: 2.760 million mel-frames/s.

## Fuse length-regulator gather with LFR memory build and merge shadow refresh kernels

Measured after the change: 2.739 million mel-frames/s. No clear change (-0.7%).

```diff
diff --git a/include/kantts_hip.h b/include/kantts_hip.h
--- a/include/kantts_hip.h
+++ b/include/kantts_hip.h
@@ -146,6 +146,36 @@
                          int Tp, int C, int ldo, int out_col_offset, void* stream);
 int kantts_lr_gather_bwd(const float* dout, const int32_t* cs, const int64_t* valid_lens, float* dx, int B, int N,
                          int Tp, int C, int ldo, int out_col_offset, int accumulate, void* stream);
+
+typedef struct kantts_lr_memory_args {
+  const float* text;
+  const float* add1;
+  const float* add2;
+  const int32_t* idx;
+  const int64_t* valid;
+  const float* pos_enc;
+  const float* spk;
+  const float* emo;
+  float* aug;
+  float* lr_text;
+  float* lr_spk;
+  float* lr_emo;
+  float* memory;
+  int32_t B, N, Tp, r, d_t, d_s, d_e, side_tokens;
+} kantts_lr_memory_args;
+int kantts_lr_memory_fwd(const kantts_lr_memory_args* args, void* stream);
+
+typedef struct kantts_lr_memory_bwd_args {
+  const float* d_memory;
+  const float* d_aug_in;
+  const int32_t* cs;
+  const int64_t* valid;
+  float* d_text;
+  float* d_spk;
+  float* d_emo;
+  int32_t B, N, Tp, r, d_t, d_s, d_e, side_tokens;
+} kantts_lr_memory_bwd_args;
+int kantts_lr_memory_bwd(const kantts_lr_memory_bwd_args* args, void* stream);
 
 int kantts_fsmn_dwconv_fwd(const float* x, const float* w, const float* res, const int64_t* lens, float* y, int B,
                            int T, int C, int K, int left_pad, void* stream);
@@ -587,6 +617,18 @@
 int kantts_fragmajor_bf16(const float* src, void* dst_bf16, const kantts_fragmajor_desc* table_dev, int ndesc,
                           int blocks_per_desc, void* stream);
 
+typedef struct kantts_refresh_images_args {
+  const float* src;
+  void* flat_dst;
+  void* tap_dst;
+  void* frag_dst;
+  const kantts_tapmajor_desc* tap_table;
+  const kantts_fragmajor_desc* frag_table;
+  int64_t n;
+  int32_t ntap, tap_blocks, nfrag, frag_blocks;
+} kantts_refresh_images_args;
+int kantts_refresh_images(const kantts_refresh_images_args* args, void* stream);
+
 int kantts_ln128_fwd(const float* x, const float* gamma, const float* beta, void* y, int y_bf16, float* mean, float* rstd,
                      int M, float eps, void* stream);
 int kantts_ln128_bwd(const void* dy, int dy_bf16, const float* x, const float* gamma, const float* mean, const float* rstd,
diff --git a/kan-tts_amd/csrc/ffn_pair.hip b/kan-tts_amd/csrc/ffn_pair.hip
--- a/kan-tts_amd/csrc/ffn_pair.hip
+++ b/kan-tts_amd/csrc/ffn_pair.hip
@@ -60,42 +60,10 @@
   KANTTS_CHECK_LAUNCH();
 }
 
+#include "fragmajor_body.inc"
 __global__ __launch_bounds__(256) void fragmajor_bf16_kernel(const float* __restrict__ src, __bf16* __restrict__ dst,
                                                             const kantts_fragmajor_desc* __restrict__ tab) {
-  const kantts_fragmajor_desc d = tab[blockIdx.y];
-  const long long total = (long long)d.R * d.K;
-  const unsigned KB = (unsigned)d.K >> 5;
-  const bool fast = total < (1ll << 31) && (d.dst_off & 7) == 0;
-  if (fast) {
-    const unsigned total8 = (unsigned)(total >> 3);
-    const bool contig = d.sk == 1 && ((d.src_off | d.sr) & 3) == 0;
-    for (unsigned o8 = blockIdx.x * blockDim.x + threadIdx.x; o8 < total8; o8 += gridDim.x * blockDim.x) {
-      const unsigned lane = o8 & 63u, blk = o8 >> 6;
-      const unsigned rb = blk / KB, kb = blk - rb * KB;
-      const long long r = (long long)rb * 16 + (lane & 15u), k0 = (long long)kb * 32 + (lane >> 4) * 8;
-      const float* sp = src + d.src_off + r * d.sr + k0 * d.sk;
-      float v[8];
-      if (contig) {
-        const float4 a = reinterpret_cast<const float4*>(sp)[0], b = reinterpret_cast<const float4*>(sp)[1];
-        v[0] = a.x, v[1] = a.y, v[2] = a.z, v[3] = a.w, v[4] = b.x, v[5] = b.y, v[6] = b.z, v[7] = b.w;
-      } else {
-#pragma unroll
-        for (int e = 0; e < 8; ++e) v[e] = sp[(long long)e * d.sk];
-      }
-      bf16x8 o;
-#pragma unroll
-      for (int e = 0; e < 8; ++e) o[e] = (__bf16)v[e];
-      *reinterpret_cast<bf16x8*>(dst + d.dst_off + (long long)o8 * 8) = o;
-    }
-    return;
-  }
-  for (long long o = (long long)blockIdx.x * blockDim.x + threadIdx.x; o < total; o += (long long)gridDim.x * blockDim.x) {
-    const int e = (int)(o & 7), lane = (int)((o >> 3) & 63);
-    const long long blk = o >> 9;
-    const int kb = (int)(blk % KB), rb = (int)(blk / KB);
-    const long long r = (long long)rb * 16 + (lane & 15), k = (long long)kb * 32 + (lane >> 4) * 8 + e;
-    dst[d.dst_off + o] = (__bf16)src[d.src_off + r * d.sr + k * d.sk];
-  }
+  fragmajor_bf16_body(src, dst, tab[blockIdx.y], blockIdx.x, gridDim.x);
 }
 
 extern "C" int kantts_fragmajor_bf16(const float* src, void* dst, const kantts_fragmajor_desc* table_dev, int ndesc,
diff --git a/kan-tts_amd/csrc/fragmajor_body.inc b/kan-tts_amd/csrc/fragmajor_body.inc
--- /dev/null
+++ b/kan-tts_amd/csrc/fragmajor_body.inc
@@ -0,0 +1,36 @@
+__device__ __forceinline__ void fragmajor_bf16_body(const float* __restrict__ src, __bf16* __restrict__ dst,
+                                                    const kantts_fragmajor_desc d, unsigned bx, unsigned gx) {
+  const long long total = (long long)d.R * d.K;
+  const unsigned KB = (unsigned)d.K >> 5;
+  const bool fast = total < (1ll << 31) && (d.dst_off & 7) == 0;
+  if (fast) {
+    const unsigned total8 = (unsigned)(total >> 3);
+    const bool contig = d.sk == 1 && ((d.src_off | d.sr) & 3) == 0;
+    for (unsigned o8 = bx * blockDim.x + threadIdx.x; o8 < total8; o8 += gx * blockDim.x) {
+      const unsigned lane = o8 & 63u, blk = o8 >> 6;
+      const unsigned rb = blk / KB, kb = blk - rb * KB;
+      const long long r = (long long)rb * 16 + (lane & 15u), k0 = (long long)kb * 32 + (lane >> 4) * 8;
+      const float* sp = src + d.src_off + r * d.sr + k0 * d.sk;
+      float v[8];
+      if (contig) {
+        const float4 a = reinterpret_cast<const float4*>(sp)[0], b = reinterpret_cast<const float4*>(sp)[1];
+        v[0] = a.x, v[1] = a.y, v[2] = a.z, v[3] = a.w, v[4] = b.x, v[5] = b.y, v[6] = b.z, v[7] = b.w;
+      } else {
+#pragma unroll
+        for (int e = 0; e < 8; ++e) v[e] = sp[(long long)e * d.sk];
+      }
+      bf16x8 o;
+#pragma unroll
+      for (int e = 0; e < 8; ++e) o[e] = (__bf16)v[e];
+      *reinterpret_cast<bf16x8*>(dst + d.dst_off + (long long)o8 * 8) = o;
+    }
+    return;
+  }
+  for (long long o = (long long)bx * blockDim.x + threadIdx.x; o < total; o += (long long)gx * blockDim.x) {
+    const int e = (int)(o & 7), lane = (int)((o >> 3) & 63);
+    const long long blk = o >> 9;
+    const int kb = (int)(blk % KB), rb = (int)(blk / KB);
+    const long long r = (long long)rb * 16 + (lane & 15), k = (long long)kb * 32 + (lane >> 4) * 8 + e;
+    dst[d.dst_off + o] = (__bf16)src[d.src_off + r * d.sr + k * d.sk];
+  }
+}
diff --git a/kan-tts_amd/csrc/gemm_bf16.hip b/kan-tts_amd/csrc/gemm_bf16.hip
--- a/kan-tts_amd/csrc/gemm_bf16.hip
+++ b/kan-tts_amd/csrc/gemm_bf16.hip
@@ -496,12 +496,17 @@
   return bg_tn_launch(ga, (hipStream_t)stream);
 }
 
-__global__ __launch_bounds__(256) void cast_bf16_kernel(const float* __restrict__ src, __bf16* __restrict__ dst, long long n8) {
-  const long long i = (long long)blockIdx.x * blockDim.x + threadIdx.x;
+__device__ __forceinline__ void cast_bf16_body(const float* __restrict__ src, __bf16* __restrict__ dst, long long n8,
+                                               unsigned bx) {
+  const long long i = (long long)bx * blockDim.x + threadIdx.x;
   if (i >= n8) return;
   const float4 a = reinterpret_cast<const float4*>(src)[2 * i], b = reinterpret_cast<const float4*>(src)[2 * i + 1];
   u32x4 w = {bg_pack2(a.x, a.y), bg_pack2(a.z, a.w), bg_pack2(b.x, b.y), bg_pack2(b.z, b.w)};
   reinterpret_cast<u32x4*>(dst)[i] = w;
+}
+
+__global__ __launch_bounds__(256) void cast_bf16_kernel(const float* __restrict__ src, __bf16* __restrict__ dst, long long n8) {
+  cast_bf16_body(src, dst, n8, blockIdx.x);
 }
 
 extern "C" int kantts_cast_f32_bf16(const float* src, void* dst, long long n, void* stream) {
@@ -513,16 +518,20 @@
   KANTTS_CHECK_LAUNCH();
 }
 
-__global__ __launch_bounds__(256) void tapmajor_bf16_kernel(const float* __restrict__ src, __bf16* __restrict__ dst,
-                                                           const kantts_tapmajor_desc* __restrict__ tab) {
-  const kantts_tapmajor_desc d = tab[blockIdx.y];
+__device__ __forceinline__ void tapmajor_bf16_body(const float* __restrict__ src, __bf16* __restrict__ dst,
+                                                   const kantts_tapmajor_desc d, unsigned bx, unsigned gx) {
   const long long total = (long long)d.N * d.Cin * d.KT;
-  for (long long o = (long long)blockIdx.x * blockDim.x + threadIdx.x; o < total; o += (long long)gridDim.x * blockDim.x) {
+  for (long long o = (long long)bx * blockDim.x + threadIdx.x; o < total; o += (long long)gx * blockDim.x) {
     const int c = (int)(o % d.Cin);
     const long long q = o / d.Cin;
     const int n = (int)(q % d.N), tap = (int)(q / d.N);
     dst[d.dst_off + o] = (__bf16)src[d.src_off + ((long long)n * d.Cin + c) * d.KT + tap];
   }
+}
+
+__global__ __launch_bounds__(256) void tapmajor_bf16_kernel(const float* __restrict__ src, __bf16* __restrict__ dst,
+                                                           const kantts_tapmajor_desc* __restrict__ tab) {
+  tapmajor_bf16_body(src, dst, tab[blockIdx.y], blockIdx.x, gridDim.x);
 }
 
 extern "C" int kantts_tapmajor_bf16(const float* src, void* dst, const kantts_tapmajor_desc* table_dev, int ndesc,
@@ -531,6 +540,42 @@
   if (ndesc == 0) return KANTTS_OK;
   hipLaunchKernelGGL(tapmajor_bf16_kernel, dim3(blocks_per_desc, ndesc), dim3(256), 0, (hipStream_t)stream, src,
                      reinterpret_cast<__bf16*>(dst), table_dev);
+  KANTTS_CHECK_LAUNCH();
+}
+
+#include "fragmajor_body.inc"
+__global__ __launch_bounds__(256) void refresh_images_kernel(const kantts_refresh_images_args g) {
+  unsigned id = blockIdx.x;
+  const unsigned nf = (unsigned)g.nfrag * (unsigned)g.frag_blocks, nt = (unsigned)g.ntap * (unsigned)g.tap_blocks;
+  if (id < nf) {
+    fragmajor_bf16_body(g.src, reinterpret_cast<__bf16*>(g.frag_dst), g.frag_table[id / g.frag_blocks], id % g.frag_blocks,
+                        g.frag_blocks);
+    return;
+  }
+  id -= nf;
+  if (id < nt) {
+    tapmajor_bf16_body(g.src, reinterpret_cast<__bf16*>(g.tap_dst), g.tap_table[id / g.tap_blocks], id % g.tap_blocks,
+                       g.tap_blocks);
+    return;
+  }
+  cast_bf16_body(g.src, reinterpret_cast<__bf16*>(g.flat_dst), g.n / 8, id - nt);
+}
+
+extern "C" int kantts_refresh_images(const kantts_refresh_images_args* gp, void* stream) {
+  if (!gp) return KANTTS_E_BADARG;
+  const kantts_refresh_images_args& g = *gp;
+  if (!g.src || !g.flat_dst || g.n < 0 || (g.n & 7) || !bg_aligned16(g.src) || !bg_aligned16(g.flat_dst)) return KANTTS_E_BADARG;
+  if (g.ntap < 0 || g.nfrag < 0 || (g.ntap && (!g.tap_dst || !g.tap_table || g.tap_blocks < 1)) ||
+      (g.nfrag && (!g.frag_dst || !g.frag_table || g.frag_blocks < 1)))
+    return KANTTS_E_BADARG;
+  const long long blocks = (long long)g.nfrag * (g.nfrag ? g.frag_blocks : 0) + (long long)g.ntap * (g.ntap ? g.tap_blocks : 0) +
+                           kantts_cdiv(g.n / 8, 256);
+  if (blocks == 0) return KANTTS_OK;
+  if (blocks > 0x7fffffffll) return KANTTS_E_BADARG;
+  kantts_refresh_images_args a = g;
+  if (!a.ntap) a.tap_blocks = 1;
+  if (!a.nfrag) a.frag_blocks = 1;
+  hipLaunchKernelGGL(refresh_images_kernel, dim3((unsigned)blocks), dim3(256), 0, (hipStream_t)stream, a);
   KANTTS_CHECK_LAUNCH();
 }
 
diff --git a/kan-tts_amd/csrc/seq.hip b/kan-tts_amd/csrc/seq.hip
--- a/kan-tts_amd/csrc/seq.hip
+++ b/kan-tts_amd/csrc/seq.hip
@@ -229,6 +229,137 @@
   if (total == 0) return KANTTS_OK;
   hipLaunchKernelGGL(lr_gather_bwd_kernel, dim3(kantts_cdiv(total, 256)), dim3(256), 0, (hipStream_t)stream, dout, cs,
                      valid_lens, dx, B, N, Tp, C, ldo, out_col_offset, accumulate);
+  KANTTS_CHECK_LAUNCH();
+}
+
+template <typename I>
+__global__ __launch_bounds__(256) void lr_memory_fwd_kernel(const kantts_lr_memory_args g) {
+  const I nA = (I)g.B * g.N * g.d_t;
+  const int W = g.d_t + g.d_s + g.d_e, L = g.Tp / g.r, ldm = g.r * g.d_t + g.d_s + g.d_e;
+  const I total = nA + (I)g.B * g.Tp * W;
+  const I i = (I)blockIdx.x * blockDim.x + threadIdx.x;
+  if (i >= total) return;
+  if (i < nA) {
+    float v = g.text[i];
+    if (g.add1) v = v + g.add1[i];
+    if (g.add2) v = v + g.add2[i];
+    g.aug[i] = v;
+    return;
+  }
+  const I k = i - nA;
+  const int c = (int)(k % (I)W);
+  const I btq = k / (I)W;
+  const int t = (int)(btq % (I)g.Tp), b = (int)(btq / (I)g.Tp);
+  const long long bt = (long long)btq;
+  const int id = g.idx[bt];
+  const bool covered = id >= 0 && (!g.valid || t < (int)g.valid[b]);
+  const long long tok = (long long)b * g.N + (covered ? id : 0);
+  float* mrow = g.memory + ((long long)b * L + t / g.r) * ldm;
+  const int f = t % g.r;
+  if (c < g.d_t) {
+    float v = 0.f;
+    if (covered) {
+      v = g.text[tok * g.d_t + c];
+      if (g.add1) v = v + g.add1[tok * g.d_t + c];
+      if (g.add2) v = v + g.add2[tok * g.d_t + c];
+    }
+    if (g.pos_enc) v = v + g.pos_enc[bt * g.d_t + c];
+    g.lr_text[bt * g.d_t + c] = v;
+    mrow[f * g.d_t + c] = v;
+  } else if (c < g.d_t + g.d_s) {
+    const int cc = c - g.d_t;
+    float v;
+    if (g.side_tokens) {
+      v = covered ? g.spk[tok * g.d_s + cc] : 0.f;
+      g.lr_spk[bt * g.d_s + cc] = v;
+    } else {
+      v = g.spk[bt * g.d_s + cc];
+    }
+    if (f == 0) mrow[g.r * g.d_t + cc] = v;
+  } else {
+    const int cc = c - g.d_t - g.d_s;
+    float v;
+    if (g.side_tokens) {
+      v = covered ? g.emo[tok * g.d_e + cc] : 0.f;
+      g.lr_emo[bt * g.d_e + cc] = v;
+    } else {
+      v = g.emo[bt * g.d_e + cc];
+    }
+    if (f == 0) mrow[g.r * g.d_t + g.d_s + cc] = v;
+  }
+}
+
+template <typename I>
+__global__ __launch_bounds__(256) void lr_memory_bwd_kernel(const kantts_lr_memory_bwd_args g) {
+  const int Wt = g.d_t + (g.side_tokens ? g.d_s + g.d_e : 0), Wf = g.side_tokens ? 0 : g.d_s + g.d_e;
+  const int L = g.Tp / g.r, ldm = g.r * g.d_t + g.d_s + g.d_e;
+  const I nA = (I)g.B * g.N * Wt, total = nA + (I)g.B * g.Tp * Wf;
+  const I i = (I)blockIdx.x * blockDim.x + threadIdx.x;
+  if (i >= total) return;
+  if (i < nA) {
+    const int c = (int)(i % (I)Wt);
+    const I bnq = i / (I)Wt;
+    const int n = (int)(bnq % (I)g.N), b = (int)(bnq / (I)g.N);
+    const long long bn = (long long)bnq;
+    int s = g.cs[(long long)b * (g.N + 1) + n], e = g.cs[(long long)b * (g.N + 1) + n + 1];
+    if (e > g.Tp) e = g.Tp;
+    if (g.valid && e > (int)g.valid[b]) e = (int)g.valid[b];
+    const float* mb = g.d_memory + (long long)b * L * ldm;
+    float acc = 0.f;
+    if (c < g.d_t) {
+      for (int t = s; t < e; ++t) acc += mb[(long long)(t / g.r) * ldm + (t % g.r) * g.d_t + c];
+      if (g.d_aug_in) acc = acc + g.d_aug_in[bn * g.d_t + c];
+      g.d_text[bn * g.d_t + c] = acc;
+    } else {
+      const bool is_spk = c < g.d_t + g.d_s;
+      const int col = g.r * g.d_t + (c - g.d_t);
+      for (int t = (s + g.r - 1) / g.r * g.r; t < e; t += g.r) acc += mb[(long long)(t / g.r) * ldm + col];
+      if (is_spk)
+        g.d_spk[bn * g.d_s + (c - g.d_t)] = acc;
+      else
+        g.d_emo[bn * g.d_e + (c - g.d_t - g.d_s)] = acc;
+    }
+    return;
+  }
+  const I k = i - nA;
+  const int c = (int)(k % (I)Wf);
+  const I btq = k / (I)Wf;
+  const int t = (int)(btq % (I)g.Tp), b = (int)(btq / (I)g.Tp);
+  const long long bt = (long long)btq;
+  const float v = (t % g.r == 0) ? g.d_memory[((long long)b * L + t / g.r) * ldm + g.r * g.d_t + c] : 0.f;
+  if (c < g.d_s)
+    g.d_spk[bt * g.d_s + c] = v;
+  else
+    g.d_emo[bt * g.d_e + (c - g.d_s)] = v;
+}
+
+extern "C" int kantts_lr_memory_fwd(const kantts_lr_memory_args* gp, void* stream) {
+  if (!gp) return KANTTS_E_BADARG;
+  const kantts_lr_memory_args& g = *gp;
+  if (g.B < 0 || g.N < 1 || g.Tp < 0 || g.r < 1 || g.Tp % g.r || g.d_t < 1 || g.d_s < 1 || g.d_e < 1) return KANTTS_E_BADARG;
+  if (!g.text || !g.idx || !g.spk || !g.emo || !g.aug || !g.lr_text || !g.memory) return KANTTS_E_BADARG;
+  if (g.side_tokens && (!g.lr_spk || !g.lr_emo)) return KANTTS_E_BADARG;
+  const long long total = (long long)g.B * g.N * g.d_t + (long long)g.B * g.Tp * (g.d_t + g.d_s + g.d_e);
+  if (g.B == 0) return KANTTS_OK;
+  if (total + 256 < (1ll << 32))
+    hipLaunchKernelGGL(lr_memory_fwd_kernel<unsigned>, dim3(kantts_cdiv(total, 256)), dim3(256), 0, (hipStream_t)stream, g);
+  else
+    hipLaunchKernelGGL(lr_memory_fwd_kernel<long long>, dim3(kantts_cdiv(total, 256)), dim3(256), 0, (hipStream_t)stream, g);
+  KANTTS_CHECK_LAUNCH();
+}
+
+extern "C" int kantts_lr_memory_bwd(const kantts_lr_memory_bwd_args* gp, void* stream) {
+  if (!gp) return KANTTS_E_BADARG;
+  const kantts_lr_memory_bwd_args& g = *gp;
+  if (g.B < 0 || g.N < 1 || g.Tp < 0 || g.r < 1 || g.Tp % g.r || g.d_t < 1 || g.d_s < 1 || g.d_e < 1) return KANTTS_E_BADARG;
+  if (!g.d_memory || !g.cs || !g.d_text || !g.d_spk || !g.d_emo) return KANTTS_E_BADARG;
+  const long long total = (long long)g.B * g.N * (g.d_t + (g.side_tokens ? g.d_s + g.d_e : 0)) +
+                          (g.side_tokens ? 0ll : (long long)g.B * g.Tp * (g.d_s + g.d_e));
+  if (g.B == 0) return KANTTS_OK;
+  if (total + 256 < (1ll << 32))
+    hipLaunchKernelGGL(lr_memory_bwd_kernel<unsigned>, dim3(kantts_cdiv(total, 256)), dim3(256), 0, (hipStream_t)stream, g);
+  else
+    hipLaunchKernelGGL(lr_memory_bwd_kernel<long long>, dim3(kantts_cdiv(total, 256)), dim3(256), 0, (hipStream_t)stream, g);
   KANTTS_CHECK_LAUNCH();
 }
 
diff --git a/kan-tts_amd/kantts/_hip/__init__.py b/kan-tts_amd/kantts/_hip/__init__.py
--- a/kan-tts_amd/kantts/_hip/__init__.py
+++ b/kan-tts_amd/kantts/_hip/__init__.py
@@ -301,6 +301,27 @@
 class TapMajorDesc(Structure):
     _fields_ = [("src_off", c_int64), ("dst_off", c_int64), ("N", c_int32), ("Cin", c_int32), ("KT", c_int32),
                 ("pad_", c_int32)]
+
+
+class LrMemoryArgs(Structure):
+    _fields_ = [("text", c_void_p), ("add1", c_void_p), ("add2", c_void_p), ("idx", c_void_p), ("valid", c_void_p),
+                ("pos_enc", c_void_p), ("spk", c_void_p), ("emo", c_void_p), ("aug", c_void_p), ("lr_text", c_void_p),
+                ("lr_spk", c_void_p), ("lr_emo", c_void_p), ("memory", c_void_p),
+                ("B", c_int32), ("N", c_int32), ("Tp", c_int32), ("r", c_int32), ("d_t", c_int32), ("d_s", c_int32),
+                ("d_e", c_int32), ("side_tokens", c_int32)]
+
+
+class LrMemoryBwdArgs(Structure):
+    _fields_ = [("d_memory", c_void_p), ("d_aug_in", c_void_p), ("cs", c_void_p), ("valid", c_void_p),
+                ("d_text", c_void_p), ("d_spk", c_void_p), ("d_emo", c_void_p),
+                ("B", c_int32), ("N", c_int32), ("Tp", c_int32), ("r", c_int32), ("d_t", c_int32), ("d_s", c_int32),
+                ("d_e", c_int32), ("side_tokens", c_int32)]
+
+
+class RefreshImagesArgs(Structure):
+    _fields_ = [("src", c_void_p), ("flat_dst", c_void_p), ("tap_dst", c_void_p), ("frag_dst", c_void_p),
+                ("tap_table", c_void_p), ("frag_table", c_void_p), ("n", c_int64),
+                ("ntap", c_int32), ("tap_blocks", c_int32), ("nfrag", c_int32), ("frag_blocks", c_int32)]
 
 
 def available() -> bool:
@@ -418,6 +439,9 @@
         L.kantts_pnca_decode_range.argtypes = [POINTER(DecodeArgs), c_int, c_int, c_void_p]
         L.kantts_lstm_fwd_range.argtypes = [p, p, p, p, p, p, p, i, i, i, i, i, i, i, i, p]
         L.kantts_fsmn_dwconv_fwd_rows.argtypes = [p, p, p, p, p, i, i, i, i, i, i, i, p]
+        L.kantts_lr_memory_fwd.argtypes = [POINTER(LrMemoryArgs), c_void_p]
+        L.kantts_lr_memory_bwd.argtypes = [POINTER(LrMemoryBwdArgs), c_void_p]
+        L.kantts_refresh_images.argtypes = [POINTER(RefreshImagesArgs), c_void_p]
         _lib = L
     return _lib
 
@@ -443,6 +467,7 @@
     "kantts_pnca_decode_run", "kantts_pnca_decode_blob_sizes", "kantts_dur_ar_run", "kantts_dur_ar_run_f32", "kantts_ctc_attn", "kantts_ctc_attn_workspace", "kantts_enc_attn_fwd",
     "kantts_launch_tuning", "kantts_sconv_launch",
     "kantts_pnca_decode_range", "kantts_lstm_fwd_range", "kantts_fsmn_dwconv_fwd_rows",
+    "kantts_lr_memory_fwd", "kantts_lr_memory_bwd", "kantts_refresh_images",
 ]
 
 
diff --git a/kan-tts_amd/kantts/_hip/ops.py b/kan-tts_amd/kantts/_hip/ops.py
--- a/kan-tts_amd/kantts/_hip/ops.py
+++ b/kan-tts_amd/kantts/_hip/ops.py
@@ -1,3 +1,4 @@
+import ctypes
 import itertools
 import os
 import weakref
@@ -1022,6 +1023,81 @@
 
 def lr_gather(x, idx, cs, valid_lens):
     return _LRGather.apply(x, idx, cs, valid_lens)
+
+
+class _LRMemory(torch.autograd.Function):
+
+    @staticmethod
+    def forward(ctx, text, add1, add2, spk, emo, pos_enc, idx, cs, valid, r, side_tokens):
+        from . import LrMemoryArgs
+
+        text, spk, emo = _c(text), _c(spk), _c(emo)
+        add1 = None if add1 is None else _c(add1)
+        add2 = None if add2 is None else _c(add2)
+        pos_enc = None if pos_enc is None else _c(pos_enc)
+        B, N, d_t = text.shape
+        Tp, d_s, d_e = int(idx.shape[1]), int(spk.shape[2]), int(emo.shape[2])
+        rows = N if side_tokens else Tp
+        if (tuple(spk.shape[:2]) != (B, rows) or tuple(emo.shape[:2]) != (B, rows) or tuple(idx.shape) != (B, Tp)
+                or any(a is not None and a.shape != text.shape for a in (add1, add2))
+                or (pos_enc is not None and tuple(pos_enc.shape) != (B, Tp, d_t))):
+            raise ValueError("lr_memory: operand shapes do not fit")
+        new = lambda *shape: torch.empty(shape, device=text.device, dtype=torch.float32)
+        aug, lr_text = new(B, N, d_t), new(B, Tp, d_t)
+        memory = new(B, Tp // max(int(r), 1), int(r) * d_t + d_s + d_e)
+        lr_spk, lr_emo = (new(B, Tp, d_s), new(B, Tp, d_e)) if side_tokens else (None, None)
+        g = LrMemoryArgs()
+        f32 = torch.float32
+        g.text, g.add1, g.add2, g.pos_enc = ptr(text, f32), ptr(add1, f32), ptr(add2, f32), ptr(pos_enc, f32)
+        g.idx, g.valid, g.spk, g.emo = ptr(idx, torch.int32), ptr(valid, torch.int64), ptr(spk, f32), ptr(emo, f32)
+        g.aug, g.lr_text, g.lr_spk, g.lr_emo, g.memory = ptr(aug), ptr(lr_text), ptr(lr_spk), ptr(lr_emo), ptr(memory)
+        g.B, g.N, g.Tp, g.r, g.d_t, g.d_s, g.d_e, g.side_tokens = B, N, Tp, int(r), d_t, d_s, d_e, int(bool(side_tokens))
+        check(lib().kantts_lr_memory_fwd(ctypes.byref(g), stream()), "lr_memory_fwd")
+        ctx.save_for_backward(cs, valid)
+        ctx.cfg = (B, N, Tp, int(r), d_t, d_s, d_e, bool(side_tokens))
+        ctx.has_add = (add1 is not None, add2 is not None)
+        if side_tokens:
+            return aug, lr_text, lr_spk, lr_emo, memory
+        return aug, lr_text, memory
+
+    @staticmethod
+    def backward(ctx, d_aug, d_lr_text, *rest):
+        from . import LrMemoryBwdArgs
+
+        cs, valid = ctx.saved_tensors
+        B, N, Tp, r, d_t, d_s, d_e, side_tokens = ctx.cfg
+        d_lr_spk, d_lr_emo = rest[:2] if side_tokens else (None, None)
+        d_memory = rest[-1]
+        f32 = torch.float32
+        new = lambda *shape: torch.empty(shape, device=cs.device, dtype=f32)
+        if d_memory is None:
+            d_memory = torch.zeros((B, Tp // r, r * d_t + d_s + d_e), device=cs.device, dtype=f32)
+        d_memory = _c(d_memory)
+        d_aug = None if d_aug is None else _c(d_aug)
+        d_text = new(B, N, d_t)
+        d_spk, d_emo = (new(B, N, d_s), new(B, N, d_e)) if side_tokens else (new(B, Tp, d_s), new(B, Tp, d_e))
+        g = LrMemoryBwdArgs()
+        g.d_memory, g.d_aug_in, g.cs, g.valid = ptr(d_memory, f32), ptr(d_aug, f32), ptr(cs, torch.int32), ptr(valid, torch.int64)
+        g.d_text, g.d_spk, g.d_emo = ptr(d_text), ptr(d_spk), ptr(d_emo)
+        g.B, g.N, g.Tp, g.r, g.d_t, g.d_s, g.d_e, g.side_tokens = B, N, Tp, r, d_t, d_s, d_e, int(side_tokens)
+        check(lib().kantts_lr_memory_bwd(ctypes.byref(g), stream()), "lr_memory_bwd")
+        for d_lr, dx, C in ((d_lr_text, d_text, d_t), (d_lr_spk, d_spk, d_s), (d_lr_emo, d_emo, d_e)):
+            if d_lr is not None:
+                check(lib().kantts_lr_gather_bwd(ptr(_c(d_lr), f32), ptr(cs), ptr(valid), ptr(dx), B, N, Tp, C, C, 0, 1,
+                                                 stream()), "lr_gather_bwd")
+        return (d_text, d_text if ctx.has_add[0] else None, d_text if ctx.has_add[1] else None, d_spk, d_emo,
+                None, None, None, None, None, None)
+
+
+def lr_memory(text, add1, add2, spk, emo, pos_enc, idx, cs, valid_lens, r, side_tokens):
+    out = _LRMemory.apply(text, add1, add2, spk, emo, pos_enc, idx, cs, valid_lens, int(r), bool(side_tokens))
+    if side_tokens:
+        return out
+    return out[0], out[1], spk, emo, out[2]
+
+
+def has_lr_memory():
+    return hasattr(lib(), "kantts_lr_memory_fwd")
 
 
 class _FsmnMemory(torch.autograd.Function):
diff --git a/kan-tts_amd/kantts/models/sambert/kantts_sambert.py b/kan-tts_amd/kantts/models/sambert/kantts_sambert.py
--- a/kan-tts_amd/kantts/models/sambert/kantts_sambert.py
+++ b/kan-tts_amd/kantts/models/sambert/kantts_sambert.py
@@ -24,6 +24,7 @@
 _PREDICTORS_AFTER_POSTNET = bool(os.environ.get("KANTTS_PREDICTORS_AFTER_POSTNET"))
 _EARLY_FORK = bool(os.environ.get("KANTTS_EARLY_FORK"))
 _CATS_EARLY = bool(os.environ.get("KANTTS_CATS_EARLY"))
+_FUSED_HANDOVER = True
 _FLUSH_EVERY = {"dec": int(os.environ.get("KANTTS_FLUSH_EVERY_DEC", "0")), "enc": int(os.environ.get("KANTTS_FLUSH_EVERY_ENC", "4"))}
 
 
@@ -210,7 +211,7 @@
 
     def forward(self, inputs_text_embedding, inputs_emo_embedding, inputs_spk_embedding, masks=None,
                 output_masks=None, duration_targets=None, pitch_targets=None, energy_targets=None, max_out_len=None,
-                teacher_plan=None):
+                teacher_plan=None, lfr_memory=False):
         info = SeqInfo.of(masks)
         out_info = SeqInfo.of(output_masks)
 
@@ -230,7 +231,22 @@
                 energy_predictions = self.energy_predictor(variance_predictor_inputs, info)
         pitch_src = pitch_targets if pitch_targets is not None else pitch_predictions
         energy_src = energy_targets if energy_targets is not None else energy_predictions
-        if teacher_plan is not None and "pe_emb" in teacher_plan:
+        fused = None
+        if (_FUSED_HANDOVER and lfr_memory and teacher_plan is not None and duration_targets is not None
+                and len(teacher_plan["lr_plan"]) > 6 and ops.has_lr_memory()):
+            if "pe_emb" in teacher_plan:
+                add1, add2 = teacher_plan["pe_emb"], None
+            else:
+                add1 = ops.conv_cl(pitch_src.unsqueeze(-1).contiguous(), self.pitch_emb.weight, self.pitch_emb.bias, pad=4)
+                add2 = ops.conv_cl(energy_src.unsqueeze(-1).contiguous(), self.energy_emb.weight, self.energy_emb.bias, pad=4)
+            lrp = teacher_plan["lr_plan"]
+            gathered = "LR_emo" in teacher_plan
+            fused = ops.lr_memory(inputs_text_embedding, add1, add2,
+                                  teacher_plan["LR_spk"] if gathered else inputs_spk_embedding,
+                                  teacher_plan["LR_emo"] if gathered else inputs_emo_embedding,
+                                  teacher_plan["pos_enc"], lrp[0], lrp[2], lrp[6], self.length_regulator.r, not gathered)
+            aug = fused[0]
+        elif teacher_plan is not None and "pe_emb" in teacher_plan:
             aug = inputs_text_embedding + teacher_plan["pe_emb"]
         else:
             aug = (inputs_text_embedding
@@ -271,6 +287,10 @@
             plan = self.length_regulator.index(durations, max_len=max_out_len)
             pos_enc = self.position_term(plan, out_info)
         LR_length_rounded = plan[3]
+        if fused is not None:
+            _, LR_text_outputs, LR_spk_outputs, LR_emo_outputs, memory = fused
+            return (LR_text_outputs, LR_emo_outputs, LR_spk_outputs, LR_length_rounded, log_duration_predictions,
+                    pitch_predictions, energy_predictions, memory)
         LR_text_outputs, _ = self.length_regulator(aug, durations, masks=out_info, plan=plan)
         if teacher_plan is not None and "LR_emo" in teacher_plan:
             LR_emo_outputs, LR_spk_outputs = teacher_plan["LR_emo"], teacher_plan["LR_spk"]
@@ -279,7 +299,7 @@
             LR_spk_outputs, _ = self.length_regulator(inputs_spk_embedding, durations, masks=out_info, plan=plan)
         LR_text_outputs = LR_text_outputs + pos_enc
         return (LR_text_outputs, LR_emo_outputs, LR_spk_outputs, LR_length_rounded, log_duration_predictions,
-                pitch_predictions, energy_predictions)
+                pitch_predictions, energy_predictions) + ((None,) if lfr_memory else ())
 
 
 class MelPNCADecoder(nn.Module):
@@ -562,9 +582,10 @@
                 max_out_len = mel_targets.size(1)
                 out_info = tplan["out_info"] if tplan is not None else SeqInfo(output_lengths, max_out_len)
             (LR_text_outputs, LR_emo_outputs, LR_spk_outputs, LR_length_rounded, log_duration_predictions,
-             pitch_predictions, energy_predictions) = self.variance_adaptor(
+             pitch_predictions, energy_predictions, memory) = self.variance_adaptor(
                 text_hid, emo_hid, spk_hid, masks=in_info, output_masks=out_info, duration_targets=duration_targets,
-                pitch_targets=pitch_targets, energy_targets=energy_targets, max_out_len=max_out_len, teacher_plan=tplan)
+                pitch_targets=pitch_targets, energy_targets=energy_targets, max_out_len=max_out_len, teacher_plan=tplan,
+                lfr_memory=True)
         Tp = LR_text_outputs.size(1)
         if tplan is not None:
             lfr_info = tplan["lfr_info"]
@@ -574,11 +595,12 @@
             out_info = SeqInfo(LR_length_rounded, Tp)
             lfr_info = SeqInfo((LR_length_rounded + r - 1) // r, Tp // r)
         d_t, d_s, d_e = text_hid.shape[-1], spk_hid.shape[-1], emo_hid.shape[-1]
-        memory = torch.cat([
-            LR_text_outputs.reshape(batch_size, -1, r * d_t),
-            LR_spk_outputs.reshape(batch_size, -1, r * d_s)[:, :, :d_s],
-            LR_emo_outputs.reshape(batch_size, -1, r * d_e)[:, :, :d_e],
-        ], dim=-1)
+        if memory is None:
+            memory = torch.cat([
+                LR_text_outputs.reshape(batch_size, -1, r * d_t),
+                LR_spk_outputs.reshape(batch_size, -1, r * d_s)[:, :, :d_s],
+                LR_emo_outputs.reshape(batch_size, -1, r * d_e)[:, :, :d_e],
+            ], dim=-1)
         if tplan is not None:
             bw_val = tplan["bw_val"]
         elif duration_targets is not None:
diff --git a/kan-tts_amd/kantts/train/optim.py b/kan-tts_amd/kantts/train/optim.py
--- a/kan-tts_amd/kantts/train/optim.py
+++ b/kan-tts_amd/kantts/train/optim.py
@@ -2,6 +2,8 @@
 import torch.distributed as dist
 
 from kantts._hip import ops
+
+_REFRESH_ONE_LAUNCH = True
 
 
 class ParamArena:
@@ -297,6 +299,20 @@
             return
         self.shadow_stale = False
 
+        if (_REFRESH_ONE_LAUNCH and self._tap_table is not None and self._frag_table is not None
+                and hasattr(lib(), "kantts_refresh_images")):
+            import ctypes
+
+            from kantts._hip import RefreshImagesArgs
+
+            a = RefreshImagesArgs()
+            a.src, a.flat_dst = ptr(self.flat, torch.float32), ptr(self.flat_bf16, torch.bfloat16)
+            a.tap_dst, a.frag_dst = ptr(self.tap_bf16, torch.bfloat16), ptr(self.frag_bf16, torch.bfloat16)
+            a.tap_table, a.frag_table, a.n = ptr(self._tap_table), ptr(self._frag_table), self.numel
+            a.ntap, a.tap_blocks = int(self._tap_table.shape[0]), int(self._tap_blocks)
+            a.nfrag, a.frag_blocks = int(self._frag_table.shape[0]), int(self._frag_blocks)
+            check(lib().kantts_refresh_images(ctypes.byref(a), stream()), "refresh_images")
+            return
         check(lib().kantts_cast_f32_bf16(ptr(self.flat, torch.float32), ptr(self.flat_bf16, torch.bfloat16), self.numel,
                                          stream()), "cast_f32_bf16")
         if self._tap_table is not None:
```
